# jsourati/nn-active-learning

Measured on AMD Instinct MI355X. Metric: patches/sec Fisher-scored (32^3, 2-class), higher is better.
Workload: dtype f32 (fp32 operands split into 16-bit pieces on the 16-bit MFMA, fp32 accumulate: fp16 pairs - 22-23 bits kept per operand, three products - in the conv under the head (forward + backward), in dec1's forward launch and in the other backward launches; bf16 triples - all 24 bits, exact, six products -

## Files before the change

### include/alq.h

```cpp
#ifndef ALQ_H
#define ALQ_H

#include <stddef.h>
#include <stdint.h>

#ifdef __cplusplus
extern "C" {
#endif

typedef struct alq_ctx alq_ctx;
typedef struct alq_model alq_model;

enum { ALQ_OK = 0, ALQ_EINVAL = -1, ALQ_EHIP = -2, ALQ_ENOMEM = -3, ALQ_EUNSUPPORTED = -4 };

enum { ALQ_CONV = 0, ALQ_CONVT = 1, ALQ_POOL = 2, ALQ_FC = 3 };

typedef struct {
    int32_t type;
    int32_t cout;
    int32_t k[3];
    int32_t s[3];
    int32_t relu;
    int32_t skip_src;
} alq_layer_t;
// ... 111 lines not shown
    const float *d_targets;
    const float *d_old_logits;
} alq_loss_t;

int alq_loss_stats(alq_ctx *ctx, const float *d_post, int c, int N, const int32_t *d_labels, const alq_loss_t *loss,
                   double *d_stats3);

int alq_param_grads_loss(alq_model *m, const float *d_x, int N, const int32_t *d_labels, const alq_loss_t *loss,
                         float loss_scale, float lwf_scale, float keep_prob, uint64_t seed, int64_t first_sample,
                         const int32_t *h_drop_layers, int n_drop_layers, float *d_grads, float *d_post, double *d_stats3);

int alq_rmsprop_step(alq_ctx *ctx, float *d_theta, const float *d_grad, float *d_ms, float *d_mom, int64_t n, float lr,
                     float decay, float momentum, float eps);

enum { ALQ_MT_L2 = 0, ALQ_MT_CE = 1 };
int64_t alq_mt_trip_voxels(void);
int alq_mt_cotangent(alq_ctx *ctx, const float *d_post, const float *d_teacher_post, int c, int64_t R, const int32_t *d_labels,
                     const alq_loss_t *loss, float loss_scale, float cons_scale, int measure, float *d_rows, double *d_stats3);
int alq_mt_stats(alq_ctx *ctx, const float *d_post, const float *d_teacher_post, int c, int64_t R, const int32_t *d_labels,
                 const alq_loss_t *loss, int measure, double *d_stats3);
int alq_param_grads_loss_mt(alq_model *m, const float *d_x, int N, const int32_t *d_labels, const alq_loss_t *loss,
                            float loss_scale, const float *d_teacher_post, int measure, float cons_scale, float keep_prob,
                            uint64_t seed, int64_t first_sample, const int32_t *h_drop_layers, int n_drop_layers, float *d_grads,
                            float *d_post, double *d_stats3);
int alq_model_set_aleatoric(alq_model *m, int on);
int alq_forward_au(alq_model *m, const float *d_x, int N, float keep_prob, uint64_t seed, int64_t first_sample,
                   const int32_t *h_drop_layers, int n_drop_layers, float *d_post, int64_t *d_pred, float *d_au, float *d_logits);
int64_t alq_mt_au_trip_voxels(void);
int alq_mt_cotangent_au(alq_ctx *ctx, const float *d_post, const float *d_teacher_post, const float *d_au, int c, int64_t R,
                        const int32_t *d_labels, const alq_loss_t *loss, float loss_scale, float cons_scale, float au_scale,
                        float au_log_rel_coeff, int measure, float *d_rows, double *d_stats3);
int alq_mt_stats_au(alq_ctx *ctx, const float *d_post, const float *d_teacher_post, const float *d_au, int c, int64_t R,
                    const int32_t *d_labels, const alq_loss_t *loss, float au_log_rel_coeff, int measure, double *d_stats3);
int alq_param_grads_loss_mt_au(alq_model *m, const float *d_x, int N, const int32_t *d_labels, const alq_loss_t *loss,
                               float loss_scale, const float *d_teacher_post, int measure, float cons_scale, float au_scale,
                               float au_log_rel_coeff, float keep_prob, uint64_t seed, int64_t first_sample,
                               const int32_t *h_drop_layers, int n_drop_layers, float *d_grads, float *d_post, double *d_stats3);
int alq_ema_step(alq_ctx *ctx, float *d_shadow, const float *d_theta, int64_t n, float decay);
int alq_perturb_input(alq_ctx *ctx, const float *d_x, float *d_out, int N, int H, int W, int C, float noise_std, uint64_t seed,
                      int64_t first_sample, int rotate, float angle);

int alq_sq_accum(alq_ctx *ctx, const float *d_grads, int64_t per_sample_len, int N, double *d_acc);

int alq_shrink_sum(alq_ctx *ctx, const float *d_grads, int N, int64_t P, const int64_t *h_layer_elems, int L, double *d_out);
int alq_class_layer_sums(alq_model *m, const float *d_x, int N, int J, const int32_t *d_cls, float *d_post, double *d_g);

int alq_diag_fisher(alq_model *m, const float *d_x, int N, const int32_t *d_cls, double *d_acc);

size_t alq_topk_mask_work_bytes(int64_t n);
int alq_topk_mask(alq_ctx *ctx, const double *d_v, int64_t n, int64_t k, float *d_mask, void *d_work);
int alq_threshold_mask(alq_ctx *ctx, const double *d_v, int64_t n, double thr, float *d_mask);
int alq_fisher_classes(alq_ctx *ctx, const double *d_g, const double *d_w, const double *d_diag, int N, int c, int L,
                       double *d_A);

int alq_row_norms(alq_ctx *ctx, const float *d_A, int64_t n, int f, double *d_norms);
int alq_cosine_sims(alq_ctx *ctx, const float *d_A, int64_t n, const float *d_B, int b, int f, const double *d_na,
                    const double *d_nb, double *d_C);
size_t alq_colsum_work_bytes(int64_t n, int b);
int alq_colsum_max(alq_ctx *ctx, const double *d_S, int64_t n, int b, const double *d_cmax,
                   const unsigned char *d_skip, double *d_out, void *d_work);
int alq_take_colmax(alq_ctx *ctx, const double *d_S, int64_t n, int b, int j, int first, double *d_v);
int alq_fold_rowmax(alq_ctx *ctx, const double *d_S, int t, int64_t n, double *d_v);

int alq_local_var2d(alq_ctx *ctx, const void *d_vol, int vol_is_f64, const int64_t pad_dims[3], const int32_t rads[3], int d,
                    const int64_t *d_inds, int64_t n, double *d_out);
int alq_segment_min(alq_ctx *ctx, const int32_t *d_labels, const int64_t dims[3], int32_t n_labels, const int64_t *d_inds,
                    const double *d_scores, int64_t n, double *d_table);

size_t alq_cc_work_bytes(const int64_t dims[3]);
int alq_cc_label(alq_ctx *ctx, const uint8_t *d_seg, const int64_t dims[3], int connectivity, int select_zero, int32_t *d_labels);
int alq_cc_keep_largest(alq_ctx *ctx, const uint8_t *d_seg, const int64_t dims[3], int connectivity, int skip_origin, uint8_t *d_out,
                        int64_t *d_info, void *d_work);
int alq_fill_holes(alq_ctx *ctx, const uint8_t *d_seg, const int64_t dims[3], uint8_t *d_out, int64_t *d_info, void *d_work);
int alq_cc_sizes(alq_ctx *ctx, const int32_t *d_labels, int64_t n, int32_t *d_sizes);
int alq_cc_relabel(alq_ctx *ctx, const int32_t *d_labels, int64_t n, const int32_t *d_table, const int32_t *d_sizes, int32_t min_size,
                   int32_t *d_out_i32, uint8_t *d_out_u8);

typedef struct alq_dcrf_params {
    float sdims_smooth[2];
    float sdims_app[2];
    float schan;
    float compat_smooth, compat_app;
    int32_t niter;
} alq_dcrf_params;
size_t alq_dcrf_work_bytes(const int64_t dims[3]);
int alq_dcrf2d(alq_ctx *ctx, const float *d_post, const float *d_img, const int64_t dims[3], const alq_dcrf_params *par,
               float *d_q1, uint8_t *d_map, void *d_work);

int alq_llfc_grads(alq_ctx *ctx, const float *d_feat, const float *d_post, const int32_t *d_labels, int n, int d, int c,
                   float *d_out);
size_t alq_llfc_hess_max_bytes(void);
int alq_llfc_hess(alq_ctx *ctx, const float *d_feat_one, const float *d_post_one, int d, int c, double *d_H);
int alq_llfc_if_path(int d, int c);
size_t alq_llfc_if_work_bytes(int n_pool, int c);
int alq_llfc_stoch_if(alq_ctx *ctx, const float *d_pool_feat, const float *d_pool_post, const int32_t *d_pool_labels, int n_pool,
                      const float *d_tr_feat, const float *d_tr_post, int n_tr, const int32_t *d_draws, int T, double scale, int d,
                      int c, int path, float *d_V, void *d_work);

int alq_aopt_tile(void);
int alq_aopt_max_workgroups(void);
size_t alq_aopt_work_bytes(int64_t n, int L);
int alq_aopt_svec(alq_ctx *ctx, const double *d_A, int64_t n, int L, double *d_V);
int alq_aopt_stats(alq_ctx *ctx, const double *d_V, const double *d_q, int64_t n, int m, const double *h_kvec,
                   const double *h_R, double mu, double obj, double *d_out, void *d_work);
int alq_aopt_direction(alq_ctx *ctx, const double *d_V, const double *d_q, int64_t n, int m, const double *h_kvec,
                       const double *h_R, const double *h_c_r, const double *h_c_1, double ratio, double mu, double obj,
                       double *d_dq, double *d_out, void *d_work);
int alq_aopt_linesearch(alq_ctx *ctx, const double *d_q, const double *d_dq, int64_t n, const double *h_alpha, int J,
                        double *d_out, void *d_work);
int alq_aopt_update(alq_ctx *ctx, double *d_q, const double *d_dq, const double *d_V, int64_t n, int m, double alpha,
                    double *d_out, void *d_work);

typedef struct {
    int32_t layer;
    int32_t pad;
    int64_t idx;
    double delta;
} alq_flip_t;
int alq_ref64_scores(alq_ctx *ctx, const alq_layer_t *layers, int n_layers, const int32_t in_dims[4],
                     const double *const *h_dW, const double *const *h_db, const float *d_x, const int64_t *d_rows, int N,
                     const alq_flip_t *d_flips, int flips_per_sample, double eps, int cand_cap,
                     double *d_logits, double *d_S, double *d_rms, alq_flip_t *d_cand, double *d_cand_key, int32_t *d_cand_count);

int alq_prof_enable(alq_ctx *ctx, int on);
int alq_prof_reset(alq_ctx *ctx);
int alq_prof_num_classes(void);
const char *alq_prof_class_name(int cls);
int alq_prof_read(alq_ctx *ctx, int cls, double *ms, int64_t *launches, double *flops);

int alq_model_debug_copy(alq_model *m, int layer_idx, int what, int N, float *d_out,
                         int64_t *elems_out);

int alq_debug_set_stamp_buffer(void *d_buf);
int alq_debug_set(int key, int value);
enum {
    ALQ_INFO_SUBNORMALS_OK = 0,
    ALQ_INFO_C3D_FWD = 1,
    ALQ_INFO_C3D_BWD = 2,
    ALQ_INFO_C3D_ONE_ACC = 3,
    ALQ_INFO_FLIP_OVERFLOW = 5,
    ALQ_INFO_F16_DERIVED = 6,
    ALQ_INFO_T3D_FWD = 7,
    ALQ_INFO_T3D_BWD = 8,
    ALQ_INFO_E3D_BWD = 9,
    ALQ_INFO_D3D_FWD = 10,
    ALQ_INFO_D3D_BWD = 11,
    ALQ_INFO_F3D_FWD = 12,
    ALQ_INFO_C3D_BWD_FORM = 13,
    ALQ_INFO_HOST_PACK_ELEMS = 14,
    ALQ_INFO_LSUM = 15,
    ALQ_INFO_DCP_FORM = 16,
    ALQ_INFO_E3D_BWD_FORM = 17,
    ALQ_INFO_C3D_BWD_WAVES = 19,
    ALQ_INFO_C3D_BWD_GRID = 20
};
int alq_model_engine_info(alq_model *m, int what);

int alq_synth_patches(alq_ctx *ctx, uint64_t seed, int64_t first_id, int64_t n,
                      int64_t elems_per_patch, float *d_out);

enum { ALQ_SRC_F32 = 0, ALQ_SRC_F64 = 1, ALQ_SRC_I16 = 2, ALQ_SRC_U8 = 3 };
int alq_vol_pack(alq_ctx *ctx, const void *const *d_src, int m, int src_type, const int32_t *dims, float *d_out);
int alq_mask_pack(alq_ctx *ctx, const uint8_t *d_src, const int32_t *dims, uint8_t *d_out);
int alq_slice_batch_check(const int32_t *h_dims, int nvol, const int32_t *h_desc, int b, const int32_t *crop, int C);
int alq_slice_batch(alq_ctx *ctx, const float *const *h_vols, const uint8_t *const *h_masks, const int32_t *h_dims, int nvol, int m,
                    const int32_t *h_desc, int b, const int32_t *crop, int C, float *d_X, int32_t *d_lab, int64_t *d_counts);
int64_t alq_slice_batch_trip_rows(void);
int alq_slice_batch_launch_samples(void);

#ifdef __cplusplus
}
#endif
#endif
```

### nn-active-learning_amd/csrc/alq_internal.h

```cpp
#pragma once
#include <hip/hip_runtime.h>

#include <cstdint>
#include <cstdio>
#include <memory>
#include <string>
#include <vector>

#include "alq.h"
#include "engine_switches.h"
#include "model_plan.h"

namespace alq {

#define ALQ_HIP(expr)                                                                     \
    do {                                                                                  \
        hipError_t e_ = (expr);                                                           \
        if (e_ != hipSuccess) {                                                           \
            ::alq::set_error("%s:%d: %s -> %s", __FILE__, __LINE__, #expr,               \
                             hipGetErrorString(e_));                                      \
            return ALQ_EHIP;                                                              \
        }                                                                                 \
    } while (0)

// ... 172 lines not shown
    int mask_cs = 0, mask_c0 = 0, mask_from = 0;
    int mask_to = 1 << 30;
    float *osumA = nullptr, *osumB = nullptr;
    int split = 0;
    int store_from = 0;
    int mask_split = 0;
    long long mask_delta = 0;
    const unsigned char *mask_bits = nullptr;
    unsigned char *sign_out = nullptr;
    const unsigned *in_bits = nullptr;
    const float *in_vec = nullptr;
    float in_vec_amax = 0.f;
    const unsigned *in_vec16 = nullptr;
    unsigned *out_amax = nullptr;
    int amax_from = 0;
    const unsigned *in_amax = nullptr, *in_amax2 = nullptr;
    float in_bound = 0.f;
    const float *fc_W = nullptr;
    long long fc_F = 0;
    float *fc_part = nullptr;
    unsigned *fc_bits = nullptr;
    unsigned *flip_cnt = nullptr, *flip_list = nullptr;
    int flip_cap = 0;
    float flip_l1 = 0.f;
    bool flip_bias_nonzero = false;
};

extern unsigned long long *g_igemm2_dbg;
extern int g_dbg_knobs[ALQ_NKNOBS];
inline bool two_slot_allowed() { return !g_dbg_knobs[KNOB_NO_V3] && !g_dbg_knobs[KNOB_NO_V4]; }
extern int g_dcp_last_form;
extern int g_no_f16x2;
extern int g_no_fixed;
extern int g_no_xcd_order;
int igemm2_build_plan(const IgemmPlan &p1, Igemm2Plan *p2);
void igemm2_pack_weights(Igemm2Plan *p2, const std::vector<float> &Bmat);
int igemm2_launch(alq_ctx *ctx, const Igemm2Plan &plan, const View &in, const View &out, const float *bias,
                  int relu, int accumulate, int N, int prof_cls, const Igemm2Fuse *fuse);

struct Igemm3Plan {
    bool ok = false;
    bool wres = false;
    int NTW = 1;
    int wgs_per_cu = 1;
    size_t lds_bytes = 0;
    std::vector<unsigned short> h_W;
    void *d_W = nullptr;
    std::vector<unsigned short> h_W16;
    void *d_W16 = nullptr;
    int w16_exp = 0;
};
int igemm3_build_plan(const Igemm2Plan &p2, Igemm3Plan *p3);
void igemm3_pack_weights(const Igemm2Plan &p2, Igemm3Plan *p3, const std::vector<float> &Bmat);
void igemm3_pack_weights_f16(const Igemm2Plan &p2, Igemm3Plan *p3, const std::vector<float> &Bmat);
int igemm3_launch(alq_ctx *ctx, const Igemm2Plan &p2, const Igemm3Plan &plan, const View &in, const View &out,
                  const float *bias, int relu, int accumulate, int N, int prof_cls, const Igemm2Fuse *fuse);

struct Igemm4Args {
    const float *in;
    float *out;
    const void *W;
    const float *bias;
    const float *mask;
    float *osumA, *osumB;
    const int *tdesc;
    const int *sdesc;
    const int *pdesc;
    const int *ttab;
    const int *vdesc;
    int in_cs, in_c0, out_cs, out_c0, Co;
    int mask_cs, mask_c0, mask_from, mask_to, split;
    int N, PT, tpg, rows;
    int PX, PYX, PZ;
    int smz, smy, smx;
    int soz, soy, sox, OD, OH, OW;
    int MD, MH, MW;
    int nph, ngr, NP;
    int nslots, plane_bytes;
    int in_pstride, out_pstride, in_bytes;
    int relu, accumulate, pair, store_from;
    int cls_ok;
    int in_split_ch, in_delta, out_split, out_delta, mask_split, mask_delta;
    int tt_ints, pd_off, td_off, wbytes, abytes;
    int dbg_repeat;
    unsigned long long *dbg;
    const unsigned *src_bits;
    int bits_pstride, bits_bytes;
    const float *fc_W;
    float *fc_part;
    unsigned char *fc_bits;
    int fc_F;
    int f16_ein;
    int f16_ew;
    const unsigned *in_amax, *in_amax2;
    unsigned *out_amax;
    int amax_from;
    int wp;
    int src_presplit;
    int xcd_order;
    int zreuse;
    float flip_tau;
    int flip_cap;
    unsigned *flip_cnt;
    unsigned *flip_list;
    const unsigned char *mask_bits;
    unsigned char *sign_out;
};

struct Igemm4Plan {
    bool ok = false;
    Igemm4Args a;
    int NTW = 1;
    int wp = 3;
    int xw = 0;
    std::shared_ptr<Igemm4Plan> alt16;
    bool multi = false;
    bool fic = false;
    int tune_fic = -1;
    int tune_epi = -1;
    size_t lds_bytes = 0;
    double flops_per_patch = 0;
    int Ci = 0, Co = 0;
    struct Unit { int chunk = 0, S = 0, w_off = 0; std::vector<int> tap; };
    std::vector<Unit> units;
    std::vector<int> h_tdesc, h_sdesc, h_pdesc, h_ttab, h_vdesc;
    int *d_tdesc = nullptr, *d_sdesc = nullptr, *d_pdesc = nullptr, *d_ttab = nullptr, *d_vdesc = nullptr;
    std::vector<unsigned short> h_W;
    void *d_W = nullptr;
    std::vector<unsigned short> h_W16;
    void *d_W16 = nullptr;
    int w16_exp = 0;
};
int igemm4_build_plan(const G4Geom &g, int max_batch, Igemm4Plan *plan, int wp = 3);
void igemm4_pack_weights(Igemm4Plan *plan, const std::vector<float> &Bmat );
int igemm4_launch(alq_ctx *ctx, const Igemm4Plan &plan, const View &in, const View &out, const float *bias,
                  int relu, int accumulate, int N, int prof_cls, const Igemm2Fuse *fuse);

struct C3dPlan {
    bool ok = false;
    int D = 0;
    int w_exp = 0;
    int oneacc = 1;
    double flops_per_patch = 0;
    std::vector<unsigned short> h_W;
    void *d_W = nullptr;
    std::vector<unsigned short> h_W7;
    void *d_W7 = nullptr;
};
void c3d_bwd7_pack(C3dPlan *plan, const std::vector<float> &Bmat);
int c3d_subnormals_ok(alq_ctx *ctx);
int c3d_fwd_build(const View &in, const View &out, const int k[3], const int lo[3], const int s[3], C3dPlan *plan);
void c3d_fwd_pack(C3dPlan *plan, const std::vector<float> &Bmat );
int c3d_fwd_launch(alq_ctx *ctx, const C3dPlan &plan, const View &in, const float *bias, int N, const unsigned *amaxA, const unsigned *amaxB,
                   const float *fc_W, float *fc_part, float *asum_part, unsigned char *fc_bits, float flip_tau);
int c3d_bwd_build(const View &fwd_in, const View &fwd_out, const int k[3], const int lo[3], const int s[3], C3dPlan *plan);
void c3d_bwd_pack(C3dPlan *plan, const std::vector<float> &Bmat_fwd );
void c3d_presplit_vec(const float *v, long long F, int e, std::vector<unsigned short> *out);
int c3d_bwd_launch(alq_ctx *ctx, const C3dPlan &plan, int N, const unsigned char *bits, const void *vec16, int e_in, const unsigned char *maskA,
                   float *dB, float *sumA, float *sumB, int rows_per_wave = 8, int waves_per_simd = 1 ,
                   int *grid_out = nullptr );

struct T3dPlan {
    bool ok = false;
    int kind = 0;
    int w_exp = 0;
    double flops_per_patch = 0;
    std::vector<unsigned short> h_W;
    void *d_W = nullptr;
};
int t3d_build(const View &in, const View &out, const int k[3], const int lo[3], const int s[3], T3dPlan *fwd, T3dPlan *bwd);
void t3d_fwd_pack(T3dPlan *plan, const float *W );
void t3d_bwd_pack(T3dPlan *plan, const float *W);
void t3d8_fwd_pack(T3dPlan *plan, const float *W );
void t3d8_bwd_pack(T3dPlan *plan, const float *W );
int t3d8_bwd_launch(alq_ctx *ctx, const T3dPlan &plan, const View &dout, const View &din, int N, float in_bound, const unsigned char *mask_bits, float *dsum);
int t3d_fwd_launch(alq_ctx *ctx, const T3dPlan &plan, const View &in, const View &out, const float *bias, int N, float *osum, unsigned *out_amax);
int t3d_bwd_launch(alq_ctx *ctx, const T3dPlan &plan, const View &dout, const View &din, int N, float in_bound, const unsigned char *mask_bits,
                   float *dsum);

struct E3dPlan {
    bool ok = false;
    int w_exp = 0;
    double flops_per_patch = 0;
    std::vector<unsigned short> h_Whi, h_Wlo;
    void *d_Whi = nullptr, *d_Wlo = nullptr;
};
int e3d_build(const View &in, const View &out, const int k[3], const int lo[3], const int s[3], E3dPlan *plan);
void e3d_pack(E3dPlan *plan, const float *W );
int e3d_bwd_launch(alq_ctx *ctx, const E3dPlan &plan, int N, const float *skip, const float *dpool, const unsigned char *am2, const unsigned char *sg2,
                   const unsigned char *am1, const unsigned char *sg1, float *dsum2, float *dsum1, float in_bound,
                   bool rows );

struct D3dPlan {
    bool ok = false;
    int w_exp = 0;
    double flops_per_patch = 0;
    std::vector<unsigned short> h_Whi, h_Wlo;
    void *d_Whi = nullptr, *d_Wlo = nullptr;
    std::vector<unsigned short> h_Bhi, h_Blo;
    void *d_Bhi = nullptr, *d_Blo = nullptr;
};
void d3d_bwd_pack(D3dPlan *plan, const float *W);
int d3d_bwd_launch(alq_ctx *ctx, const D3dPlan &plan, int N, const float *dout, float in_bound, float *dinA, float *dinB, float *sumB);
int d3d_build(const View &in, const View &out, const int k[3], const int lo[3], const int s[3], D3dPlan *plan);
void d3d_pack(D3dPlan *plan, const float *W );
int d3d_fwd_launch(alq_ctx *ctx, const D3dPlan &plan, int N, const float *inA, const float *inB, const unsigned *amaxA, const unsigned *amaxB,
                   const float *bias, int relu, float *out, unsigned char *sg, float *osum);

struct F3dPlan {
    bool ok = false;
    int w_exp = 0;
    double flops_per_patch = 0;
    std::vector<unsigned short> h_Whi, h_Wlo;
    void *d_Whi = nullptr, *d_Wlo = nullptr;
};
int f3d_build(const View &in, const View &out, const int k[3], const int lo[3], const int s[3], F3dPlan *plan);
void f3d_pack(F3dPlan *plan, const float *W );
int f3d_fwd_launch(alq_ctx *ctx, const F3dPlan &plan, int N, const float *in, const unsigned *amax, const float *bias, float *out, unsigned char *sg,
                   float *osum, float *pout, unsigned char *parg, float *posum);

struct DirectArgs {
    const float *in;
    float *out;
    const float *W;
    const float *bias;
    float *osum;
    int in_cs, in_c0, Ci, ID, IH, IW;
    int out_cs, out_c0, Co, OD, OH, OW;
    int MD, MH, MW;
    int PT, TZ, TY, TX, HZ, HY, HX, rows;
    int minz, miny, minx;
    int ntaps, tnx, tny, tnz;
    int tilesZ, tilesY, tilesX;
    int N, relu;
};

struct DirectPlan {
    DirectArgs a;
    bool ok = false;
    size_t lds_bytes = 0;
    double flops_per_patch = 0;
    float *d_W = nullptr;
};

int direct_build_plan(const IgemmPlan &p1, DirectPlan *dp);
int direct_launch(alq_ctx *ctx, const DirectPlan &dp, const View &in, const View &out, const float *bias, int relu,
                  int N, float *osum, int prof_cls);
int direct_conv_pool_launch(alq_ctx *ctx, const float *d_W, const View &in, const View &out, const View &pout,
                            const float *bias, int relu, uint8_t *argmax, float *osum, float *posum, int N,
                            double flops_per_patch, unsigned *amax = nullptr, unsigned char *sg = nullptr, unsigned char *psg = nullptr);

struct FcGemmPlan {
    bool ok = false;
    int K = 0, N = 0;
    std::vector<unsigned short> h_W;
    void *d_W = nullptr;
    std::vector<unsigned short> h_W16;
    void *d_W16 = nullptr;
    int w_exp = 0;
    int form = 0;
};
int fcgemm_build_plan(int K, int N, FcGemmPlan *plan);
void fcgemm_pack_weights(FcGemmPlan *plan, const std::vector<float> &Bmat );
void fcgemm_pack_weights_f16(FcGemmPlan *plan, const std::vector<float> &Bmat );
int fcgemm_launch(alq_ctx *ctx, const FcGemmPlan &plan, const View &in, const View &out, const float *bias, int relu,
                  int M, int prof_cls, float in_bound = 0.f, unsigned *row_amax = nullptr);

int wpack_stats(alq_ctx *ctx, const float *d_W, int Co, long long F, void *d_scal);
int wpack_permute(alq_ctx *ctx, const float *d_W, float *d_Wp, int Co, int D, int H, int Wd, int C);
int wpack_fc(alq_ctx *ctx, const float *d_Wp, long long ld, int K, int N, int kmajor, void *d_W3, void *d_W16, const void *d_scal);

struct Gemm {
    IgemmPlan p1;
    Igemm2Plan p2;
    Igemm3Plan p3;
    Igemm4Plan p4;
    FcGemmPlan pfc;
    bool pfc_f16 = false;
    bool p3_f16 = false;
    unsigned *fc_row_amax = nullptr;
    DirectPlan pd;
};

int k_pool_fwd(alq_ctx *, const View &in, const View &out, uint8_t *argmax, const int w[3],
               const int lo[3], int N, float *osum = nullptr, bool *fused = nullptr);
int k_pool_bwd_first(alq_ctx *, const View &dout, const View &pool_out, const uint8_t *argmax, const int w[3],
                     int ID, int IH, int IW, int N, float *dsum, int accumulate, int use_signs = 0);
int k_pool_bwd(alq_ctx *, const View &dout, const View &din, const uint8_t *argmax,
               const int w[3], const int lo[3], int N, int accumulate, const View *mask_act = nullptr,
               float *dsum = nullptr, bool *fused = nullptr, int store_din = 1, int use_signs = 0);
int k_chansum(alq_ctx *, const View &in, float *field, int N);
int k_mask_chansum(alq_ctx *, const View &dact, const View *act_or_null, float *field, int N);
int boxdot_slabs(long long vox);
int boxdot_conv_slabs(int D, int H, int W, const int k[3]);
int boxdot_convT_slabs(int ID, int IH, int IW, const int k[3], const int s[3]);
int k_boxdot_conv(alq_ctx *, const float *dsum, const float *asum, const float *asum2, int D, int H, int W,
                  const int k[3], const int lo[3], int N, double *Spart, int nslab_max);
int k_boxdot_convT(alq_ctx *, const float *dsum, const float *asum, const float *asum2, int ID, int IH, int IW,
                   const int k[3], const int s[3], const int lo[3], int N, double *Spart, int nslab_max);
int k_fc_small_fwd(alq_ctx *, const float *act, int64_t F, const float *Wp, int nout, int N,
                   float *partials, int nslices, unsigned *maskbits = nullptr);
int k_fc_small_dsum_bits(alq_ctx *, const unsigned *maskbits, const float *wv, int64_t F, int N, float *dsum);
int k_fc_small_finish(alq_ctx *, const float *partials, int nslices, const float *bias, int nout,
                      int relu, int N, float *out);
int k_fc_small_finish_diff(alq_ctx *, const float *partials, int nslices, const float *bias, int N, float *out);
int k_fc_small_bwd(alq_ctx *, const float *delta, int nout, const float *Wp, int64_t F, int N,
                   float *dact, const float *mask_act = nullptr, float *dsum = nullptr, int C = 0,
// ... 151 lines not shown
```

### nn-active-learning_amd/csrc/c3d.hip

```cpp
#include "f16_pair.h"
#include "sweep_common.h"

#include <algorithm>
#include <cmath>
#include <cstdlib>
#include <cstring>
#include <vector>

namespace alq {

namespace {
#ifndef C3_SCHED_MASK
#define C3_SCHED_MASK 0
#endif
#ifndef C3_PF
#define C3_PF 8
#endif
#ifndef C3_WD
#define C3_WD 4
#endif
static_assert(C3_PF == 8 || C3_PF == 16, "the ring of staging registers must divide the 16 units of a plane");
static_assert(C3_WD >= 1 && C3_WD <= 8, "weight-difference slices are fetched 1..8 rows ahead");
#ifndef C3_ABL
#define C3_ABL 0
#endif
#ifndef C3_PIPE
#define C3_PIPE 2
#endif
#ifndef C3_FILL_MASK
#define C3_FILL_MASK SW_FILL_MASK
#endif
#ifndef C3_PIN_SUMS
#define C3_PIN_SUMS 1
#endif
#ifndef C3_PEEL
#define C3_PEEL 1
#endif
#ifndef C3_EPI2
#define C3_EPI2 1
#endif
#ifndef C3_BPIPE
#define C3_BPIPE 2
#endif
#ifndef C3_B7PIPE
#define C3_B7PIPE 4
#endif
#ifndef C3_B7PIPE2
#define C3_B7PIPE2 2
#endif
#ifndef C3_B7PINW
#define C3_B7PINW 0
#endif
#ifndef C3_B7ABL
#define C3_B7ABL 0
#endif

constexpr int C3_TEN = 34 * 16;
constexpr int C3_PIECE = 2 * C3_TEN;
constexpr int C3_ROW = 2 * C3_PIECE;
constexpr int C3_PLANE = 34 * C3_ROW;
constexpr int C3_LDS = 2 * C3_PLANE;
static_assert(C3_LDS <= 160 * 1024, "two plane images must fit the CU's LDS");
}

struct C3FwdArgs {
    const float *inA, *inB;
    const void *W;
    const float *bias;
    const unsigned *amaxA, *amaxB;
    const float *fc_W;
    float *fc_part;
    float *asum_part;
    unsigned char *fc_bits;
    int N, D;
    int e_w;
    float flip_tau;
    unsigned long long *clk;
};

template <bool SUMS, bool ONEACC>
__global__ __launch_bounds__(256) __attribute__((amdgpu_waves_per_eu(1, 1))) void c3d_fwd_kernel(const C3FwdArgs a) {
    extern __shared__ __attribute__((aligned(16))) char lds[];
    const int tid = threadIdx.x;
    const int lane = tid & 63;
    const int wave = __builtin_amdgcn_readfirstlane(tid >> 6);
    const int lr = lane & 15, lq = lane >> 4;
    const int D = a.D;
    const unsigned plane_f = 32u * 32u * 8u;
    const unsigned patch_f = (unsigned)D * plane_f;

    for (int i = tid * 16; i < C3_LDS; i += 256 * 16) *reinterpret_cast<i32x4 *>(lds + i) = i32x4{0, 0, 0, 0};

    f16x8 Wh[18], Wl[18];
    {
        const i32x4 *Wg = reinterpret_cast<const i32x4 *>(a.W);
#pragma unroll
        for (int k = 0; k < 18; ++k) {
            Wh[k] = __builtin_bit_cast(f16x8, Wg[(k * 2 + 0) * 64 + lane]);
            Wl[k] = __builtin_bit_cast(f16x8, Wg[(k * 2 + 1) * 64 + lane]);
        }
#ifndef C3_NO_PIN
#pragma unroll
        for (int k = 0; k < 18; ++k) {
            i32x4 h = __builtin_bit_cast(i32x4, Wh[k]), l = __builtin_bit_cast(i32x4, Wl[k]);
            asm volatile("" : "+a"(h), "+a"(l));
            Wh[k] = __builtin_bit_cast(f16x8, h); Wl[k] = __builtin_bit_cast(f16x8, l);
        }
#endif
    }
    const f32x4 bias4 = *reinterpret_cast<const f32x4 *>(a.bias + (lq & 1) * 4);

    const int frag_lane = (lq >> 1) * C3_TEN + (2 * lr + (lq & 1)) * 16 + wave * 8 * C3_ROW;
    const int st_lane = (wave * 8 + 1) * C3_ROW + 16 + lane * 8;
    const unsigned epi_lane_f = 16u * lr + 4u * lq;

    const int G = gridDim.x, b0 = blockIdx.x;
    const int np = b0 < a.N ? (a.N - b0 + G - 1) / G : 0;
#ifdef C3_CLK
    const unsigned long long clk0 = __builtin_amdgcn_s_memtime(), rt0 = __builtin_amdgcn_s_memrealtime();
#endif

    f32x4 acc[3][8], accx[3][ONEACC ? 1 : 8];
#pragma unroll
    for (int s = 0; s < 3; ++s)
#pragma unroll
        for (int i = 0; i < 8; ++i) { acc[s][i] = f32x4{0.f, 0.f, 0.f, 0.f}; if constexpr (!ONEACC) accx[s][i] = f32x4{0.f, 0.f, 0.f, 0.f}; }

    typedef const unsigned __attribute__((address_space(4))) *cu32p;
    const cu32p amaxA_c = (cu32p)(unsigned long long)a.amaxA, amaxB_c = (cu32p)(unsigned long long)a.amaxB;
    auto patch_exp = [&](int p) __attribute__((always_inline)) {
        const unsigned fa = amaxA_c[p], fb = amaxB_c[p];
        return sw_patch_exp(fa > fb ? fa : fb);
    };
    const __amdgpu_buffer_rsrc_t inA_rsrc = sw_rsrc(a.inA, (unsigned long long)a.N * patch_f * 4u);
    const __amdgpu_buffer_rsrc_t inB_rsrc = sw_rsrc(a.inB, (unsigned long long)a.N * patch_f * 4u);
    const __amdgpu_buffer_rsrc_t wd_rsrc = sw_rsrc(a.fc_W, (unsigned long long)patch_f * 4u);
    const __amdgpu_buffer_rsrc_t bits_rsrc = sw_rsrc(a.fc_bits, (SUMS && a.fc_bits) ? (unsigned long long)a.N * (patch_f >> 2) : 0ull);
    auto patch_of = [&](int pi) __attribute__((always_inline)) { return (unsigned)(b0 + pi * G); };

    f32x4 R4[C3_PF];
    float sc = 1.f, sc11 = 2048.f;
    auto stage_unit = [&](int wbase, auto U) __attribute__((always_inline)) {
        constexpr int u = decltype(U)::value;
        const f32x4 v = R4[u % C3_PF];
        const float x0 = v.x * sc, x1 = v.y * sc, x2 = v.z * sc, x3 = v.w * sc;
        const f16x2 h01 = __builtin_convertvector(f32x2{x0, x1}, f16x2);
        const f16x2 h23 = __builtin_convertvector(f32x2{x2, x3}, f16x2);
        const f32x2 g01 = __builtin_convertvector(h01, f32x2), g23 = __builtin_convertvector(h23, f32x2);
        f16x2 l01, l23;
        if constexpr (ONEACC) {
            l01 = __builtin_convertvector(f32x2{x0 - g01.x, x1 - g01.y}, f16x2);
            l23 = __builtin_convertvector(f32x2{x2 - g23.x, x3 - g23.y}, f16x2);
        } else {
            l01 = __builtin_convertvector(f32x2{__builtin_fmaf(g01.x, -2048.f, v.x * sc11), __builtin_fmaf(g01.y, -2048.f, v.y * sc11)}, f16x2);
            l23 = __builtin_convertvector(f32x2{__builtin_fmaf(g23.x, -2048.f, v.z * sc11), __builtin_fmaf(g23.y, -2048.f, v.w * sc11)}, f16x2);
        }
        char *dst = lds + wbase + (u >> 1) * C3_ROW + (u & 1) * C3_TEN;
        if constexpr (C3_ABL & 64) { asm volatile("" :: "v"(h01), "v"(h23), "v"(l01), "v"(l23), "v"(dst)); return; }
        *reinterpret_cast<uint2 *>(dst) = uint2{__builtin_bit_cast(unsigned, h01), __builtin_bit_cast(unsigned, h23)};
        *reinterpret_cast<uint2 *>(dst + C3_PIECE) = uint2{__builtin_bit_cast(unsigned, l01), __builtin_bit_cast(unsigned, l23)};
    };
    auto load_unit = [&](unsigned voff, unsigned soff, auto U) __attribute__((always_inline)) {
        constexpr int u = decltype(U)::value;
        R4[u % C3_PF] = __builtin_bit_cast(f32x4, __builtin_amdgcn_raw_buffer_load_b128((u & 1) ? inB_rsrc : inA_rsrc, (int)voff, (int)(soff + (unsigned)((u % 16) >> 1) * 1024u), 0));
    };
    struct Cur { unsigned voff, soff; };
    auto cursor = [&](int pi, int z) __attribute__((always_inline)) {
        Cur c;
        const bool ok = pi < np;
        c.voff = ok ? (unsigned)lane * 16u : SW_OOB;
        c.soff = ok ? (patch_of(pi) * patch_f + (unsigned)z * plane_f) * 4u + (unsigned)(wave * 8) * 1024u : 0u;
        if constexpr (C3_ABL & 8) c.soff = (unsigned)(wave * 8) * 1024u;
        return c;
    };
    int c1_pi = 0, c1_z = 0, c2_pi = 0, c2_z = 0;
    auto advance = [&](int &pi, int &z) __attribute__((always_inline)) { if (++z == D) { z = 0; ++pi; } };

    float fs = 0.f, sa = 0.f;
    f32x4 wdq[C3_WD];
#pragma unroll
    for (int i = 0; i < C3_WD; ++i) wdq[i] = f32x4{0.f, 0.f, 0.f, 0.f};

    struct Epi { float inv; f32x4 b4; float tau; unsigned tau_u; unsigned zadj; unsigned off_w, off_b, row_f, bits_s; };
    auto epi_setup = [&](bool valid, int pe, int zo) __attribute__((always_inline)) {
        Epi e;
        const int p = valid ? (int)patch_of(pe) : 0;
        const int ce = valid ? patch_exp(p) : 0;
        e.inv = valid ? __builtin_ldexpf(1.f, -(ce + a.e_w)) : 0.f;
        e.b4 = valid ? bias4 : f32x4{0.f, 0.f, 0.f, 0.f};
        e.tau = (valid && (amaxA_c[p] | amaxB_c[p]) != 0u) ? __builtin_ldexpf(a.flip_tau, 14 - ce) : 0.f;
        e.tau_u = e.tau > 0.f ? (__builtin_bit_cast(unsigned, e.tau) - 1u) >> 1 : 0u;
        e.zadj = (bias4.x == 0.f && bias4.y == 0.f && bias4.z == 0.f && bias4.w == 0.f) ? 1u : 0u;
        e.off_w = valid ? epi_lane_f * 4u : SW_OOB;
        e.off_b = valid ? (epi_lane_f >> 2) : SW_OOB;
        e.row_f = (unsigned)(zo * 32 + wave * 8) * 256u;
        e.bits_s = (unsigned)p * (patch_f >> 2);
        return e;
    };
    auto wd_load = [&](const Epi &E, auto I) __attribute__((always_inline)) {
        constexpr int i = decltype(I)::value;
        if constexpr (C3_ABL & 32) return;
        wdq[i % C3_WD] = __builtin_bit_cast(f32x4, __builtin_amdgcn_raw_buffer_load_b128(wd_rsrc, (int)E.off_w, (int)((E.row_f + (unsigned)i * 256u) * 4u), 0));
    };

    auto wd_first = [&](const Epi &E) __attribute__((always_inline)) {
        wd_load(E, IC<0>{});
        if constexpr (C3_WD > 1) wd_load(E, IC<1>{});
        if constexpr (C3_WD > 2) wd_load(E, IC<2>{});
        if constexpr (C3_WD > 3) wd_load(E, IC<3>{});
        if constexpr (C3_WD > 4) wd_load(E, IC<4>{});
        if constexpr (C3_WD > 5) wd_load(E, IC<5>{});
        if constexpr (C3_WD > 6) wd_load(E, IC<6>{});
        if constexpr (C3_WD > 7) wd_load(E, IC<7>{});
    };
    auto epi_row = [&](auto S, auto I, const Epi &E) __attribute__((always_inline)) {
        constexpr int s = decltype(S)::value, i = decltype(I)::value;
        const f32x4 w4 = wdq[i % C3_WD];
        if constexpr (i + C3_WD < 8) wd_load(E, IC<i + C3_WD>{});
        const f32x4 c = acc[s][i];
        f32x4 val;
        if constexpr (ONEACC) {
            val.x = __builtin_fmaf(c.x, E.inv, E.b4.x); val.y = __builtin_fmaf(c.y, E.inv, E.b4.y);
            val.z = __builtin_fmaf(c.z, E.inv, E.b4.z); val.w = __builtin_fmaf(c.w, E.inv, E.b4.w);
        } else {
            const f32x4 d = accx[s][i];
            val.x = __builtin_fmaf(__builtin_fmaf(d.x, 0x1p-11f, c.x), E.inv, E.b4.x);
            val.y = __builtin_fmaf(__builtin_fmaf(d.y, 0x1p-11f, c.y), E.inv, E.b4.y);
            val.z = __builtin_fmaf(__builtin_fmaf(d.z, 0x1p-11f, c.z), E.inv, E.b4.z);
            val.w = __builtin_fmaf(__builtin_fmaf(d.w, 0x1p-11f, c.w), E.inv, E.b4.w);
        }
        unsigned unsure = 0u;
        if constexpr (SUMS) {
            const float mn = fminf(fminf(__builtin_fabsf(val.x), __builtin_fabsf(val.y)), fminf(__builtin_fabsf(val.z), __builtin_fabsf(val.w)));
#if C3_EPI2
            unsure = (((__builtin_bit_cast(unsigned, mn) - E.zadj) >> 1) - E.tau_u) >> 31;
#else
            unsure = (mn < E.tau && mn > 0.f) ? 16u : 0u;
#endif
        }
        val.x = fmaxf(val.x, 0.f); val.y = fmaxf(val.y, 0.f); val.z = fmaxf(val.z, 0.f); val.w = fmaxf(val.w, 0.f);
        fs += __builtin_fmaf(val.y, w4.y, val.x * w4.x) + __builtin_fmaf(val.w, w4.w, val.z * w4.z);
        if constexpr (SUMS) {
            sa += (val.x + val.y) + (val.z + val.w);
#if C3_EPI2
            const float r0 = val.x, r1 = val.y, r2 = val.z, r3 = val.w;
            unsigned nib = unsure;
            nib = __builtin_amdgcn_alignbit(nib, 0u - __builtin_bit_cast(unsigned, r3), 31);
            nib = __builtin_amdgcn_alignbit(nib, 0u - __builtin_bit_cast(unsigned, r2), 31);
            nib = __builtin_amdgcn_alignbit(nib, 0u - __builtin_bit_cast(unsigned, r1), 31);
            nib = __builtin_amdgcn_alignbit(nib, 0u - __builtin_bit_cast(unsigned, r0), 31);
#else
            const unsigned nib = (val.x > 0.f ? 1u : 0u) | (val.y > 0.f ? 2u : 0u) | (val.z > 0.f ? 4u : 0u) | (val.w > 0.f ? 8u : 0u) | unsure;
#endif
            if constexpr (!(C3_ABL & 16))
                __builtin_amdgcn_raw_buffer_store_b8((unsigned char)nib, bits_rsrc, (int)E.off_b, (int)(E.bits_s + ((E.row_f + (unsigned)i * 256u) >> 2)), 0);
            else asm volatile("" :: "v"(nib));
        }
#if C3_PIN_SUMS
        if constexpr (SUMS) asm volatile("" : "+v"(fs), "+v"(sa));
        else asm volatile("" : "+v"(fs));
#endif
    };
    auto wave_sum = [&](float x) __attribute__((always_inline)) {
        int v = __builtin_bit_cast(int, x);
#define C3_ROW_SHR_ADD(n) v = __builtin_bit_cast(int, __builtin_bit_cast(float, v) + __builtin_bit_cast(float, __builtin_amdgcn_update_dpp(0, v, 0x110 + (n), 0xf, 0xf, true)))
        C3_ROW_SHR_ADD(1); C3_ROW_SHR_ADD(2); C3_ROW_SHR_ADD(4); C3_ROW_SHR_ADD(8);
#undef C3_ROW_SHR_ADD
        const float r0 = __builtin_bit_cast(float, __builtin_amdgcn_readlane(v, 15));
        const float r1 = __builtin_bit_cast(float, __builtin_amdgcn_readlane(v, 31));
        const float r2 = __builtin_bit_cast(float, __builtin_amdgcn_readlane(v, 47));
        const float r3 = __builtin_bit_cast(float, __builtin_amdgcn_readlane(v, 63));
        return (r0 + r1) + (r2 + r3);
    };
    auto finish_patch = [&](int p) __attribute__((always_inline)) {
        const float t = wave_sum(fs);
        if (lane == 0) a.fc_part[(size_t)p * 4 + wave] = t;
        if constexpr (SUMS) {
            const float u = wave_sum(sa);
            if (lane == 0 && a.asum_part) a.asum_part[(size_t)p * 4 + wave] = u;
        }
        fs = 0.f; sa = 0.f;
    };

    auto step = [&](auto RR, int pi, int z, long long n) __attribute__((always_inline)) {
        constexpr int R = decltype(RR)::value;
        constexpr int S_lo = (R + 2) % 3, S_mid = R, S_hi = (R + 1) % 3;
        if constexpr (!(C3_ABL & 4)) asm volatile("s_waitcnt lgkmcnt(0)\n\ts_barrier" ::: "memory");
        const int abase = frag_lane + (int)(n & 1) * C3_PLANE;
        const int wbase = st_lane + (int)((n + 1) & 1) * C3_PLANE;
        const Cur C1 = cursor(c1_pi, c1_z), C2 = cursor(c2_pi, c2_z);
        {
            const int ce = c1_pi < np ? patch_exp((int)patch_of(c1_pi)) : 0;
            sc = __builtin_ldexpf(1.f, ce); sc11 = __builtin_ldexpf(1.f, ce + 11);
        }
        const bool ev = z >= 2 || (z == 0 && pi > 0);
        const Epi E = epi_setup(ev, z >= 2 ? pi : pi - 1, z >= 2 ? z - 2 : D - 1);

        auto frag = [&](int j, int s, f16x8 &bh, f16x8 &bl) __attribute__((always_inline)) {
            const char *p = lds + abase + j * C3_ROW + s * 32;
            bh = __builtin_bit_cast(f16x8, *reinterpret_cast<const i32x4 *>(p));
            bl = __builtin_bit_cast(f16x8, *reinterpret_cast<const i32x4 *>(p + C3_PIECE));
        };
        f16x8 Fh[3], Fl[3];
        frag(0, 0, Fh[0], Fl[0]);
        frag(0, 1, Fh[1], Fl[1]);
        auto block = [&](auto J, auto SS) __attribute__((always_inline)) {
            constexpr int j = decltype(J)::value, s = decltype(SS)::value, b = 2 * j + s;
            __builtin_amdgcn_sched_barrier(0);
            if constexpr (s == 0 && j < 8) {
                if constexpr (!(C3_ABL & 2)) epi_row(IC<S_hi>{}, J, E);
            }
            if constexpr (!(C3_ABL & 1) && j >= 2) {
                constexpr int u = 2 * (j - 2) + s;
                stage_unit(wbase, IC<u>{});
                if constexpr (u + C3_PF < 16) load_unit(C1.voff, C1.soff, IC<u + C3_PF>{}); else load_unit(C2.voff, C2.soff, IC<u + C3_PF - 16>{});
            }
            if constexpr (b + 2 < 20) frag((b + 2) / 2, (b + 2) & 1, Fh[(b + 2) % 3], Fl[(b + 2) % 3]);
            const f16x8 bh = Fh[b % 3], bl = Fl[b % 3];
            constexpr int rows_here = (j < 2 ? j + 1 : 3) < (10 - j) ? (j < 2 ? j + 1 : 3) : (10 - j);
#pragma unroll
            for (int di = 0; di < 3; ++di) {
                const int i = j - di;
                if (i < 0 || i > 7) continue;
#pragma unroll
                for (int dzi = 0; dzi < 3; ++dzi) {
                    const int k = (dzi * 3 + di) * 2 + s;
                    const int set = dzi == 0 ? S_hi : (dzi == 1 ? S_mid : S_lo);
                    const bool start = dzi == 0 && di == 0 && s == 0;
                    f32x4 c = acc[set][i];
                    if (start) c = f32x4{0.f, 0.f, 0.f, 0.f};
                    if constexpr (ONEACC) {
                        c = __builtin_amdgcn_mfma_f32_16x16x32_f16(Wl[k], bh, c, 0, 0, 0);
                        c = __builtin_amdgcn_mfma_f32_16x16x32_f16(Wh[k], bl, c, 0, 0, 0);
                        c = __builtin_amdgcn_mfma_f32_16x16x32_f16(Wh[k], bh, c, 0, 0, 0);
                    } else {
                        f32x4 d = accx[set][i];
                        if (start) d = f32x4{0.f, 0.f, 0.f, 0.f};
                        d = __builtin_amdgcn_mfma_f32_16x16x32_f16(Wl[k], bh, d, 0, 0, 0);
                        c = __builtin_amdgcn_mfma_f32_16x16x32_f16(Wh[k], bh, c, 0, 0, 0);
                        d = __builtin_amdgcn_mfma_f32_16x16x32_f16(Wh[k], bl, d, 0, 0, 0);
                        accx[set][i] = d;
                    }
                    acc[set][i] = c;
                }
            }
#if C3_PIPE
#pragma unroll
            for (int m = 0; m < 9 * rows_here; ++m) {
                __builtin_amdgcn_sched_group_barrier(0x008, 1, 0);
                __builtin_amdgcn_sched_group_barrier(C3_FILL_MASK, C3_PIPE, 0);
            }
#endif
        };
        auto row = [&](auto J) __attribute__((always_inline)) { block(J, IC<0>{}); block(J, IC<1>{}); };
        row(IC<0>{}); row(IC<1>{}); row(IC<2>{}); row(IC<3>{}); row(IC<4>{});
        row(IC<5>{}); row(IC<6>{}); row(IC<7>{}); row(IC<8>{}); row(IC<9>{});
        {
            const Epi En = epi_setup(z + 1 < D ? z >= 1 : true, pi, z + 1 < D ? z - 1 : D - 2);
            wd_first(En);
        }
        if constexpr (R == 0) { if (z == 0 && pi > 0) finish_patch((int)patch_of(pi - 1)); }
        c1_pi = c2_pi; c1_z = c2_z;
        advance(c2_pi, c2_z);
    };
    auto light = [&](auto S, int pe, int zo) __attribute__((always_inline)) {
        constexpr int s = decltype(S)::value;
        const Epi E = epi_setup(true, pe, zo);
        auto rows = [&](auto I) __attribute__((always_inline)) { epi_row(S, I, E); };
        rows(IC<0>{}); rows(IC<1>{}); rows(IC<2>{}); rows(IC<3>{}); rows(IC<4>{}); rows(IC<5>{}); rows(IC<6>{}); rows(IC<7>{});
#pragma unroll
        for (int i = 0; i < 8; ++i) { acc[s][i] = f32x4{0.f, 0.f, 0.f, 0.f}; if constexpr (!ONEACC) accx[s][i] = f32x4{0.f, 0.f, 0.f, 0.f}; }
        {
            const Epi En = epi_setup(zo == D - 2, pe, D - 1);
            wd_first(En);
        }
    };

    __syncthreads();
    if (np > 0) {
        const Cur C0 = cursor(0, 0);
        const int ce = patch_exp((int)patch_of(0));
        sc = __builtin_ldexpf(1.f, ce); sc11 = __builtin_ldexpf(1.f, ce + 11);
        const int wb = st_lane;
        auto eight = [&](auto U0) __attribute__((always_inline)) {
            constexpr int u0 = decltype(U0)::value;
            load_unit(C0.voff, C0.soff, IC<u0>{}); load_unit(C0.voff, C0.soff, IC<u0 + 1>{}); load_unit(C0.voff, C0.soff, IC<u0 + 2>{}); load_unit(C0.voff, C0.soff, IC<u0 + 3>{});
            load_unit(C0.voff, C0.soff, IC<u0 + 4>{}); load_unit(C0.voff, C0.soff, IC<u0 + 5>{}); load_unit(C0.voff, C0.soff, IC<u0 + 6>{}); load_unit(C0.voff, C0.soff, IC<u0 + 7>{});
            stage_unit(wb, IC<u0>{}); stage_unit(wb, IC<u0 + 1>{}); stage_unit(wb, IC<u0 + 2>{}); stage_unit(wb, IC<u0 + 3>{});
            stage_unit(wb, IC<u0 + 4>{}); stage_unit(wb, IC<u0 + 5>{}); stage_unit(wb, IC<u0 + 6>{}); stage_unit(wb, IC<u0 + 7>{});
        };
        eight(IC<0>{}); eight(IC<8>{});
        c1_pi = 0; c1_z = 0;
        advance(c1_pi, c1_z);
        c2_pi = c1_pi; c2_z = c1_z;
        advance(c2_pi, c2_z);
        const Cur C1 = cursor(c1_pi, c1_z);
        load_unit(C1.voff, C1.soff, IC<0>{}); load_unit(C1.voff, C1.soff, IC<1>{}); load_unit(C1.voff, C1.soff, IC<2>{}); load_unit(C1.voff, C1.soff, IC<3>{});
        load_unit(C1.voff, C1.soff, IC<4>{}); load_unit(C1.voff, C1.soff, IC<5>{}); load_unit(C1.voff, C1.soff, IC<6>{}); load_unit(C1.voff, C1.soff, IC<7>{});
        if constexpr (C3_PF == 16) {
            load_unit(C1.voff, C1.soff, IC<8>{}); load_unit(C1.voff, C1.soff, IC<9>{}); load_unit(C1.voff, C1.soff, IC<10>{}); load_unit(C1.voff, C1.soff, IC<11>{});
            load_unit(C1.voff, C1.soff, IC<12>{}); load_unit(C1.voff, C1.soff, IC<13>{}); load_unit(C1.voff, C1.soff, IC<14>{}); load_unit(C1.voff, C1.soff, IC<15>{});
        }
    }

    long long n = 0;
    for (int pi = 0; pi < np; ++pi) {
#if C3_PEEL
        for (int zz = 0; zz < 10; ++zz) {
            step(IC<0>{}, pi, 3 * zz, n); ++n;
            step(IC<1>{}, pi, 3 * zz + 1, n); ++n;
            step(IC<2>{}, pi, 3 * zz + 2, n); ++n;
        }
        step(IC<0>{}, pi, 30, n); ++n;
        step(IC<1>{}, pi, 31, n); ++n;
        light(IC<0>{}, pi, D - 2);
#else
        for (int zz = 0; zz < 11; ++zz) {
            step(IC<0>{}, pi, 3 * zz, n); ++n;
            step(IC<1>{}, pi, 3 * zz + 1, n); ++n;
            if (zz < 10) { step(IC<2>{}, pi, 3 * zz + 2, n); ++n; }
            else light(IC<0>{}, pi, D - 2);
        }
#endif
    }
    if (np > 0) {
        light(IC<1>{}, np - 1, D - 1);
        finish_patch((int)patch_of(np - 1));
    }
#ifdef C3_CLK
    if (a.clk && tid == 0) { a.clk[2 * b0] = __builtin_amdgcn_s_memtime() - clk0; a.clk[2 * b0 + 1] = __builtin_amdgcn_s_memrealtime() - rt0; }
#endif
}

namespace {
constexpr int B3_TEN = 34 * 16;
constexpr int B3_ROW = 2 * B3_TEN;
}

struct C3BwdArgs {
    const unsigned char *bits;
    const void *vec;
    const void *W;
    const unsigned char *maskA;
    float *dB;
    float *sumA, *sumB;
    int N, D;
    int e_in, e_w;
};

template <bool ONEACC, int RW>
__global__ __launch_bounds__(256) __attribute__((amdgpu_waves_per_eu(1, 1))) void c3d_bwd_kernel(const C3BwdArgs a) {
    extern __shared__ __attribute__((aligned(16))) char lds[];
    static_assert(ONEACC, "the backward kernel is built for the one-accumulator form");
    static_assert(RW == 4 || RW == 8, "4 waves x RW rows: a half or a whole patch per workgroup");
    constexpr int NR = 4 * RW;
    constexpr int NPARTS = 32 / NR;
    constexpr int PLANE = (NR + 2) * B3_ROW;
    constexpr int DUMMY = 2 * PLANE;
    constexpr int NU = RW / 2;
    const int tid = threadIdx.x;
    const int lane = tid & 63;
    const int wave = __builtin_amdgcn_readfirstlane(tid >> 6);
    const int lj = lane & 15, lq = lane >> 4;
    const int D = a.D;
    const unsigned plane_v = 32u * 32u;
    const unsigned patch_v = (unsigned)D * plane_v;

    for (int i = tid * 16; i < DUMMY + 2 * B3_ROW; i += 256 * 16) *reinterpret_cast<i32x4 *>(lds + i) = i32x4{0, 0, 0, 0};

    f16x8 Wh[9], Wl[9];
    {
        const i32x4 *Wg = reinterpret_cast<const i32x4 *>(a.W);
#pragma unroll
        for (int k = 0; k < 9; ++k) {
            Wh[k] = __builtin_bit_cast(f16x8, Wg[(k * 2 + 0) * 64 + lane]);
            Wl[k] = __builtin_bit_cast(f16x8, Wg[(k * 2 + 1) * 64 + lane]);
        }
        if constexpr (RW == 4) {
#pragma unroll
            for (int k = 0; k < 9; ++k) {
                i32x4 h = __builtin_bit_cast(i32x4, Wh[k]), l = __builtin_bit_cast(i32x4, Wl[k]);
                asm volatile("" : "+a"(h), "+a"(l));
                Wh[k] = __builtin_bit_cast(f16x8, h); Wl[k] = __builtin_bit_cast(f16x8, l);
            }
        }
    }
    const int frag_lane = (lj + (lq < 2 ? lq : 2)) * 16 + wave * RW * B3_ROW;
    const int st_lane = (wave * RW + 1 + (lane >> 5)) * B3_ROW + ((lane & 31) + 1) * 16;
    const float inv = __builtin_ldexpf(1.f, -(a.e_in + a.e_w));

    const int G = gridDim.x, b0 = blockIdx.x;
    const int nitems = a.N * NPARTS;
    const int np = b0 < nitems ? (nitems - b0 + G - 1) / G : 0;

    f32x4 acc[3][RW][2];
#pragma unroll
    for (int s = 0; s < 3; ++s)
#pragma unroll
        for (int i = 0; i < RW; ++i) { acc[s][i][0] = f32x4{0.f, 0.f, 0.f, 0.f}; acc[s][i][1] = f32x4{0.f, 0.f, 0.f, 0.f}; }

    const __amdgpu_buffer_rsrc_t vec_rsrc = sw_rsrc(a.vec, (unsigned long long)patch_v * 32u);
    const __amdgpu_buffer_rsrc_t bits_rsrc = sw_rsrc(a.bits, (unsigned long long)a.N * patch_v * 2u);
    const __amdgpu_buffer_rsrc_t mask_rsrc = sw_rsrc(a.maskA, a.maskA ? (unsigned long long)a.N * patch_v * 2u : 0ull);
    const __amdgpu_buffer_rsrc_t dB_rsrc = sw_rsrc(a.dB, (unsigned long long)a.N * patch_v * 32u);
    const __amdgpu_buffer_rsrc_t sA_rsrc = sw_rsrc(a.sumA, (unsigned long long)a.N * patch_v * 4u);
    const __amdgpu_buffer_rsrc_t sB_rsrc = sw_rsrc(a.sumB, (unsigned long long)a.N * patch_v * 4u);
    auto item_patch = [&](int pi) __attribute__((always_inline)) { return (unsigned)((b0 + pi * G) / NPARTS); };
    auto item_y0 = [&](int pi) __attribute__((always_inline)) { return ((b0 + pi * G) % NPARTS) * NR; };

    i32x4 Vh[2], Vl[2], Hh, Hl;
    unsigned Sb[2], Hb = 0u;
    struct Src { unsigned voff, vvox, soff; };
    auto src_of = [&](int pi, bool halo) __attribute__((always_inline)) {
        Src c;
        const bool ok = pi < np;
        const int y0 = ok ? item_y0(pi) : 0;
        int y = y0 + wave * RW + (lane >> 5);
        bool live = ok;
        if (halo) {
            y = wave == 0 ? y0 - 1 : y0 + NR;
            live = ok && lane < 32 && y >= 0 && y < 32;
        }
        c.vvox = (unsigned)((live ? y : 0) * 32 + (lane & 31));
        c.voff = live ? c.vvox * 2u : SW_OOB;
        c.soff = ok ? item_patch(pi) * patch_v * 2u : 0u;
        return c;
    };
    auto mask8 = [&](int b, i32x4 h, i32x4 l, i32x4 *oh, i32x4 *ol) __attribute__((always_inline)) {
// ... 211 lines not shown
        }
        c1_pi = 0; c1_z = 0;
        advance(c1_pi, c1_z);
        c2_pi = c1_pi; c2_z = c1_z;
        advance(c2_pi, c2_z);
        const Src C1 = src_of(c1_pi, false);
        load_unit(C1, (unsigned)c1_z, IC<0>{}); load_unit(C1, (unsigned)c1_z, IC<1>{});
        if constexpr (RW == 4) { if (halo_wave) load_halo(src_of(c1_pi, true), (unsigned)c1_z); }
    }
    long long n = 0;
    for (int pi = 0; pi < np; ++pi) {
#if C3_PEEL
        for (int zz = 0; zz < 10; ++zz) {
            step(IC<0>{}, pi, 3 * zz, n); ++n;
            step(IC<1>{}, pi, 3 * zz + 1, n); ++n;
            step(IC<2>{}, pi, 3 * zz + 2, n); ++n;
        }
        step(IC<0>{}, pi, 30, n); ++n;
        step(IC<1>{}, pi, 31, n); ++n;
        light(IC<0>{}, pi, D - 2);
#else
        for (int zz = 0; zz < 11; ++zz) {
            step(IC<0>{}, pi, 3 * zz, n); ++n;
            step(IC<1>{}, pi, 3 * zz + 1, n); ++n;
            if (zz < 10) { step(IC<2>{}, pi, 3 * zz + 2, n); ++n; }
            else light(IC<0>{}, pi, D - 2);
        }
#endif
    }
    if (np > 0) light(IC<1>{}, np - 1, D - 1);
}

namespace {
constexpr int P7_ROW = 34 * 16;
constexpr int P7_PIECE = 34 * P7_ROW;
constexpr int P7_PLANE = 2 * P7_PIECE + 128;
constexpr int P7_LDS = 4 * P7_PLANE;
constexpr int P7_WS = 2 * 64 * 16;
static_assert((P7_ROW / 16) % 16 == 2 && (P7_PLANE / 16) % 16 == 0 && P7_LDS + P7_WS <= 160 * 1024, "bank-conflict-free pitches (see above)");
}

template <int RW, int NW>
__global__ __launch_bounds__(NW * 64) __attribute__((amdgpu_waves_per_eu(NW / 4, NW / 4))) void c3d_bwd7_kernel(const C3BwdArgs a) {
    extern __shared__ __attribute__((aligned(16))) char lds[];
    static_assert(RW * NW == 32 && (NW == 4 || NW == 8), "the waves' strips of RW rows tile the 32 rows of a plane");
    constexpr int NU = RW / 2;
    constexpr int FSETS = NW == 4 ? 2 : 1;
    constexpr int PIPE = NW == 4 ? C3_B7PIPE : C3_B7PIPE2;
    constexpr bool WS_LDS = NW == 8;
    const int tid = threadIdx.x;
    const int lane = tid & 63;
    const int wave = __builtin_amdgcn_readfirstlane(tid >> 6);
    const int lj = lane & 15, lq = lane >> 4;
    const int D = a.D;
    const unsigned plane_v = 32u * 32u;
    const unsigned patch_v = (unsigned)D * plane_v;

    for (int i = tid * 16; i < P7_LDS; i += NW * 64 * 16) *reinterpret_cast<i32x4 *>(lds + i) = i32x4{0, 0, 0, 0};

    f16x8 Wa[3][2], Wb[3][2], Ws[2];
    {
        const i32x4 *Wg = reinterpret_cast<const i32x4 *>(a.W);
#pragma unroll
        for (int dz = 0; dz < 3; ++dz)
#pragma unroll
            for (int pc = 0; pc < 2; ++pc) {
                Wa[dz][pc] = __builtin_bit_cast(f16x8, Wg[((0 + dz) * 2 + pc) * 64 + lane]);
                Wb[dz][pc] = __builtin_bit_cast(f16x8, Wg[((3 + dz) * 2 + pc) * 64 + lane]);
            }
        Ws[0] = __builtin_bit_cast(f16x8, Wg[(6 * 2 + 0) * 64 + lane]);
        Ws[1] = __builtin_bit_cast(f16x8, Wg[(6 * 2 + 1) * 64 + lane]);
        if constexpr (WS_LDS) {
            if (wave == 0) {
                *reinterpret_cast<i32x4 *>(lds + P7_LDS + lane * 16) = __builtin_bit_cast(i32x4, Ws[0]);
                *reinterpret_cast<i32x4 *>(lds + P7_LDS + 1024 + lane * 16) = __builtin_bit_cast(i32x4, Ws[1]);
            }
        }
#if C3_B7PINW
#pragma unroll
        for (int dz = 0; dz < 3; ++dz)
#pragma unroll
            for (int pc = 0; pc < 2; ++pc) {
                i32x4 x = __builtin_bit_cast(i32x4, Wa[dz][pc]), y = __builtin_bit_cast(i32x4, Wb[dz][pc]);
                asm volatile("" : "+a"(x), "+a"(y));
                Wa[dz][pc] = __builtin_bit_cast(f16x8, x); Wb[dz][pc] = __builtin_bit_cast(f16x8, y);
            }
#endif
    }
    const int offA = wave * RW * P7_ROW + (lq < 3 ? (lj + lq) * 16 : P7_ROW + lj * 16);
    const int offB = (wave * RW + 1) * P7_ROW + (lq < 2 ? (lj + 1 + lq) * 16 : P7_ROW + (lj + lq - 2) * 16);
    const int offS = (wave * RW + 2) * P7_ROW + (lj + 2) * 16;
    const int ringS = lq < 2 ? lq + 2 : 0;
    const int st_lane = (wave * RW + 1 + (lane >> 5)) * P7_ROW + ((lane & 31) + 1) * 16;
    const float inv = __builtin_ldexpf(1.f, -(a.e_in + a.e_w));

    const int G = gridDim.x, b0 = blockIdx.x;
    const int np = b0 < a.N ? (a.N - b0 + G - 1) / G : 0;

    f32x4 acc[3][RW][2];
#pragma unroll
    for (int s = 0; s < 3; ++s)
#pragma unroll
        for (int i = 0; i < RW; ++i) { acc[s][i][0] = f32x4{0.f, 0.f, 0.f, 0.f}; acc[s][i][1] = f32x4{0.f, 0.f, 0.f, 0.f}; }

    const __amdgpu_buffer_rsrc_t vec_rsrc = sw_rsrc(a.vec, (unsigned long long)patch_v * 32u);
    const __amdgpu_buffer_rsrc_t bits_rsrc = sw_rsrc(a.bits, (unsigned long long)a.N * patch_v * 2u);
    const __amdgpu_buffer_rsrc_t mask_rsrc = sw_rsrc(a.maskA, a.maskA ? (unsigned long long)a.N * patch_v * 2u : 0ull);
    const __amdgpu_buffer_rsrc_t dB_rsrc = sw_rsrc(a.dB, (unsigned long long)a.N * patch_v * 32u);
    const __amdgpu_buffer_rsrc_t sA_rsrc = sw_rsrc(a.sumA, (unsigned long long)a.N * patch_v * 4u);
    const __amdgpu_buffer_rsrc_t sB_rsrc = sw_rsrc(a.sumB, (unsigned long long)a.N * patch_v * 4u);
    auto item_patch = [&](int pi) __attribute__((always_inline)) { return (unsigned)(b0 + pi * G); };

    i32x4 Vh[2], Vl[2];
    unsigned Sb[2];
    struct Src { unsigned voff, vvox, soff; };
    auto src_of = [&](int pi) __attribute__((always_inline)) {
        Src c;
        const bool ok = pi < np;
        const int y = wave * RW + (lane >> 5);
        c.vvox = (unsigned)(y * 32 + (lane & 31));
        c.voff = ok ? c.vvox * 2u : SW_OOB;
        c.soff = ok ? item_patch(pi) * patch_v * 2u : 0u;
        return c;
    };
    auto mask8 = [&](int b, i32x4 h, i32x4 l, i32x4 *oh, i32x4 *ol) __attribute__((always_inline)) {
        const unsigned m0 = (unsigned)__builtin_amdgcn_sbfe(b, 0, 1), m1 = (unsigned)__builtin_amdgcn_sbfe(b, 1, 1);
        const unsigned m2 = (unsigned)__builtin_amdgcn_sbfe(b, 2, 1), m3 = (unsigned)__builtin_amdgcn_sbfe(b, 3, 1);
        const unsigned m4 = (unsigned)__builtin_amdgcn_sbfe(b, 8, 1), m5 = (unsigned)__builtin_amdgcn_sbfe(b, 9, 1);
        const unsigned m6 = (unsigned)__builtin_amdgcn_sbfe(b, 10, 1), m7 = (unsigned)__builtin_amdgcn_sbfe(b, 11, 1);
        const unsigned k0 = (m0 & 0xffffu) | (m1 & 0xffff0000u), k1 = (m2 & 0xffffu) | (m3 & 0xffff0000u);
        const unsigned k2 = (m4 & 0xffffu) | (m5 & 0xffff0000u), k3 = (m6 & 0xffffu) | (m7 & 0xffff0000u);
        *oh = i32x4{(int)((unsigned)h.x & k0), (int)((unsigned)h.y & k1), (int)((unsigned)h.z & k2), (int)((unsigned)h.w & k3)};
        *ol = i32x4{(int)((unsigned)l.x & k0), (int)((unsigned)l.y & k1), (int)((unsigned)l.z & k2), (int)((unsigned)l.w & k3)};
    };
    auto load_unit = [&](const Src &c, unsigned z, auto U) __attribute__((always_inline)) {
        constexpr int u = decltype(U)::value;
        const unsigned so = (z * plane_v + (unsigned)u * 64u);
        Vh[u & 1] = __builtin_amdgcn_raw_buffer_load_b128(vec_rsrc, (int)(c.vvox * 32u), (int)(so * 32u), 0);
        Vl[u & 1] = __builtin_amdgcn_raw_buffer_load_b128(vec_rsrc, (int)(c.vvox * 32u + 16u), (int)(so * 32u), 0);
        Sb[u & 1] = (unsigned short)__builtin_amdgcn_raw_buffer_load_b16(bits_rsrc, (int)c.voff, (int)(c.soff + so * 2u), 0);
    };
    auto stage_unit = [&](int wbase, auto U) __attribute__((always_inline)) {
        constexpr int u = decltype(U)::value;
        i32x4 oh, ol;
        mask8((int)Sb[u & 1], Vh[u & 1], Vl[u & 1], &oh, &ol);
        char *dst = lds + wbase + (2 * u) * P7_ROW;
        *reinterpret_cast<i32x4 *>(dst) = oh;
        *reinterpret_cast<i32x4 *>(dst + P7_PIECE) = ol;
    };

    int c1_pi = 0, c1_z = 0, c2_pi = 0, c2_z = 0;
    auto advance = [&](int &pi, int &z) __attribute__((always_inline)) { if (++z == D) { z = 0; ++pi; } };

    unsigned mkq[2][2] = {{0u, 0u}, {0u, 0u}};
    struct Epi { unsigned pv; unsigned row_v; float inv; unsigned off_mask, off_dB, off_sum; };
    auto epi_setup = [&](bool valid, int pe, int zo) __attribute__((always_inline)) {
        Epi e;
        e.pv = valid ? item_patch(pe) * patch_v : 0u;
        e.row_v = (unsigned)(zo * 32 + wave * RW) * 32u;
        e.inv = valid ? inv : 0.f;
        e.off_mask = (valid && lq < 2) ? (unsigned)(lj * 2 + lq) : SW_OOB;
        e.off_dB = (valid && lq >= 2) ? (unsigned)lj * 32u + (unsigned)(lq - 2) * 16u : SW_OOB;
        e.off_sum = valid ? (unsigned)((lq & 1) * 16 + lj) * 4u : SW_OOB;
        return e;
    };
    auto mask_load = [&](const Epi &E, auto I) __attribute__((always_inline)) {
        constexpr int i = decltype(I)::value;
#pragma unroll
        for (int hx = 0; hx < 2; ++hx)
            mkq[i & 1][hx] = (unsigned char)__builtin_amdgcn_raw_buffer_load_b8(mask_rsrc, (int)E.off_mask,
                                                                               (int)((E.pv + E.row_v + (unsigned)i * 32u + (unsigned)hx * 16u) * 2u), 0);
    };
    const bool has_mask = a.maskA != nullptr;
    float t_keep = 0.f;
    auto epi_half = [&](auto S, auto I, auto HX, const Epi &E) __attribute__((always_inline)) {
        constexpr int s = decltype(S)::value, i = decltype(I)::value, hx = decltype(HX)::value;
        const unsigned mk = mkq[i & 1][hx];
        if constexpr (hx == 1 && i + 2 < RW) mask_load(E, IC<i + 2>{});
        const f32x4 c = acc[s][i][hx];
        const int nib = (lq < 2 && has_mask) ? (int)mk : 15;
        const float v0 = c.x * E.inv, v1 = c.y * E.inv, v2 = c.z * E.inv, v3 = c.w * E.inv;
        f32x4 val;
        unsigned k0 = (unsigned)__builtin_amdgcn_sbfe(nib, 0, 1), k1 = (unsigned)__builtin_amdgcn_sbfe(nib, 1, 1);
        unsigned k2 = (unsigned)__builtin_amdgcn_sbfe(nib, 2, 1), k3 = (unsigned)__builtin_amdgcn_sbfe(nib, 3, 1);
        asm("" : "+v"(k0), "+v"(k1), "+v"(k2), "+v"(k3));
        val.x = __builtin_bit_cast(float, __builtin_bit_cast(unsigned, v0) & k0);
        val.y = __builtin_bit_cast(float, __builtin_bit_cast(unsigned, v1) & k1);
        val.z = __builtin_bit_cast(float, __builtin_bit_cast(unsigned, v2) & k2);
        val.w = __builtin_bit_cast(float, __builtin_bit_cast(unsigned, v3) & k3);
        const unsigned vox = E.pv + E.row_v + (unsigned)i * 32u + (unsigned)hx * 16u;
        __builtin_amdgcn_raw_buffer_store_b128(__builtin_bit_cast(i32x4, val), dB_rsrc, (int)E.off_dB, (int)(vox * 32u), 2 );
        if constexpr (!(C3_B7ABL & 8)) ALQ_STORE_HOLD("v"(val));
        const float t = (val.x + val.y) + (val.z + val.w);
        const unsigned tu = __builtin_bit_cast(unsigned, t);
        const auto sw = hx == 0 ? __builtin_amdgcn_permlane16_swap(tu, 0u, false, false) : __builtin_amdgcn_permlane16_swap(0u, tu, false, false);
        const unsigned s0 = sw[0], s1 = sw[1];
        const float t2 = __builtin_bit_cast(float, s0) + __builtin_bit_cast(float, s1);
        if constexpr (hx == 0) {
            t_keep = t2;
        } else {
            const float ts = t_keep + t2;
            const unsigned rowv = E.pv + E.row_v + (unsigned)i * 32u;
            __builtin_amdgcn_raw_buffer_store_b32(__builtin_bit_cast(int, ts), sA_rsrc, (int)(lq < 2 ? E.off_sum : SW_OOB), (int)(rowv * 4u), 0);
            __builtin_amdgcn_raw_buffer_store_b32(__builtin_bit_cast(int, ts), sB_rsrc, (int)(lq >= 2 ? E.off_sum : SW_OOB), (int)(rowv * 4u), 0);
        }
    };
    auto epi_row = [&](auto S, auto I, const Epi &E) __attribute__((always_inline)) {
        epi_half(S, I, IC<0>{}, E);
        epi_half(S, I, IC<1>{}, E);
    };
    auto s_weights = [&](int kill, f16x8 &sh, f16x8 &sl) __attribute__((always_inline)) {
        const int km = lq == kill ? 0 : -1;
        i32x4 h, l;
        if constexpr (WS_LDS) {
            h = *reinterpret_cast<const i32x4 *>(lds + P7_LDS + lane * 16);
            l = *reinterpret_cast<const i32x4 *>(lds + P7_LDS + 1024 + lane * 16);
        } else {
            h = __builtin_bit_cast(i32x4, Ws[0]); l = __builtin_bit_cast(i32x4, Ws[1]);
        }
        h.x &= km; h.y &= km; h.z &= km; h.w &= km;
        l.x &= km; l.y &= km; l.z &= km; l.w &= km;
        sh = __builtin_bit_cast(f16x8, h); sl = __builtin_bit_cast(f16x8, l);
    };
    auto mac3 = [&](f32x4 c, const f16x8 &wh, const f16x8 &wl, const f16x8 &bh, const f16x8 &bl) __attribute__((always_inline)) {
        c = __builtin_amdgcn_mfma_f32_16x16x32_f16(wl, bh, c, 0, 0, 0);
        c = __builtin_amdgcn_mfma_f32_16x16x32_f16(wh, bl, c, 0, 0, 0);
        c = __builtin_amdgcn_mfma_f32_16x16x32_f16(wh, bh, c, 0, 0, 0);
        return c;
    };

    auto step = [&](auto RR, int pi, int z, long long n) __attribute__((always_inline)) {
        constexpr int R = decltype(RR)::value;
        constexpr int S_lo = (R + 2) % 3, S_mid = R, S_hi = (R + 1) % 3;
        asm volatile("s_waitcnt lgkmcnt(0)\n\ts_barrier" ::: "memory");
        const int cur = (int)(n & 3) * P7_PLANE;
        const int baseA = offA + cur, baseB = offB + cur;
        const int baseS = offS + (int)((unsigned)((int)(n & 3) + ringS) & 3u) * P7_PLANE;
        const int wbase = st_lane + (int)((n + 1) & 3) * P7_PLANE;
        const Src C1 = src_of(c1_pi), C2 = src_of(c2_pi);
        const unsigned z1 = (unsigned)c1_z, z2 = (unsigned)c2_z;
        const bool ev = z >= 2 || (z == 0 && pi > 0);
        const Epi E = epi_setup(ev, z >= 2 ? pi : pi - 1, z >= 2 ? z - 2 : D - 1);
        f16x8 sh, sl;
        s_weights(z == 1 ? 0 : -1, sh, sl);

        struct Frag { f16x8 ah, al, bh, bl, sh, sl; };
        auto frag_s = [&](int i, int hx, Frag &f) __attribute__((always_inline)) {
            const int o = i * P7_ROW + hx * 256;
            f.sh = __builtin_bit_cast(f16x8, *reinterpret_cast<const i32x4 *>(lds + baseS + o));
            f.sl = __builtin_bit_cast(f16x8, *reinterpret_cast<const i32x4 *>(lds + baseS + o + P7_PIECE));
        };
        auto frag_a = [&](int i, int hx, Frag &f) __attribute__((always_inline)) {
            const int o = i * P7_ROW + hx * 256;
            f.ah = __builtin_bit_cast(f16x8, *reinterpret_cast<const i32x4 *>(lds + baseA + o));
            f.al = __builtin_bit_cast(f16x8, *reinterpret_cast<const i32x4 *>(lds + baseA + o + P7_PIECE));
        };
        auto frag_b = [&](int i, int hx, Frag &f) __attribute__((always_inline)) {
            const int o = i * P7_ROW + hx * 256;
            f.bh = __builtin_bit_cast(f16x8, *reinterpret_cast<const i32x4 *>(lds + baseB + o));
            f.bl = __builtin_bit_cast(f16x8, *reinterpret_cast<const i32x4 *>(lds + baseB + o + P7_PIECE));
        };
        auto frag_ab = [&](int i, int hx, Frag &f) __attribute__((always_inline)) { frag_a(i, hx, f); frag_b(i, hx, f); };
        auto frag = [&](int i, int hx, Frag &f) __attribute__((always_inline)) { frag_ab(i, hx, f); frag_s(i, hx, f); };
        Frag fc, fn;
        if constexpr (FSETS == 2) frag(0, 0, fc);
        if constexpr (FSETS == 1) frag_a(0, 0, fc);
        auto mfma_half = [&](auto I, int hx) __attribute__((always_inline)) {
            constexpr int i = decltype(I)::value;
            f32x4 c0 = f32x4{0.f, 0.f, 0.f, 0.f}, c1 = acc[S_mid][i][hx], c2 = acc[S_lo][i][hx];
            c0 = mac3(c0, Wa[0][0], Wa[0][1], fc.ah, fc.al);
            c1 = mac3(c1, Wa[1][0], Wa[1][1], fc.ah, fc.al);
            c2 = mac3(c2, Wa[2][0], Wa[2][1], fc.ah, fc.al);
            c0 = mac3(c0, Wb[0][0], Wb[0][1], fc.bh, fc.bl);
            c1 = mac3(c1, Wb[1][0], Wb[1][1], fc.bh, fc.bl);
            c2 = mac3(c2, Wb[2][0], Wb[2][1], fc.bh, fc.bl);
            if constexpr (!(C3_B7ABL & 4)) c2 = mac3(c2, sh, sl, fc.sh, fc.sl);
            acc[S_hi][i][hx] = c0; acc[S_mid][i][hx] = c1; acc[S_lo][i][hx] = c2;
        };
        auto row = [&](auto I) __attribute__((always_inline)) {
            constexpr int i = decltype(I)::value;
            __builtin_amdgcn_sched_barrier(0);
            if constexpr (FSETS == 1) {
                static_assert(NU == 2, "two units per plane and wave");
#pragma unroll
                for (int hx = 0; hx < 2; ++hx) {
                    frag_b(i, hx, fc);
                    if constexpr (!(C3_B7ABL & 4)) frag_s(i, hx, fc);
                    if constexpr (!(C3_B7ABL & 1)) {
                        if (hx == 0) epi_half(IC<S_hi>{}, I, IC<0>{}, E);
                        else epi_half(IC<S_hi>{}, I, IC<1>{}, E);
                    } else { const f32x4 k0 = acc[S_hi][i][hx]; asm volatile("" :: "v"(k0)); }
                    if (hx == 0) frag_a(i, 1, fn);
                    else if (i < RW - 1) frag_a(i + 1, 0, fn);
                    if constexpr ((i & 1) == 0 && !(C3_B7ABL & 2)) {
                        if (hx == 1) {
                            stage_unit(wbase, IC<i / 2>{});
                            load_unit(C2, z2, IC<i / 2>{});
                        }
                    }
                    mfma_half(I, hx);
                    fc.ah = fn.ah; fc.al = fn.al;
                    if constexpr (PIPE != 0) {
#pragma unroll
                        for (int m = 0; m < 21; ++m) {
                            __builtin_amdgcn_sched_group_barrier(0x008, 1, 0);
                            __builtin_amdgcn_sched_group_barrier(C3_FILL_MASK, PIPE, 0);
                        }
                        __builtin_amdgcn_sched_barrier(0);
                    }
                }
                return;
            }
            if constexpr (!(C3_B7ABL & 1)) epi_row(IC<S_hi>{}, I, E);
            else { const f32x4 k0 = acc[S_hi][i][0], k1 = acc[S_hi][i][1]; asm volatile("" :: "v"(k0), "v"(k1)); }
            if constexpr ((i & 1) == 0 && !(C3_B7ABL & 2)) {
                stage_unit(wbase, IC<i / 2>{});
                if constexpr (i / 2 + 2 < NU) load_unit(C1, z1, IC<i / 2 + 2>{}); else load_unit(C2, z2, IC<i / 2 + 2 - NU>{});
            }
#pragma unroll
            for (int hx = 0; hx < 2; ++hx) {
                if (hx == 0) frag(i, 1, fn);
                else if (i < RW - 1) frag(i + 1, 0, fn);
                mfma_half(I, hx);
                fc = fn;
            }
            if constexpr (PIPE != 0) {
#pragma unroll
                for (int m = 0; m < 42; ++m) {
                    __builtin_amdgcn_sched_group_barrier(0x008, 1, 0);
                    __builtin_amdgcn_sched_group_barrier(C3_FILL_MASK, PIPE, 0);
                }
            }
        };
        row(IC<0>{}); row(IC<1>{}); row(IC<2>{}); row(IC<3>{});
        if constexpr (RW == 8) { row(IC<4>{}); row(IC<5>{}); row(IC<6>{}); row(IC<7>{}); }
        {
            const Epi En = epi_setup(z + 1 < D ? z >= 1 : true, pi, z + 1 < D ? z - 1 : D - 2);
            mask_load(En, IC<0>{});
            mask_load(En, IC<1>{});
        }
        c1_pi = c2_pi; c1_z = c2_z;
        advance(c2_pi, c2_z);
    };
    auto light = [&](auto S, auto LAST, int pe, int zo, long long n) __attribute__((always_inline)) {
        constexpr int s = decltype(S)::value;
        constexpr bool last = decltype(LAST)::value != 0;
        const Epi E = epi_setup(true, pe, zo);
        auto rows = [&](auto I) __attribute__((always_inline)) { epi_row(S, I, E); };
        rows(IC<0>{}); rows(IC<1>{}); rows(IC<2>{}); rows(IC<3>{});
        if constexpr (RW == 8) { rows(IC<4>{}); rows(IC<5>{}); rows(IC<6>{}); rows(IC<7>{}); }
#pragma unroll
        for (int i = 0; i < RW; ++i) { acc[s][i][0] = f32x4{0.f, 0.f, 0.f, 0.f}; acc[s][i][1] = f32x4{0.f, 0.f, 0.f, 0.f}; }
        if constexpr (last) {
            constexpr int sp = (s + 1) % 3;
            f16x8 sh, sl;
            s_weights(2, sh, sl);
            const int baseS = offS + (int)((unsigned)((int)(n & 3) + ringS) & 3u) * P7_PLANE;
#pragma unroll
            for (int i = 0; i < RW; ++i)
#pragma unroll
                for (int hx = 0; hx < 2; ++hx) {
                    const int o = i * P7_ROW + hx * 256;
                    const f16x8 bh = __builtin_bit_cast(f16x8, *reinterpret_cast<const i32x4 *>(lds + baseS + o));
                    const f16x8 bl = __builtin_bit_cast(f16x8, *reinterpret_cast<const i32x4 *>(lds + baseS + o + P7_PIECE));
                    acc[sp][i][hx] = mac3(acc[sp][i][hx], sh, sl, bh, bl);
                }
        }
        {
            const Epi En = epi_setup(zo == D - 2, pe, D - 1);
            mask_load(En, IC<0>{});
            mask_load(En, IC<1>{});
        }
    };

    __syncthreads();
    if (np > 0) {
        const Src C0 = src_of(0);
        const int wb = st_lane;
        load_unit(C0, 0u, IC<0>{}); load_unit(C0, 0u, IC<1>{});
        stage_unit(wb, IC<0>{}); stage_unit(wb, IC<1>{});
        if constexpr (NU == 4) {
            load_unit(C0, 0u, IC<2>{}); load_unit(C0, 0u, IC<3>{});
            stage_unit(wb, IC<2>{}); stage_unit(wb, IC<3>{});
        }
        c1_pi = 0; c1_z = 0;
        advance(c1_pi, c1_z);
        c2_pi = c1_pi; c2_z = c1_z;
        advance(c2_pi, c2_z);
        const Src C1 = src_of(c1_pi);
        load_unit(C1, (unsigned)c1_z, IC<0>{}); load_unit(C1, (unsigned)c1_z, IC<1>{});
    }
    long long n = 0;
    for (int pi = 0; pi < np; ++pi) {
        for (int zz = 0; zz < 10; ++zz) {
            step(IC<0>{}, pi, 3 * zz, n); ++n;
            step(IC<1>{}, pi, 3 * zz + 1, n); ++n;
            step(IC<2>{}, pi, 3 * zz + 2, n); ++n;
        }
        step(IC<0>{}, pi, 30, n); ++n;
        step(IC<1>{}, pi, 31, n); ++n;
        light(IC<0>{}, IC<1>{}, pi, D - 2, n);
    }
    if (np > 0) light(IC<1>{}, IC<0>{}, np - 1, D - 1, n);
}

__global__ void c3d_subnormal_probe(float *out) {
    f16x8 a, b;
#pragma unroll
    for (int i = 0; i < 8; ++i) { a[i] = (_Float16)0x1p-20f; b[i] = (_Float16)0x1p10f; }
    const f32x4 d = __builtin_amdgcn_mfma_f32_16x16x32_f16(a, b, f32x4{0.f, 0.f, 0.f, 0.f}, 0, 0, 0);
    if (threadIdx.x == 0) out[0] = d.x;
}

int c3d_subnormals_ok(alq_ctx *ctx) {
    if (ctx->f16_subnormal_mfma >= 0) return ctx->f16_subnormal_mfma;
    float *d = nullptr, h = -1.f;
    if (hipMalloc(&d, sizeof(float)) != hipSuccess) { (void)hipGetLastError(); return 0; }
    hipLaunchKernelGGL(c3d_subnormal_probe, dim3(1), dim3(64), 0, ctx->stream, d);
    const bool ok = hipGetLastError() == hipSuccess &&
                    hipMemcpyAsync(&h, d, sizeof(float), hipMemcpyDeviceToHost, ctx->stream) == hipSuccess &&
                    hipStreamSynchronize(ctx->stream) == hipSuccess;
    (void)hipFree(d);
    if (!ok) { (void)hipGetLastError(); return 0; }
    ctx->f16_subnormal_mfma = (h == 0x1p-5f) ? 1 : 0;
    return ctx->f16_subnormal_mfma;
}

int c3d_fwd_build(const View &in, const View &out, const int k[3], const int lo[3], const int s[3], C3dPlan *plan) {
    plan->ok = false;
    if (getenv("ALQ_NO_C3D")) return ALQ_OK;
    if (!is_conv3_same(k, lo, s)) return ALQ_OK;
    if (!(in.D == 32 && in.H == 32 && in.W == 32 && out.D == 32 && out.H == 32 && out.W == 32)) return ALQ_OK;
    if (!(in.C == 16 && in.split == 8 && in.cs == 8 && in.c0 == 0 && out.C == 8)) return ALQ_OK;
    plan->D = in.D;
    plan->oneacc = getenv("ALQ_C3D_TWOACC") ? 0 : 1;
    plan->flops_per_patch = 2.0 * 27 * 16 * 8 * (double)in.vox();
    plan->ok = true;
    return ALQ_OK;
}

void c3d_fwd_pack(C3dPlan *plan, const std::vector<float> &Bmat) {
    plan->w_exp = f16_pair_exp(Bmat.data(), Bmat.size());
    plan->h_W.assign((size_t)18 * 2 * 64 * 8, 0);
    for (int dzi = 0; dzi < 3; ++dzi)
        for (int dyi = 0; dyi < 3; ++dyi)
            for (int s = 0; s < 2; ++s)
                for (int lane = 0; lane < 64; ++lane) {
                    const int i = lane & 15, kg = lane >> 4, v = i >> 3, co = i & 7, t = kg >> 1, p = kg & 1;
                    const int dxi = 2 * s + p - v;
                    const int ks = (dzi * 3 + dyi) * 2 + s;
                    for (int c = 0; c < 8; ++c) {
                        float w = 0.f;
                        if (dxi >= 0 && dxi <= 2) w = Bmat[((size_t)((dzi * 3 + dyi) * 3 + dxi) * 16 + 8 * t + c) * 8 + co];
                        f16_pair_split(w, plan->w_exp, plan->oneacc ? 0 : 11, &plan->h_W[((size_t)(ks * 2 + 0) * 64 + lane) * 8 + c],
                                       &plan->h_W[((size_t)(ks * 2 + 1) * 64 + lane) * 8 + c]);
                    }
                }
}

int c3d_fwd_launch(alq_ctx *ctx, const C3dPlan &plan, const View &in, const float *bias, int N, const unsigned *amaxA, const unsigned *amaxB,
                   const float *fc_W, float *fc_part, float *asum_part, unsigned char *fc_bits, float flip_tau) {
    ALQ_REQUIRE(plan.ok && plan.d_W, ALQ_EINVAL, "c3d: weights not set");
    ALQ_REQUIRE(in.split == 8 && in.cs == 8 && in.C == 16 && in.D == plan.D && in.H == 32 && in.W == 32 && plan.D == 32, ALQ_EINVAL, "c3d: input view mismatch");
    ALQ_REQUIRE(amaxA && amaxB && fc_W && fc_part && bias, ALQ_EINVAL, "c3d: missing argument");
    SWEEP_REQUIRE_PATCHES(N, "c3d");
    if (N <= 0) return ALQ_OK;
    C3FwdArgs a;
    a.inA = in.p; a.inB = in.p + in.delta; a.W = plan.d_W; a.bias = bias; a.amaxA = amaxA; a.amaxB = amaxB;
    a.fc_W = fc_W; a.fc_part = fc_part; a.asum_part = asum_part; a.fc_bits = fc_bits; a.N = N; a.D = plan.D; a.e_w = plan.w_exp;
    a.flip_tau = flip_tau; a.clk = nullptr;
    const unsigned grid = (unsigned)std::min(N, 256);
    ProfScope ps(ctx, PROF_IGEMM_F16, plan.flops_per_patch * N);
    auto go = [&](auto kfn) { return sweep_launch(ctx, kfn, grid, 256, C3_LDS, a); };
    if (fc_bits) return plan.oneacc ? go(c3d_fwd_kernel<true, true>) : go(c3d_fwd_kernel<true, false>);
    return plan.oneacc ? go(c3d_fwd_kernel<false, true>) : go(c3d_fwd_kernel<false, false>);
}

int c3d_bwd_build(const View &fwd_in, const View &fwd_out, const int k[3], const int lo[3], const int s[3], C3dPlan *plan) {
    C3dPlan f;
    ALQ_TRY(c3d_fwd_build(fwd_in, fwd_out, k, lo, s, &f));
    plan->ok = f.ok;
    plan->D = f.D;
    plan->oneacc = 1;
    plan->flops_per_patch = f.flops_per_patch;
    return ALQ_OK;
}

void c3d_bwd_pack(C3dPlan *plan, const std::vector<float> &Bmat) {
    plan->w_exp = f16_pair_exp(Bmat.data(), Bmat.size());
    plan->h_W.assign((size_t)9 * 2 * 64 * 8, 0);
    for (int dzi = 0; dzi < 3; ++dzi)
        for (int di = 0; di < 3; ++di)
            for (int lane = 0; lane < 64; ++lane) {
                const int ci = lane & 15, kg = lane >> 4;
                const int ks = dzi * 3 + di;
                for (int c = 0; c < 8; ++c) {
                    float w = 0.f;
                    if (kg < 3) w = Bmat[((size_t)(((2 - dzi) * 3 + (2 - di)) * 3 + (2 - kg)) * 16 + ci) * 8 + c];
                    f16_pair_split(w, plan->w_exp, 0, &plan->h_W[((size_t)(ks * 2 + 0) * 64 + lane) * 8 + c], &plan->h_W[((size_t)(ks * 2 + 1) * 64 + lane) * 8 + c]);
                }
            }
}

void c3d_bwd7_pack(C3dPlan *plan, const std::vector<float> &Bmat) {
    plan->h_W7.assign((size_t)7 * 2 * 64 * 8, 0);
    for (int f = 0; f < 7; ++f)
        for (int lane = 0; lane < 64; ++lane) {
            const int ci = lane & 15, q = lane >> 4;
            int dz = -1, dy = 0, dx = 0;
            if (f < 3) { dz = f; if (q < 3) { dy = 0; dx = q; } else { dy = 1; dx = 0; } }
            else if (f < 6) { dz = f - 3; const int p = 4 + q; dy = p / 3; dx = p % 3; }
            else if (q < 3) { dz = q; dy = 2; dx = 2; }
            for (int c = 0; c < 8; ++c) {
                float w = 0.f;
                if (dz >= 0) w = Bmat[((size_t)(((2 - dz) * 3 + (2 - dy)) * 3 + (2 - dx)) * 16 + ci) * 8 + c];
                f16_pair_split(w, plan->w_exp, 0, &plan->h_W7[((size_t)(f * 2 + 0) * 64 + lane) * 8 + c], &plan->h_W7[((size_t)(f * 2 + 1) * 64 + lane) * 8 + c]);
            }
        }
}

void c3d_presplit_vec(const float *v, long long F, int e, std::vector<unsigned short> *out) {
    out->assign((size_t)F * 2, 0);
    for (long long vox = 0; vox < F / 8; ++vox)
        for (int c = 0; c < 8; ++c) f16_pair_split(v[vox * 8 + c], e, 0, &(*out)[(size_t)vox * 16 + c], &(*out)[(size_t)vox * 16 + 8 + c]);
}

int c3d_bwd_launch(alq_ctx *ctx, const C3dPlan &plan, int N, const unsigned char *bits, const void *vec16, int e_in, const unsigned char *maskA,
                   float *dB, float *sumA, float *sumB, int rows_per_wave, int waves_per_simd, int *grid_out) {
    ALQ_REQUIRE(plan.ok && plan.d_W && plan.D == 32, ALQ_EINVAL, "c3d: backward weights not set");
    ALQ_REQUIRE(bits && vec16 && dB && sumA && sumB, ALQ_EINVAL, "c3d: missing argument");
    SWEEP_REQUIRE_PATCHES(N, "c3d");
    if (grid_out) *grid_out = 0;
    if (N <= 0) return ALQ_OK;
    C3BwdArgs a;
    a.bits = bits; a.vec = vec16; a.W = plan.d_W; a.maskA = maskA; a.dB = dB; a.sumA = sumA; a.sumB = sumB;
    a.N = N; a.D = plan.D; a.e_in = e_in; a.e_w = plan.w_exp;
    ProfScope ps(ctx, PROF_IGEMM_F16, plan.flops_per_patch * N);
    const int rows8 = rows_per_wave == 4 ? 0 : 1;
    if (rows_per_wave == 7 && plan.d_W7) {
        a.W = plan.d_W7;
        unsigned g = (unsigned)std::min(N, 256);
        if (g_dbg_knobs[KNOB_C3B7_GRID_CAP] > 0) g = std::min<unsigned>(g, (unsigned)g_dbg_knobs[KNOB_C3B7_GRID_CAP]);
        if (grid_out) *grid_out = (int)g;
        if (waves_per_simd == 2) return sweep_launch(ctx, c3d_bwd7_kernel<4, 8>, g, 512, P7_LDS + P7_WS, a);
        return sweep_launch(ctx, c3d_bwd7_kernel<8, 4>, g, 256, P7_LDS, a);
    }
    if (grid_out) *grid_out = rows8 ? std::min(N, 256) : std::min(2 * N, 256);
    if (rows8) return sweep_launch(ctx, c3d_bwd_kernel<true, 8>, (unsigned)std::min(N, 256), 256, 2 * (32 + 2) * B3_ROW + 2 * B3_ROW, a);
    return sweep_launch(ctx, c3d_bwd_kernel<true, 4>, (unsigned)std::min(2 * N, 256), 256, 2 * (16 + 2) * B3_ROW + 2 * B3_ROW, a);
}

}
```

### nn-active-learning_amd/csrc/engine_switches.h

```cpp
#ifndef ALQ_ENGINE_SWITCHES_H
#define ALQ_ENGINE_SWITCHES_H
#include <cstddef>
#include <cstdlib>

namespace alq {

enum Knob {
    KNOB_REPEAT = 0,
    KNOB_FLAGS = 1,
    KNOB_NO_BWD_FUSE = 2,
    KNOB_NO_FWD_FUSE = 3,
    KNOB_NO_V3 = 4,
    KNOB_NO_V4 = 5,
    KNOB_NO_POOL_FIRST = 6,
    KNOB_NO_CONV_POOL = 7,
    KNOB_DCP_NARROW = 8,
    KNOB_E3D_GRID_CAP = 9,
    KNOB_C3B7_GRID_CAP = 10,
    ALQ_NKNOBS = 11
};

struct EngineSwitches {
    int knobs[ALQ_NKNOBS] = {0, 0, 0, 0, 0, 0, 0, 0, 0, 0, 0};
    int disable_v2 = 0;
    int disable_v3 = 0;
    int disable_v4 = 0;
    int no_fcgemm = 0;
    int no_split = 0;
    int no_wide2d_rule = 0;
    int no_v3_f16 = 0;
    int no_v3_f16_fwd = 0;
    int no_co_split = 0;
    int no_co_split_f16 = 0;
    int no_class_tiles = 0;
    int no_fc_bits = 0;
    int no_fc_fuse = 0;
    int no_fc_f16 = 0;
    int no_fc_f16_fwd = 0;
    int f16_derived_mask = 0;
    int has_f16_derived_mask = 0;
    int no_f16x2 = 0;
    int no_xcd_order = 0;
    int no_fixed = 0;
    int no_bound16 = 0;
    int no_flipfix = 0;
    int no_presplit = 0;
    int no_signs = 0;
    int no_signs0 = 0;
    int f16_fwd_mask = -1;
    int no_f16_derived = 0;
    int no_light_kernels = 0;
    int no_c3d = 0;
    int c3_bwd_rows = 7;
    int c3_bwd_waves = 2;
    int no_e3d = 0;
    int e3d_rows = 0;
    int no_d3d = 0;
    int no_d3b = 0;
    int no_f3d = 0;
    int no_t3d = 0;
};

enum SwitchRule {
    SW_PRESENT,
    SW_FIRST_IS_1,
    SW_ATOI_EQ,
    SW_INT,
    SW_ROWS
};

struct SwitchRow {
    const char *env;
    size_t member;
    SwitchRule rule;
    int arg;
};

#define ALQ_SW(env, member, rule, arg) {env, offsetof(EngineSwitches, member), rule, arg}
inline const SwitchRow kSwitchTable[] = {
    ALQ_SW("ALQ_DEBUG_REPEAT", knobs[KNOB_REPEAT], SW_INT, 0),
    ALQ_SW("ALQ_DEBUG_FLAGS", knobs[KNOB_FLAGS], SW_INT, 0),
    ALQ_SW("ALQ_NO_BWD_FUSE", knobs[KNOB_NO_BWD_FUSE], SW_INT, 0),
    ALQ_SW("ALQ_NO_FWD_FUSE", knobs[KNOB_NO_FWD_FUSE], SW_INT, 0),
    ALQ_SW("ALQ_NO_V3", knobs[KNOB_NO_V3], SW_INT, 0),
    ALQ_SW("ALQ_NO_V4", knobs[KNOB_NO_V4], SW_INT, 0),
    ALQ_SW("ALQ_NO_POOL_FIRST", knobs[KNOB_NO_POOL_FIRST], SW_INT, 0),
    ALQ_SW("ALQ_NO_CONV_POOL", knobs[KNOB_NO_CONV_POOL], SW_INT, 0),
    ALQ_SW("ALQ_DCP_NARROW", knobs[KNOB_DCP_NARROW], SW_INT, 0),
    ALQ_SW("ALQ_E3D_GRID_CAP", knobs[KNOB_E3D_GRID_CAP], SW_INT, 0),
    ALQ_SW("ALQ_DISABLE_V2", disable_v2, SW_FIRST_IS_1, 0),
    ALQ_SW("ALQ_DISABLE_V3", disable_v3, SW_FIRST_IS_1, 0),
    ALQ_SW("ALQ_DISABLE_V4", disable_v4, SW_PRESENT, 0),
    ALQ_SW("ALQ_NO_FCGEMM", no_fcgemm, SW_PRESENT, 0),
    ALQ_SW("ALQ_NO_SPLIT", no_split, SW_PRESENT, 0),
    ALQ_SW("ALQ_NO_WIDE2D_RULE", no_wide2d_rule, SW_PRESENT, 0),
    ALQ_SW("ALQ_NO_V3_F16", no_v3_f16, SW_PRESENT, 0),
    ALQ_SW("ALQ_NO_V3_F16_FWD", no_v3_f16_fwd, SW_PRESENT, 0),
    ALQ_SW("ALQ_NO_CO_SPLIT", no_co_split, SW_PRESENT, 0),
    ALQ_SW("ALQ_NO_CO_SPLIT_F16", no_co_split_f16, SW_PRESENT, 0),
    ALQ_SW("ALQ_NO_CLASS_TILES", no_class_tiles, SW_PRESENT, 0),
    ALQ_SW("ALQ_NO_FC_BITS", no_fc_bits, SW_PRESENT, 0),
    ALQ_SW("ALQ_NO_FC_FUSE", no_fc_fuse, SW_PRESENT, 0),
    ALQ_SW("ALQ_NO_FC_F16", no_fc_f16, SW_PRESENT, 0),
    ALQ_SW("ALQ_NO_FC_F16_FWD", no_fc_f16_fwd, SW_PRESENT, 0),
    ALQ_SW("ALQ_F16_DERIVED_MASK", f16_derived_mask, SW_INT, 0),
    ALQ_SW("ALQ_F16_DERIVED_MASK", has_f16_derived_mask, SW_PRESENT, 0),
    ALQ_SW("ALQ_NO_F16X2", no_f16x2, SW_PRESENT, 0),
    ALQ_SW("ALQ_NO_XCD_ORDER", no_xcd_order, SW_PRESENT, 0),
    ALQ_SW("ALQ_NO_FIXED", no_fixed, SW_PRESENT, 0),
    ALQ_SW("ALQ_NO_BOUND16", no_bound16, SW_PRESENT, 0),
    ALQ_SW("ALQ_NO_FLIPFIX", no_flipfix, SW_PRESENT, 0),
    ALQ_SW("ALQ_NO_PRESPLIT", no_presplit, SW_PRESENT, 0),
    ALQ_SW("ALQ_NO_SIGNS", no_signs, SW_PRESENT, 0),
    ALQ_SW("ALQ_NO_SIGNS0", no_signs0, SW_PRESENT, 0),
    ALQ_SW("ALQ_F16_FWD_MASK", f16_fwd_mask, SW_INT, 0),
    ALQ_SW("ALQ_F16_DERIVED", no_f16_derived, SW_ATOI_EQ, 0),
    ALQ_SW("ALQ_NO_F16_DERIVED", no_f16_derived, SW_ATOI_EQ, 1),
    ALQ_SW("ALQ_NO_LIGHT_KERNELS", no_light_kernels, SW_PRESENT, 0),
    ALQ_SW("ALQ_NO_C3D", no_c3d, SW_PRESENT, 0),
    ALQ_SW("ALQ_C3D_BWD_ROWS", c3_bwd_rows, SW_ROWS, 0),
    ALQ_SW("ALQ_NO_E3D", no_e3d, SW_PRESENT, 0),
    ALQ_SW("ALQ_E3D_ROWS", e3d_rows, SW_ATOI_EQ, 1),
    ALQ_SW("ALQ_NO_D3D", no_d3d, SW_PRESENT, 0),
    ALQ_SW("ALQ_NO_D3D_BWD", no_d3b, SW_PRESENT, 0),
    ALQ_SW("ALQ_NO_F3D", no_f3d, SW_PRESENT, 0),
    ALQ_SW("ALQ_NO_T3D", no_t3d, SW_PRESENT, 0),
};
#undef ALQ_SW
inline const int kNumSwitchRows = (int)(sizeof(kSwitchTable) / sizeof(kSwitchTable[0]));

inline int &switch_member(EngineSwitches &sw, const SwitchRow &row) {
    return *reinterpret_cast<int *>(reinterpret_cast<char *>(&sw) + row.member);
}

inline EngineSwitches read_engine_switches() {
    EngineSwitches sw;
    for (const SwitchRow &row : kSwitchTable) {
        const char *v = std::getenv(row.env);
        int &dst = switch_member(sw, row);
        switch (row.rule) {
            case SW_PRESENT:    if (v) dst = 1; break;
            case SW_FIRST_IS_1: if (v && v[0] == '1') dst = 1; break;
            case SW_ATOI_EQ:    if (v && std::atoi(v) == row.arg) dst = 1; break;
            case SW_INT:        if (v) dst = std::atoi(v); break;
            case SW_ROWS:       dst = (v && std::atoi(v) == 4) ? 4 : ((v && std::atoi(v) == 8) ? 8 : 7); break;
        }
    }
    if (const char *v = std::getenv("ALQ_C3D_BWD_WAVES")) sw.c3_bwd_waves = std::atoi(v) == 1 ? 1 : 2;
    return sw;
}

}
#endif
```

### nn-active-learning_amd/csrc/igemm2.hip

```cpp
#include "alq_internal.h"

#include <algorithm>
#include <cmath>
#include <cstring>

namespace alq {

typedef float f32x4 __attribute__((ext_vector_type(4)));
typedef float f32x2 __attribute__((ext_vector_type(2)));

#ifdef ALQ_STAMPS
#define STAMP(var) asm volatile("s_memtime %0\n\ts_waitcnt lgkmcnt(0)" : "=s"(var)::"memory")
#define PHASE_END(idx)                         \
    do {                                       \
        unsigned long long t_now_;             \
        STAMP(t_now_);                         \
        ph[idx] += t_now_ - t_last;            \
        t_last = t_now_;                       \
    } while (0)
#else
#define PHASE_END(idx) do {} while (0)
#endif

constexpr int I2_CBP = 12;
// ... 331 lines not shown
                        mm(a1, b1);
                        __builtin_amdgcn_sched_barrier(0);
                    }
                }
            }
            PHASE_END(6);
        }
        have_pend = true;
        p_out = c_out; p_cls = c_cls; p_l = c_l; p_g = c_g;
        more = next_more;
    }
    if (have_pend) flush();
#ifdef ALQ_STAMPS
    PHASE_END(7);
    if (a.dbg && tid == 0)
        for (int i = 0; i < 8; ++i) a.dbg[blockIdx.x * 8 + i] = ph[i];
#endif
}

int igemm2_build_plan(const IgemmPlan &p1, Igemm2Plan *p2) {
    p2->ok = false;
    const IgemmArgs &a1 = p1.a;
    if (p1.smallc || p1.CB != 8 || a1.NB != 1 || p1.NTW > 3 || a1.ntaps > 27 || a1.Co % 4) return ALQ_OK;
    const int halo = a1.HZ * a1.HY * a1.HX;
    const int nhv = a1.PT * halo;
    if (nhv * 2 > 256 * I2_MAXSLOT) return ALQ_OK;
    if (a1.HZ > 255 || a1.HY > 255 || a1.HX > 255 || a1.PT > 127) return ALQ_OK;
    const size_t wchunk = (size_t)a1.ntaps * p1.NTW * 128 * 4;
    size_t wres_max = I2_WRES_MAX;
    if (const char *e = getenv("ALQ_WRES_KB")) wres_max = (size_t)atoi(e) * 1024;
    const bool wres = wchunk * a1.nchunks <= wres_max * p1.NTW;
    const size_t wbytes = wres ? wchunk * a1.nchunks : wchunk;
    const size_t lds = wbytes + (size_t)nhv * I2_CBP * 4;
    if (lds > 156 * 1024) return ALQ_OK;
    Igemm2Args &a = p2->a;
    std::memset(&a, 0, sizeof(a));
    a.Ci = a1.Ci; a.ID = a1.ID; a.IH = a1.IH; a.IW = a1.IW;
    a.Co = a1.Co; a.OD = a1.OD; a.OH = a1.OH; a.OW = a1.OW;
    a.MD = a1.MD; a.MH = a1.MH; a.MW = a1.MW;
    a.sm = a1.sm; a.so = a1.so; a.ooffz = a1.ooffz; a.ooffy = a1.ooffy; a.ooffx = a1.ooffx;
    a.PT = a1.PT; a.TZ = a1.TZ; a.TY = a1.TY; a.TX = a1.TX; a.HZ = a1.HZ; a.HY = a1.HY; a.HX = a1.HX;
    a.rows = a1.rows; a.minz = a1.minz; a.miny = a1.miny; a.minx = a1.minx;
    a.ntaps = a1.ntaps; a.nchunks = a1.nchunks;
    a.tilesZ = a1.tilesZ; a.tilesY = a1.tilesY; a.tilesX = a1.tilesX;
    {
        std::vector<int> off(a1.ntaps);
        for (int t = 0; t < a1.ntaps; ++t) off[t] = a1.tapoff[t] / 10 * I2_CBP;
        bool found = false;
        for (int nx = 1; nx <= a1.ntaps && !found; ++nx) {
            if (a1.ntaps % nx) continue;
            for (int ny = 1; nx * ny <= a1.ntaps && !found; ++ny) {
                if ((a1.ntaps / nx) % ny) continue;
                const int nz = a1.ntaps / (nx * ny);
                const int sx = nx > 1 ? off[1] - off[0] : 0;
                const int sy = ny > 1 ? off[nx] - off[0] : 0;
                const int sz = nz > 1 ? off[nx * ny] - off[0] : 0;
                bool okb = true;
                for (int t = 0; t < a1.ntaps && okb; ++t) {
                    const int ix = t % nx, iy = (t / nx) % ny, iz = t / (nx * ny);
                    okb = off[t] == off[0] + iz * sz + iy * sy + ix * sx;
                }
                if (okb) {
                    a.t0 = off[0]; a.tsx = sx; a.tsy = sy; a.tsz = sz; a.tnx = nx; a.tny = ny;
                    found = true;
                }
            }
        }
        if (!found) return ALQ_OK;
    }
    a.split = 1 << 30;
    {
        const int dimsI[3] = {a.ID, a.IH, a.IW}, dimsM[3] = {a.MD, a.MH, a.MW};
        const int T[3] = {a.TZ, a.TY, a.TX}, tiles[3] = {a.tilesZ, a.tilesY, a.tilesX};
        const int mins[3] = {a.minz, a.miny, a.minx}, H[3] = {a.HZ, a.HY, a.HX};
        auto cls_of = [&](int d, int t) { return (t == 0 ? 1 : 0) | (t == tiles[d] - 1 ? 2 : 0); };
        auto valid1 = [&](int d, int t, int h) {
            const int c = t * T[d] * a.sm + mins[d] + h;
            return c >= 0 && c < dimsI[d];
        };
        for (int d = 0; d < 3; ++d)
            for (int t = 1; t + 1 < tiles[d]; ++t)
                for (int h = 0; h < H[d]; ++h)
                    if (!valid1(d, t, h)) return ALQ_OK;
        a.tpg = a.tilesZ * a.tilesY * a.tilesX;
        a.in_pstride = a.PT * a.ID * a.IH * a.IW;
        a.out_pstride = a.PT * a.OD * a.OH * a.OW;
        p2->h_tdesc.assign((size_t)a.tpg * 8, 0);
        for (int tz = 0; tz < a.tilesZ; ++tz)
            for (int ty = 0; ty < a.tilesY; ++ty)
                for (int tx = 0; tx < a.tilesX; ++tx) {
                    int *td = &p2->h_tdesc[(((size_t)tz * a.tilesY + ty) * a.tilesX + tx) * 8];
                    const int mz0 = tz * a.TZ, my0 = ty * a.TY, mx0 = tx * a.TX;
                    const int z0 = mz0 * a.sm + a.minz, y0 = my0 * a.sm + a.miny, x0 = mx0 * a.sm + a.minx;
                    td[0] = (z0 * a.IH + y0) * a.IW + x0;
                    td[1] = ((mz0 * a.so + a.ooffz) * a.OH + my0 * a.so + a.ooffy) * a.OW + mx0 * a.so + a.ooffx;
                    const int cls = cls_of(0, tz) | (cls_of(1, ty) << 2) | (cls_of(2, tx) << 4);
                    const bool full = a.rows == 256 && mz0 + a.TZ <= a.MD && my0 + a.TY <= a.MH && mx0 + a.TX <= a.MW;
                    td[2] = cls | (full ? 256 : 0);
                    td[3] = mz0; td[4] = my0; td[5] = mx0;
                }
        (void)dimsM;
        auto rep = [&](int d, int c) { return (c & 1) ? 0 : ((c & 2) ? tiles[d] - 1 : (tiles[d] > 2 ? 1 : 0)); };
        p2->h_sdesc.assign((size_t)nhv * 4, 0);
        for (int pt = 0; pt < a.PT; ++pt)
            for (int hz = 0; hz < a.HZ; ++hz)
                for (int hy = 0; hy < a.HY; ++hy)
                    for (int hx = 0; hx < a.HX; ++hx) {
                        const int hv = ((pt * a.HZ + hz) * a.HY + hy) * a.HX + hx;
                        int *sd = &p2->h_sdesc[(size_t)hv * 4];
                        sd[0] = ((pt * a.ID + hz) * a.IH + hy) * a.IW + hx;
                        unsigned long long m = 0;
                        for (int c = 0; c < 64; ++c) {
                            const int cz = c & 3, cy = (c >> 2) & 3, cx = (c >> 4) & 3;
                            if (valid1(0, rep(0, cz), hz) && valid1(1, rep(1, cy), hy) && valid1(2, rep(2, cx), hx))
                                m |= 1ull << c;
                        }
                        sd[1] = (int)(unsigned)(m & 0xffffffffull);
                        sd[2] = (int)(unsigned)(m >> 32);
                        sd[3] = (pt << 24) | (hz << 16) | (hy << 8) | hx;
                    }
    }
    p2->NTW = p1.NTW;
    p2->wres = wres;
    p2->lds_bytes = lds;
    int max_wgs = 2;
    if (const char *e = getenv("ALQ_MAX_WGS")) max_wgs = atoi(e);
    p2->wgs_per_cu = std::max<int>(1, std::min<int>(max_wgs, (int)((160 * 1024) / (lds + 512))));
    p2->flops_per_patch = p1.flops_per_patch;
    p2->ok = true;
    return ALQ_OK;
}

void igemm2_pack_weights(Igemm2Plan *p2, const std::vector<float> &Bmat) {
    const Igemm2Args &a = p2->a;
    const int NTW = p2->NTW, Ci = a.Ci, Co = a.Co;
    p2->h_W.assign((size_t)a.nchunks * a.ntaps * NTW * 128, 0.f);
    for (int ch = 0; ch < a.nchunks; ++ch)
        for (int tp = 0; tp < a.ntaps; ++tp)
            for (int nt = 0; nt < NTW; ++nt)
                for (int lane = 0; lane < 64; ++lane)
                    for (int s = 0; s < 2; ++s) {
                        const int c = ch * 8 + 2 * (lane >> 4) + s;
                        const int co = nt * 16 + (lane & 15);
                        if (co < Co)
                            p2->h_W[((((size_t)ch * a.ntaps + tp) * NTW + nt) * 64 + lane) * 2 + s] =
                                Bmat[((size_t)tp * Ci + c) * Co + co];
                    }
}

unsigned long long *g_igemm2_dbg = nullptr;
int g_no_f16x2 = 0;
int g_no_xcd_order = 0;
int g_no_fixed = 0;
int g_dbg_knobs[ALQ_NKNOBS] = {0, 0, 0, 0, 0, 0, 0, 0, 0, 0, 0};

template <int NTW, bool WRES, int GEO, bool SUMS>
static int launch2_s(alq_ctx *ctx, const Igemm2Plan &plan, const Igemm2Args &a, unsigned grid) {
    auto kfn = igemm2_kernel<NTW, WRES, GEO, SUMS>;
    if (plan.lds_bytes > 64 * 1024)
        ALQ_HIP(hipFuncSetAttribute(reinterpret_cast<const void *>(kfn), hipFuncAttributeMaxDynamicSharedMemorySize,
                                    (int)plan.lds_bytes));
    hipLaunchKernelGGL(kfn, dim3(grid), dim3(256), plan.lds_bytes, ctx->stream, a);
    ALQ_HIP(hipGetLastError());
    return ALQ_OK;
}

template <int NTW, bool WRES, int GEO>
static int launch2_t(alq_ctx *ctx, const Igemm2Plan &plan, const Igemm2Args &a, unsigned grid) {
    return (a.osumA || a.osumB) ? launch2_s<NTW, WRES, GEO, true>(ctx, plan, a, grid)
                                : launch2_s<NTW, WRES, GEO, false>(ctx, plan, a, grid);
}

int igemm2_launch(alq_ctx *ctx, const Igemm2Plan &plan, const View &in, const View &out, const float *bias, int relu,
                  int accumulate, int N, int prof_cls, const Igemm2Fuse *fuse) {
    Igemm2Args a = plan.a;
    ALQ_REQUIRE(in.C == a.Ci && in.D == a.ID && in.H == a.IH && in.W == a.IW, ALQ_EINVAL,
                "igemm2: input view does not match plan");
    ALQ_REQUIRE(out.C == a.Co && out.D == a.OD && out.H == a.OH && out.W == a.OW, ALQ_EINVAL,
                "igemm2: output view does not match plan");
    ALQ_REQUIRE(plan.d_W != nullptr, ALQ_EINVAL, "igemm2: weights not set");
    ALQ_REQUIRE((long long)N * in.vox() * in.cs < (1LL << 29) && (long long)N * out.vox() * out.cs < (1LL << 29),
                ALQ_EUNSUPPORTED, "igemm2: tensor exceeds the 32-bit byte-offset range (lower the batch)");
    ALQ_REQUIRE(in.cs % 4 == 0 && in.c0 % 4 == 0 && out.cs % 4 == 0 && out.c0 % 4 == 0, ALQ_EUNSUPPORTED,
                "igemm2: channel slice not 16-byte aligned");
    if (fuse) ALQ_REQUIRE(fuse->split % 4 == 0 && fuse->mask_cs % 4 == 0 && fuse->mask_c0 % 4 == 0 && fuse->mask_from % 4 == 0, ALQ_EUNSUPPORTED,
                          "igemm2: fused epilogue needs 4-channel aligned slices");
    a.in = in.p; a.in_cs = in.cs; a.in_c0 = in.c0;
    a.out = out.p; a.out_cs = out.cs; a.out_c0 = out.c0;
    a.W = plan.d_W; a.bias = bias; a.relu = relu; a.accumulate = accumulate; a.N = N;
    a.in_bytes = (int)((long long)N * in.vox() * in.cs * 4);
    a.dbg = nullptr;
    if (g_igemm2_dbg) {
        static int want = -2;
        if (want == -2) { const char *e = getenv("ALQ_STAMP_ONLY"); want = e ? atoi(e) : -1; }
        static int ordinal = 0;
        static unsigned long long *last = nullptr;
        if (last != g_igemm2_dbg) { last = g_igemm2_dbg; ordinal = 0; }
        if (want < 0 || ordinal == want) a.dbg = g_igemm2_dbg;
        ++ordinal;
    }
    a.dbg_repeat = g_dbg_knobs[KNOB_REPEAT];
    a.dbg_flags = g_dbg_knobs[KNOB_FLAGS];
    if (fuse) {
        a.mask = fuse->mask; a.mask_cs = fuse->mask_cs; a.mask_c0 = fuse->mask_c0; a.mask_from = fuse->mask_from;
        a.osumA = fuse->osumA; a.osumB = fuse->osumB;
        a.split = fuse->split > 0 ? fuse->split : (1 << 30);
    }
    const int pgroups = (N + a.PT - 1) / a.PT;
    const long long total = (long long)pgroups * a.tilesZ * a.tilesY * a.tilesX;
    const unsigned grid = (unsigned)std::min<long long>(total, 256LL * plan.wgs_per_cu);
    ProfScope ps(ctx, prof_cls, plan.flops_per_patch * N);
    int geo = 0;
    if (a.ntaps == 27 && a.tnx == 3 && a.tny == 3 && a.HY == 6 && a.HX == 18) {
        const int SX = I2_CBP, SY = 18 * I2_CBP, SZ = 6 * 18 * I2_CBP;
        if (a.t0 == 0 && a.tsx == SX && a.tsy == SY && a.tsz == SZ) geo = 1;
        if (a.t0 == 2 * (SX + SY + SZ) && a.tsx == -SX && a.tsy == -SY && a.tsz == -SZ) geo = 2;
    }
#define ALQ_L2(NT)                                                                                       \
    case NT:                                                                                             \
        if (geo == 1) return plan.wres ? launch2_t<NT, true, 1>(ctx, plan, a, grid) : launch2_t<NT, false, 1>(ctx, plan, a, grid); \
        if (geo == 2) return plan.wres ? launch2_t<NT, true, 2>(ctx, plan, a, grid) : launch2_t<NT, false, 2>(ctx, plan, a, grid); \
        return plan.wres ? launch2_t<NT, true, 0>(ctx, plan, a, grid) : launch2_t<NT, false, 0>(ctx, plan, a, grid)
    switch (plan.NTW) { ALQ_L2(1); ALQ_L2(2); ALQ_L2(3); }
#undef ALQ_L2
    set_error("igemm2: NTW=%d unsupported", plan.NTW);
    return ALQ_EUNSUPPORTED;
}

}
```

### nn-active-learning_amd/csrc/model.hip

```cpp
#include <algorithm>
#include <cstring>
#include <string>

#include "model_types.h"

using namespace alq;

static int g_knob_override[ALQ_NKNOBS] = {-1, -1, -1, -1, -1, -1, -1, -1, -1, -1, -1};

static void apply_knobs(const alq_model *m) {
    for (int k = 0; k < ALQ_NKNOBS; ++k) g_dbg_knobs[k] = g_knob_override[k] >= 0 ? g_knob_override[k] : m->sw.knobs[k];
    g_no_f16x2 = m->sw.no_f16x2;
    g_no_xcd_order = m->sw.no_xcd_order;
    g_no_fixed = m->sw.no_fixed;
}

static int gemm_build(const EngineSwitches &sw, const ConvDesc &d, int max_batch, Gemm *g, const G4Geom *g4 = nullptr) {
    ALQ_TRY(igemm_build_plan(d, max_batch, &g->p1));
    if (g4 && !sw.disable_v4) {
        G4Geom gg = *g4;
        gg.flops_per_patch = g->p1.flops_per_patch;
        ALQ_TRY(igemm4_build_plan(gg, max_batch, &g->p4));
    }
    ALQ_TRY(igemm2_build_plan(g->p1, &g->p2));
    ALQ_TRY(direct_build_plan(g->p1, &g->pd));
    if (sw.disable_v2) { g->p2.ok = false; g->pd.ok = false; }
    ALQ_TRY(igemm3_build_plan(g->p2, &g->p3));
    if (d.ID == 1 && d.IH == 1 && d.IW == 1 && d.tz.size() == 1 && d.sm == 1 && d.so == 1 && !sw.no_fcgemm)
        ALQ_TRY(fcgemm_build_plan(d.Ci, d.Co, &g->pfc));
    if (sw.disable_v3) g->p3.ok = false;
    return ALQ_OK;
}

int prepare_call(alq_model *m, bool fisher) {
    m->last.call_fisher = fisher;
    apply_knobs(m);
    if (!two_slot_allowed()) ALQ_TRY(refresh_fallback_forms(m));
    return ALQ_OK;
}

GemmRoute gemm_route(const Gemm &g, const View &in, const View &out, int accumulate, const Igemm2Fuse *fuse) {
    if (g.pd.ok && !accumulate && !(fuse && (fuse->mask || fuse->osumB || fuse->split))) return ROUTE_DIRECT;
    if (g.pfc.ok && !accumulate && !fuse && two_slot_allowed()) return ROUTE_FCGEMM;
    const bool split_view = in.split != 0 || out.split != 0;
    if (g.p4.ok && (two_slot_allowed() || split_view)) return ROUTE_IGEMM4;
    if (g.p3.ok && !g_dbg_knobs[KNOB_NO_V3]) return ROUTE_IGEMM3;
    return g.p2.ok ? ROUTE_IGEMM2 : ROUTE_IGEMM;
}

int gemm_launch(alq_ctx *ctx, const Gemm &g, const View &in, const View &out, const float *bias, int relu,
                int accumulate, int N, int cls, const Igemm2Fuse *fuse, bool *fused, float fc_in_bound) {
    const GemmRoute route = gemm_route(g, in, out, accumulate, fuse);
    ALQ_REQUIRE(route <= ROUTE_FCGEMM || g.p4.ok || (in.split == 0 && out.split == 0), ALQ_EUNSUPPORTED, "split concat view without a two-slot plan");
    if (fused) *fused = fuse != nullptr && route != ROUTE_FCGEMM && route != ROUTE_IGEMM;
    const int cls3 = cls == PROF_IGEMM_BWD ? PROF_IGEMM3_BWD : PROF_IGEMM3_FWD;
    switch (route) {
        case ROUTE_DIRECT: return direct_launch(ctx, g.pd, in, out, bias, relu, N, fuse ? fuse->osumA : nullptr, PROF_DIRECT);
        case ROUTE_FCGEMM:
            return fcgemm_launch(ctx, g.pfc, in, out, bias, relu, N, cls3, (g_no_f16x2 || bias || relu) ? 0.f : fc_in_bound,
                                 (cls == PROF_IGEMM_FWD && !g_no_f16x2) ? g.fc_row_amax : nullptr);
        case ROUTE_IGEMM4: return igemm4_launch(ctx, g.p4, in, out, bias, relu, accumulate, N, cls3, fuse);
        case ROUTE_IGEMM3: return igemm3_launch(ctx, g.p2, g.p3, in, out, bias, relu, accumulate, N, cls3, fuse);
        case ROUTE_IGEMM2: return igemm2_launch(ctx, g.p2, in, out, bias, relu, accumulate, N, cls, fuse);
        case ROUTE_IGEMM: break;
    }
    return igemm_launch(ctx, g.p1, in, out, bias, relu, accumulate, N, cls);
}

static View mkview(float *p, const Shp &s, int cs, int c0, int C) {
    View v; v.p = p; v.D = s.D; v.H = s.H; v.W = s.W; v.cs = cs; v.c0 = c0; v.C = C; return v;
}

struct ActViews { std::vector<View> act, dact, catv, dcatv; };

static int alloc_activations(alq_model *m, const ModelShape &ms, ActViews *av) {
    const EngineSwitches &sw = m->sw;
    const int n_layers = (int)ms.layers.size(), NB = m->max_batch;
    std::vector<View> &act = av->act, &dact = av->dact, &catv = av->catv, &dcatv = av->dcatv;
    act.resize(n_layers); dact.resize(n_layers); catv.resize(n_layers); dcatv.resize(n_layers);
    for (int d = 0; d < n_layers; ++d) {
        if (ms.src_of[d] < 0) continue;
        const int s = ms.src_of[d];
        const LayerShape &dl = ms.layers[d];
        const alq_layer_t &dsp = m->layers[d].spec;
        const Shp &sh = ms.layers[s].out;
        const int Cs = sh.C, Cp = ms.layers[d - 1].out.C;
        float *buf, *dbuf;
        const size_t el = (size_t)NB * sh.D * sh.H * sh.W * (Cs + Cp);
        ALQ_TRY(m->dalloc(&buf, el));
        ALQ_TRY(m->dalloc(&dbuf, el));
        unsigned char *sbuf = nullptr;
        if (Cs % 4 == 0 && Cp % 4 == 0) ALQ_TRY(m->dalloc(&sbuf, el / 4));
        bool split_ok = false;
        if (Cs == Cp && Cs % 8 == 0 && dsp.type == ALQ_CONV && !sw.disable_v4 && !sw.no_split) {
            Igemm4Plan tf, tb;
            ALQ_TRY(igemm4_build_plan(conv_fwd_geom(dl.in, dl.out, dsp, dl.lo), NB, &tf));
            ALQ_TRY(igemm4_build_plan(conv_bwd_geom(dl.in, dl.out, dsp, dl.lo), NB, &tb));
            split_ok = tf.ok && tb.ok && !tb.a.pair;
        }
        m->layers[s].out_is_skip_src = true;
        if (split_ok) {
            const long long half = (long long)NB * sh.D * sh.H * sh.W * Cs;
            act[s] = mkview(buf, sh, Cs, 0, Cs);
            act[d - 1] = mkview(buf + half, sh, Cp, 0, Cp);
            dact[s] = mkview(dbuf, sh, Cs, 0, Cs);
            dact[d - 1] = mkview(dbuf + half, sh, Cp, 0, Cp);
            catv[d] = mkview(buf, sh, Cs, 0, Cs + Cp);
            catv[d].split = Cs; catv[d].delta = half;
            if (sbuf) { act[s].sg = sbuf; act[d - 1].sg = sbuf + half / 4; catv[d].sg = sbuf; }
            dcatv[d] = mkview(dbuf, sh, Cs, 0, Cs + Cp);
            dcatv[d].split = Cs; dcatv[d].delta = half;
            continue;
        }
        act[s] = mkview(buf, sh, Cs + Cp, 0, Cs);
        act[d - 1] = mkview(buf, sh, Cs + Cp, Cs, Cp);
        dact[s] = mkview(dbuf, sh, Cs + Cp, 0, Cs);
        dact[d - 1] = mkview(dbuf, sh, Cs + Cp, Cs, Cp);
        catv[d] = mkview(buf, sh, Cs + Cp, 0, Cs + Cp);
        dcatv[d] = mkview(dbuf, sh, Cs + Cp, 0, Cs + Cp);
        if (sbuf) { act[s].sg = sbuf; act[d - 1].sg = sbuf; catv[d].sg = sbuf; }
    }
    for (int i = 0; i < n_layers; ++i) {
        if (act[i].p) continue;
        const Shp &sh = ms.layers[i].out;
        const alq_layer_t &sp = m->layers[i].spec;
        float *buf, *dbuf;
        const size_t el = (size_t)NB * sh.D * sh.H * sh.W * sh.C;
        ALQ_TRY(m->dalloc(&buf, el));
        ALQ_TRY(m->dalloc(&dbuf, el));
        act[i] = mkview(buf, sh, sh.C, 0, sh.C);
        dact[i] = mkview(dbuf, sh, sh.C, 0, sh.C);
        if (sh.C % 4 == 0 && sp.type != ALQ_FC && (sp.type == ALQ_POOL || sp.relu)) ALQ_TRY(m->dalloc(&act[i].sg, el / 4));
    }
    m->logits = act[n_layers - 1].p;
    m->dlogits = dact[n_layers - 1].p;
    ALQ_TRY(m->dalloc(&m->post, (size_t)NB * m->nclass * m->V));
    ALQ_TRY(m->dalloc(&m->S, (size_t)NB * m->L));
    ALQ_TRY(m->dalloc(&m->sizes, (size_t)m->L));
    ALQ_TRY(m->dalloc(&m->Apart, (size_t)((NB + 63) / 64) * m->L * m->L));
    return ALQ_OK;
}

static int plan_conv(alq_model *m, const LayerShape &ls, Layer &ly) {
    const EngineSwitches &sw = m->sw;
    const int NB = m->max_batch;
    const alq_layer_t &sp = ly.spec;
    const bool first_param = (ly.pidx == 0);
    const ConvDesc d = conv_fwd_desc(ls.in, ls.out, sp, ly.lo);
    const G4Geom g4 = conv_fwd_geom(ls.in, ls.out, sp, ly.lo);
    ly.fwd.resize(1);
    ALQ_TRY(gemm_build(sw, d, NB, &ly.fwd[0], &g4));
    if (ly.fwd[0].p4.ok && ly.fwd[0].p3.ok && d.ID == 1 && d.tz.size() >= 25 && !sw.no_wide2d_rule) ly.fwd[0].p4.ok = false;
    if (!ly.fwd[0].p4.ok && !ly.fwd[0].pd.ok && !ly.fwd[0].pfc.ok && ly.fwd[0].p3.ok && ly.fwd[0].p2.a.PT == 1 && sp.skip_src < 0 &&
        !sw.no_v3_f16_fwd && !sw.no_v3_f16) {
        ly.fwd[0].p3_f16 = true;
        m->v3_fwd_f16 = true;
    }
    if (!ly.fwd[0].p4.ok && !ly.fwd[0].p3.ok && !ly.fwd[0].pd.ok && sp.cout > 32 && !sw.no_co_split) {
        for (int w : {32, 48, 16}) {
            if (sp.cout % w || sp.cout <= w) continue;
            std::vector<Gemm> parts(sp.cout / w);
// ... 368 lines not shown
    ALQ_TRY(k_softmax(m->ctx, m->logits, m->nclass, N, m->post, nullptr));
    ALQ_TRY(run_backward(m, d_x, N));
    int nblocks = 0;
    ALQ_TRY(k_fisher_finalize(m->ctx, m->Spart, m->nslab, m->nslab_max, m->max_batch, m->S, m->L, m->sizes, m->post,
                              d_p1_in, N, diag_load, d_p1_out, d_g0, d_g1, d_A, d_trace, m->Apart, &nblocks));
    if (d_Asum) ALQ_TRY(k_reduce_Asum(m->ctx, m->Apart, nblocks, m->L * m->L, d_Asum));
    return ALQ_OK;
}

static int stage_rows(alq_model *m, const float *d_pool, const int64_t *d_rows, int N) {
    ALQ_REQUIRE(d_pool && d_rows, ALQ_EINVAL, "null pool / row list");
    if (!m->x_stage) ALQ_TRY(m->dalloc(&m->x_stage, (size_t)m->max_batch * m->epp));
    return gather_rows_impl(m->ctx, d_pool, d_rows, N, m->epp, m->x_stage);
}

int alq_forward_rows(alq_model *m, const float *d_pool, const int64_t *d_rows, int N, float *d_post, int64_t *d_pred,
                     float *d_feat, int feature_layer_idx) {
    ALQ_REFUSE_DENSE(m, "alq_forward_rows");
    ALQ_REQUIRE(m != nullptr, ALQ_EINVAL, "alq_forward_rows: null model");
    ALQ_REQUIRE(N >= 0 && N <= m->max_batch, ALQ_EINVAL, "alq_forward_rows: N=%d exceeds max_batch=%d", N, m->max_batch);
    if (N == 0) return ALQ_OK;
    ALQ_HIP(hipSetDevice(m->ctx->device));
    ALQ_TRY(stage_rows(m, d_pool, d_rows, N));
    return alq_forward(m, m->x_stage, N, d_post, d_pred, d_feat, feature_layer_idx);
}

int alq_fisher_rows(alq_model *m, const float *d_pool, const int64_t *d_rows, int N, const float *d_p1_in, double diag_load,
                    float *d_p1_out, double *d_g0, double *d_g1, double *d_A, double *d_trace, double *d_Asum) {
    ALQ_REFUSE_DENSE(m, "alq_fisher_rows");
    ALQ_REQUIRE(m != nullptr, ALQ_EINVAL, "alq_fisher_rows: null model");
    ALQ_REQUIRE(N >= 0 && N <= m->max_batch, ALQ_EINVAL, "alq_fisher_rows: N=%d exceeds max_batch=%d", N, m->max_batch);
    ALQ_HIP(hipSetDevice(m->ctx->device));
    if (N > 0) ALQ_TRY(stage_rows(m, d_pool, d_rows, N));
    return alq_fisher(m, N > 0 ? m->x_stage : d_pool, N, d_p1_in, diag_load, d_p1_out, d_g0, d_g1, d_A, d_trace, d_Asum);
}

int alq_model_debug_copy(alq_model *m, int layer_idx, int what, int N, float *d_out, int64_t *elems_out) {
    ALQ_REQUIRE(m && d_out && N >= 1 && N <= m->max_batch, ALQ_EINVAL, "alq_model_debug_copy: bad argument");
    ALQ_HIP(hipSetDevice(m->ctx->device));
    if (what == 4) {
        if (elems_out) *elems_out = (int64_t)N * m->L;
        return debug_f64_copy(m->ctx, m->S, (long long)N * m->L, d_out);
    }
    if (what == 5) {
        const Layer &head = m->layers.back();
        ALQ_REQUIRE(head.fc_part2 && m->last.fwd.head_fused, ALQ_EUNSUPPORTED, "the last pass did not run the fused fc head");
        const int ns = m->last.fwd.c3 ? 4 : head.fc_slices2;
        if (elems_out) *elems_out = (int64_t)N * ns;
        ALQ_HIP(hipMemcpyAsync(d_out, m->last.fwd.c3 ? head.c3_part : head.fc_part2, (size_t)N * ns * sizeof(float), hipMemcpyDeviceToDevice,
                               m->ctx->stream));
        return ALQ_OK;
    }
    ALQ_REQUIRE(layer_idx >= 0 && layer_idx < (int)m->layers.size(), ALQ_EINVAL, "bad layer index");
    const Layer &ly = m->layers[layer_idx];
    if (what >= 6 && what <= 10) {
        ALQ_REQUIRE(ly.spec.type == ALQ_FC && ly.fwd.size() == 1 && ly.fwd[0].pfc.ok && ly.weights_set, ALQ_EUNSUPPORTED, "layer %d has no streaming-GEMM weights", layer_idx);
        if (what == 10) {
            int32_t wd[4] = {ly.fwd[0].pfc.w_exp, ly.bwd.pfc.w_exp, 0, 0};
            std::memcpy(&wd[2], &ly.bwd_l1, 8);
            if (elems_out) *elems_out = 4;
            ALQ_HIP(hipMemcpyAsync(d_out, wd, 16, hipMemcpyHostToDevice, m->ctx->stream));
            ALQ_HIP(hipStreamSynchronize(m->ctx->stream));
            return ALQ_OK;
        }
        const FcGemmPlan &pl = what <= 7 ? ly.fwd[0].pfc : ly.bwd.pfc;
        const void *src = (what & 1) ? pl.d_W16 : pl.d_W;
        ALQ_REQUIRE(pl.ok && src, ALQ_EUNSUPPORTED, "layer %d: this form is not packed", layer_idx);
        const int64_t e = (int64_t)pl.K * pl.N * ((what & 1) ? 2 : 3) / 2;
        if (elems_out) *elems_out = e;
        ALQ_HIP(hipMemcpyAsync(d_out, src, (size_t)e * 4, hipMemcpyDeviceToDevice, m->ctx->stream));
        return ALQ_OK;
    }
    if (what >= 11 && what <= 13) {
        if (what == 11) {
            ALQ_REQUIRE(ly.osum && m->last.call_fisher, ALQ_EUNSUPPORTED, "layer %d: no channel sums of its output in the last pass", layer_idx);
            if (elems_out) *elems_out = (int64_t)N * ly.out.vox();
            ALQ_HIP(hipMemcpyAsync(d_out, ly.osum, (size_t)N * ly.out.vox() * sizeof(float), hipMemcpyDeviceToDevice, m->ctx->stream));
            return ALQ_OK;
        }
        if (what == 12) {
            const View &v = ly.out;
            ALQ_REQUIRE(v.sg && m->last.fwd.signs_ready[layer_idx] && ((v.C | v.cs | v.c0) & 3) == 0 && ((int64_t)N * v.vox() * v.cs) % 16 == 0, ALQ_EUNSUPPORTED,
                        "layer %d: no sign field of its output in the last pass", layer_idx);
            if (elems_out) *elems_out = (int64_t)N * v.vox() * v.cs / 16;
            ALQ_HIP(hipMemcpyAsync(d_out, v.sg, (size_t)N * v.vox() * v.cs / 4, hipMemcpyDeviceToDevice, m->ctx->stream));
            return ALQ_OK;
        }
        ALQ_REQUIRE(ly.spec.type == ALQ_POOL && ly.argmax && ((int64_t)N * ly.out.vox() * ly.out.C) % 4 == 0, ALQ_EUNSUPPORTED, "layer %d has no arg-max field", layer_idx);
        if (elems_out) *elems_out = (int64_t)N * ly.out.vox() * ly.out.C / 4;
        ALQ_HIP(hipMemcpyAsync(d_out, ly.argmax, (size_t)N * ly.out.vox() * ly.out.C, hipMemcpyDeviceToDevice, m->ctx->stream));
        return ALQ_OK;
    }
    if (what == 14) {
        ALQ_REQUIRE(ly.spec.type == ALQ_FC && ly.fc_maskbits && m->last.call_fisher && ((int64_t)N * ly.F) % 16 == 0, ALQ_EUNSUPPORTED,
                    "layer %d: no sign bytes of its input in the last pass", layer_idx);
        if (elems_out) *elems_out = (int64_t)N * ly.F / 16;
        ALQ_HIP(hipMemcpyAsync(d_out, ly.fc_maskbits, (size_t)N * ly.F / 4, hipMemcpyDeviceToDevice, m->ctx->stream));
        return ALQ_OK;
    }
    if (what == 0 || what == 1) {
        const Layer &head = m->layers.back();
        ALQ_REQUIRE(!(layer_idx + 2 == (int)m->layers.size() && head.spec.type == ALQ_FC &&
                      (what == 0 ? m->last.fwd.head_fused
                                 : (m->last.call_fisher && head.fc_maskbits != nullptr && two_slot_allowed()))),
                    ALQ_EUNSUPPORTED, "layer %d: this tensor is not materialised in a Fisher pass (fc head fused into the layer: "
                    "create the model under ALQ_NO_FC_BITS=1 to keep it)", layer_idx);
        const View &v = what == 0 ? ly.out : ly.dout;
        if (elems_out) *elems_out = (int64_t)N * v.elems();
        return debug_view_copy(m->ctx, v, N, d_out);
    }
    ALQ_REQUIRE(ly.pidx >= 0 && !ly.dense_head && (what == 2 || what == 3), ALQ_EINVAL, "layer has no channel-sum fields");
    const bool isfc = ly.spec.type == ALQ_FC;
    const int64_t e = (int64_t)N * (isfc ? 1 : (what == 2 ? ly.in.vox() : ly.out.vox()));
    if (elems_out) *elems_out = e;
    ALQ_HIP(hipMemcpyAsync(d_out, what == 2 ? ly.asum : ly.dsum, e * sizeof(float), hipMemcpyDeviceToDevice,
                           m->ctx->stream));
    return ALQ_OK;
}

int alq_model_engine_info(alq_model *m, int what) {
    ALQ_REQUIRE(m, ALQ_EINVAL, "alq_model_engine_info: bad argument");
    switch (what) {
        case ALQ_INFO_SUBNORMALS_OK:
            ALQ_HIP(hipSetDevice(m->ctx->device));
            return c3d_subnormals_ok(m->ctx);
        case ALQ_INFO_C3D_FWD: return m->last.fwd.c3 ? 1 : 0;
        case ALQ_INFO_C3D_BWD: return m->last.bwd.c3_bwd ? 1 : 0;
        case ALQ_INFO_C3D_ONE_ACC:
            for (const Layer &ly : m->layers)
                if (ly.c3f.ok) return ly.c3f.oneacc;
            return 0;
        case ALQ_INFO_FLIP_OVERFLOW: {
            ALQ_HIP(hipSetDevice(m->ctx->device));
            if (!m->flip_overflow) return 0;
            unsigned h = 0;
            ALQ_HIP(hipMemcpyAsync(&h, m->flip_overflow, sizeof(unsigned), hipMemcpyDeviceToHost, m->ctx->stream));
            ALQ_HIP(hipStreamSynchronize(m->ctx->stream));
            return h > 0x7fffffffu ? 0x7fffffff : (int)h;
        }
        case ALQ_INFO_F16_DERIVED: return m->last.fwd.f16_derived ? 1 : 0;
        case ALQ_INFO_T3D_FWD: return m->last.fwd.t3f;
        case ALQ_INFO_T3D_BWD: return m->last.bwd.t3b;
        case ALQ_INFO_E3D_BWD: return m->last.bwd.e3b;
        case ALQ_INFO_D3D_FWD: return m->last.fwd.d3f;
        case ALQ_INFO_D3D_BWD: return m->last.bwd.d3b;
        case ALQ_INFO_F3D_FWD: return m->last.fwd.f3f;
        case ALQ_INFO_C3D_BWD_FORM: return m->last.bwd.c3_bwd ? m->sw.c3_bwd_rows : 0;
        case ALQ_INFO_HOST_PACK_ELEMS: return m->host_pack_elems > 0x7fffffffll ? 0x7fffffff : (int)m->host_pack_elems;
        case ALQ_INFO_LSUM: return m->last.lsum;
        case ALQ_INFO_DCP_FORM: return m->last.fwd.dcp;
        case ALQ_INFO_E3D_BWD_FORM: return m->last.bwd.e3b_form;
        case ALQ_INFO_C3D_BWD_WAVES: return m->last.bwd.c3_bwd ? (m->sw.c3_bwd_rows == 7 ? m->sw.c3_bwd_waves : 1) : 0;
        case ALQ_INFO_C3D_BWD_GRID: return m->last.bwd.c3_bwd ? m->last.bwd.c3b_grid : 0;
        default: break;
    }
    set_error("alq_model_engine_info: bad argument");
    return ALQ_EINVAL;
}

int alq_debug_set(int key, int value) {
    ALQ_REQUIRE(key >= 0 && key < ALQ_NKNOBS, ALQ_EINVAL, "alq_debug_set: bad key");
    g_knob_override[key] = value > 0 ? value : -1;
    g_dbg_knobs[key] = value;
    return ALQ_OK;
}

int alq_debug_set_stamp_buffer(void *d_buf) {
    g_igemm2_dbg = reinterpret_cast<unsigned long long *>(d_buf);
    return ALQ_OK;
}

}
```

### nn-active-learning_amd/csrc/model_types.h

```cpp
#pragma once
#include <algorithm>

#include "alq_internal.h"

namespace alq {

struct Layer {
    alq_layer_t spec;
    int pidx = -1;
    View in, out;
    View din, dout;
    int lo[3] = {0, 0, 0};
    bool dense_fc_small = false;
    bool dense_head = false;
    int64_t F = 0;
    int64_t w_elems = 0, b_elems = 0;
    float *d_bias = nullptr;
    float *d_Wp = nullptr;
    std::vector<Gemm> fwd;
    std::vector<Gemm> fwd_co;
    int fwd_co_w = 0;
    Igemm4Plan fwd_all;
    Gemm bwd;
    bool has_bwd = false;
    bool weights_set = false;
    float *d_Wres = nullptr;
    bool fallback_stale = false;
    uint8_t *argmax = nullptr;
    float *asum = nullptr, *dsum = nullptr;
    double *ls_field = nullptr;
    float *osum = nullptr;
    float *fc_partials = nullptr;
    unsigned *fc_maskbits = nullptr;
    float *fc_wv = nullptr;
    unsigned *fc_wv16 = nullptr;
    float fc_wv_amax = 0.f;
    unsigned *amax_fwd = nullptr;
    double bwd_l1 = 0;
    float *d_W32 = nullptr;
    float fwd_l1 = 0.f;
    float out_l1 = 0.f, out_bmax = 0.f;
    unsigned *bound_fwd = nullptr;
    float *fc_part2 = nullptr;
    int fc_slices2 = 0;
    C3dPlan c3f, c3b;
    D3dPlan d3f;
    F3dPlan f3f;
    E3dPlan e3b;
    T3dPlan t3f, t3b;
    float *c3_part = nullptr, *c3_asum = nullptr;
    unsigned short *fc_wv16c = nullptr;
    int fc_slices = 0;
    bool out_is_skip_src = false;
    std::vector<std::vector<int>> class_taps;
    std::vector<float> hv_hW;
    int hv_src = 0;
    bool hv_stale = false;
    float *hv_W = nullptr;
    double *hv_A = nullptr, *hv_D = nullptr, *hv_Ra = nullptr, *hv_Rd = nullptr;
};

}

struct PassInfo {
    struct Fwd {
        bool head_fused = false;
        bool c3 = false;
        int t3f = 0;
        int d3f = 0;
        int f3f = 0;
        int dcp = 0;
        bool f16_derived = false;
        bool signs_ready[64] = {};
    } fwd;
    struct Bwd {
        bool c3_bwd = false;
        int c3b_grid = 0;
        int t3b = 0;
        int e3b = 0;
        int e3b_form = 0;
        int d3b = 0;
    } bwd;
    int lsum = 0;
    bool call_fisher = false;
};

struct alq_model {
    alq_ctx *ctx = nullptr;
    int max_batch = 0;
    alq::EngineSwitches sw;
    PassInfo last;
    unsigned *amax_a = nullptr, *amax_b = nullptr, *amax_tiles = nullptr;
    unsigned *flip_cnt = nullptr, *flip_list = nullptr;
    int flip_cap = 0;
    unsigned *bound_all = nullptr;
    unsigned *in_amax = nullptr;
    bool v3_fwd_f16 = false;
    unsigned *flip_overflow = nullptr;
    size_t amax_tiles_len = 0;
    int in_dims[4] = {1, 1, 1, 1};
    int nclass = 0;
    bool dense = false;
    int64_t V = 1;
    bool aleatoric = false;
    float *au = nullptr;
    double *dh_part = nullptr;
    int L = 0;
    std::vector<alq::Layer> layers;
    std::vector<void *> allocs;
    float *logits = nullptr, *dlogits = nullptr, *post = nullptr;
    double *S = nullptr, *sizes = nullptr, *Apart = nullptr;
    double *Spart = nullptr;
    int *nslab = nullptr;
    int nslab_max = 1;
    float *wg_partial = nullptr;
    size_t wg_partial_len = 0;
    double *gn_partial = nullptr;
    size_t gn_partial_len = 0;
    double *df_scratch = nullptr;
    double *ls_part = nullptr;
    std::vector<int> ls_nslab;
    int ls_nslab_max = 0;
    float *x_stage = nullptr;
    int64_t epp = 0;
    int f16_fwd_derived = 0;
    int64_t host_pack_elems = 0;
    void *d_wscal = nullptr;
    bool hv_ready = false;
    double *hv_part = nullptr;
    double *hv_p64 = nullptr;

    template <typename T>
    int dalloc(T **p, size_t count) {
        void *q = nullptr;
        const size_t bytes = std::max<size_t>(count * sizeof(T), 256);
        if (hipMalloc(&q, bytes) != hipSuccess) {
            alq::set_error("hipMalloc of %zu bytes failed", bytes);
            return ALQ_ENOMEM;
        }
        allocs.push_back(q);
        *p = reinterpret_cast<T *>(q);
        return ALQ_OK;
    }
};

template <typename T, typename D>
int ensure(alq_model *m, D **d, size_t count) {
    T *p = static_cast<T *>(*d);
    if (!p) ALQ_TRY(m->dalloc(&p, count));
    *d = p;
    return ALQ_OK;
}

template <typename T, typename D>
int upload(alq_model *m, D **d, const std::vector<T> &h) {
    ALQ_TRY(ensure<T>(m, d, h.size()));
    ALQ_HIP(hipMemcpyAsync(*d, h.data(), h.size() * sizeof(T), hipMemcpyHostToDevice, m->ctx->stream));
    return ALQ_OK;
}

template <typename T, typename D>
int upload_release(alq_model *m, D **d, std::vector<T> *h) {
    ALQ_TRY(upload(m, d, *h));
    ALQ_HIP(hipStreamSynchronize(m->ctx->stream));
    std::vector<T>().swap(*h);
    return ALQ_OK;
}

namespace alq { int refresh_fallback_forms(alq_model *m); }

struct DropSpec {
    unsigned long long layers = 0;
    float keep_prob = 1.f;
    unsigned long long seed = 0;
    long long first_sample = 0;
    bool on(int i) const { return keep_prob < 1.f && i < 64 && ((layers >> i) & 1ull); }
};
int make_drop(const alq_model *m, float keep_prob, uint64_t seed, int64_t first_sample, const int32_t *h_layers, int n_layers, DropSpec *d);
int prepare_call(alq_model *m, bool fisher);
int run_forward(alq_model *m, const float *d_x, int N, bool with_sums, bool keep_all = false, const DropSpec *drop = nullptr);
int run_backward(alq_model *m, const float *d_x, int N);
enum GemmRoute { ROUTE_DIRECT, ROUTE_FCGEMM, ROUTE_IGEMM4, ROUTE_IGEMM3, ROUTE_IGEMM2, ROUTE_IGEMM };
GemmRoute gemm_route(const alq::Gemm &g, const alq::View &in, const alq::View &out, int accumulate, const alq::Igemm2Fuse *fuse);
int gemm_launch(alq_ctx *ctx, const alq::Gemm &g, const alq::View &in, const alq::View &out, const float *bias, int relu, int accumulate, int N,
                int cls, const alq::Igemm2Fuse *fuse = nullptr, bool *fused = nullptr, float fc_in_bound = 0.f);
alq::View flat_view(const alq::View &v);

int dense_forward_head(alq_model *m, const float *d_x, int N, float *d_post, int64_t *d_pred, bool want_logits, float *d_au = nullptr,
                       float *d_logits = nullptr);
#define ALQ_REFUSE_ALEATORIC(m, who)                                                                                           \
    ALQ_REQUIRE(!(m) || !(m)->aleatoric, ALQ_EUNSUPPORTED,                                                                      \
                "%s: the model's head has a log-variance channel (alq_model_set_aleatoric): alq_param_grads_loss_mt_au", who)
#define ALQ_REFUSE_DENSE(m, who)                                                                                                \
    ALQ_REQUIRE(!(m) || !(m)->dense, ALQ_EUNSUPPORTED, "%s: not defined for a fully-convolutional model (1x1 conv head)", who)
```

### nn-active-learning_amd/csrc/passes.hip

```cpp
#include <algorithm>
#include <cmath>

#include "model_types.h"

using namespace alq;

static int ensure_bounds(alq_model *m) {
    if (m->bound_all) return ALQ_OK;
    const int nl = (int)m->layers.size();
    ALQ_TRY(m->dalloc(&m->bound_all, (size_t)nl * m->max_batch));
    for (int k = 0; k < nl; ++k) m->layers[k].bound_fwd = m->bound_all + (size_t)k * m->max_batch;
    return ALQ_OK;
}

static int ensure_amax_tiles(alq_model *m, size_t len) {
    if (len <= m->amax_tiles_len) return ALQ_OK;
    ALQ_TRY(m->dalloc(&m->amax_tiles, (size_t)m->max_batch * len));
    m->amax_tiles_len = len;
    return ALQ_OK;
}

static FwdBoundsArgs fwd_bounds_args(const alq_model *m) {
    const int nl = (int)m->layers.size();
    FwdBoundsArgs ba;
// ... 60 lines not shown
static bool d3d_fwd_applies(const FwdPass &P, int i, const Igemm2Fuse *fuse) {
    const alq_model *m = P.m;
    const Layer &ly = m->layers[i];
    return fuse && ly.d3f.ok && ly.d3f.d_Whi && !m->sw.no_d3d && fuse->in_amax && fuse->in_amax2 && !P.prod[i] && !g_no_f16x2 && two_slot_allowed() &&
           ((P.with_sums && fuse->osumA) || (P.light && !m->sw.no_light_kernels)) && ly.in.split == 16 && !(P.drop && P.drop->on(i));
}

static bool f3d_fwd_applies(const FwdPass &P, int i, const Igemm2Fuse *fuse) {
    const alq_model *m = P.m;
    const DropSpec *drop = P.drop;
    const Layer &ly = m->layers[i];
    const Layer *nx = i + 1 < (int)m->layers.size() ? &m->layers[i + 1] : nullptr;
    return fuse && ly.f3f.ok && ly.f3f.d_Whi && !m->sw.no_f3d && P.cons[i] == 2 && fuse->in_amax && !fuse->in_amax2 && !P.prod[i] && !g_no_f16x2 && two_slot_allowed() &&
           ((P.with_sums && fuse->osumA) || (P.light && !m->sw.no_light_kernels)) && ly.spec.relu && ly.in.split == 0 && !(drop && (drop->on(i) || drop->on(i + 1))) && nx && nx->spec.type == ALQ_POOL &&
           nx->spec.k[0] == 2 && nx->spec.k[1] == 2 && nx->spec.k[2] == 2 && nx->lo[0] == 0 && nx->lo[1] == 0 && nx->lo[2] == 0 && nx->out.D == 8 && nx->out.H == 8 &&
           nx->out.W == 8 && nx->out.C == 16 && nx->out.cs == 16 && nx->out.c0 == 0 && !nx->out.split && nx->argmax && !P.prod[i + 1];
}

static bool t3d_fwd_applies(const FwdPass &P, int i) {
    const alq_model *m = P.m;
    const Layer &ly = m->layers[i];
    return ly.t3f.ok && ly.t3f.d_W && !m->sw.no_t3d && !g_dbg_knobs[KNOB_NO_FWD_FUSE] && two_slot_allowed() && !P.cons[i] && !ly.spec.relu &&
           !(P.drop && P.drop->on(i)) && (!P.with_sums || ly.osum) && !(ly.t3f.kind == 8 && P.prod[i]);
}

static int plan_input_scales(FwdPass &P) {
    alq_model *m = P.m;
    const DropSpec *drop = P.drop;
    const int nl = (int)m->layers.size();
    const bool no16 = g_no_f16x2 != 0;
    std::vector<char> &prod = P.prod, &cons = P.cons;
    prod.assign(nl, 0);
    cons.assign(nl, 0);
    if ((P.with_sums || P.light) && !no16 && !g_dbg_knobs[KNOB_NO_FWD_FUSE] && two_slot_allowed()) {
        auto prod_ok = [&](int p) {
            if (p < 0) return false;
            const Layer &l = m->layers[p];
            if (p == 0 && P.dcp) return true;
            if (!l.osum) return false;
            if (l.spec.type == ALQ_CONV) return l.fwd[0].p4.ok && !l.fwd[0].pd.ok && !l.fwd[0].pfc.ok && l.fwd[0].p4.a.PT == 1;
            if (l.spec.type == ALQ_CONVT) return l.fwd_all.ok && l.fwd_all.a.PT == 1;
            return false;
        };
        size_t need = 0;
        for (int j = 1; j < nl; ++j) {
            const Layer &l = m->layers[j];
            if (l.dense_head) continue;
            const Igemm4Plan *pl = l.spec.type == ALQ_CONV ? &l.fwd[0].p4 : (l.spec.type == ALQ_CONVT ? &l.fwd_all : nullptr);
            if (!pl || !pl->ok || !pl->d_W16 || pl->multi || pl->a.PT != 1 || !l.osum) continue;
            if (l.spec.type == ALQ_CONV && (l.fwd[0].pd.ok || l.fwd[0].pfc.ok)) continue;
            const int s_ = l.spec.skip_src;
            if (m->sw.f16_fwd_mask < 0 && !m->sw.no_f16_derived && nl <= 16 && ((m->f16_fwd_derived >> j) & 1) && l.spec.type == ALQ_CONV && P.dcp &&
                (s_ >= 0) == (l.in.split != 0) && !(drop && drop->layers)) {
                cons[j] = 2;
                prod[0] = 1;
                continue;
            }
            if (!(j == nl - 2 && m->layers[nl - 1].fc_part2 && l.spec.type == ALQ_CONV) && m->sw.f16_fwd_mask < 0) continue;
            if (l.spec.type == ALQ_CONVT && !pl->fic) continue;
            if (!prod_ok(j - 1) || (s_ >= 0 && !prod_ok(s_))) continue;
            if ((s_ >= 0) != (l.in.split != 0)) continue;
            if (m->sw.f16_fwd_mask >= 0 && !((m->sw.f16_fwd_mask >> j) & 1)) continue;
            cons[j] = 1; prod[j - 1] = 1;
            if (s_ >= 0) prod[s_] = 1;
        }
        for (int p = 0; p < nl; ++p) {
            if (!prod[p]) continue;
            Layer &l = m->layers[p];
            if (!l.amax_fwd) ALQ_TRY(m->dalloc(&l.amax_fwd, (size_t)m->max_batch));
            if (l.spec.type == ALQ_CONV && !(p == 0 && P.dcp)) need = std::max(need, (size_t)l.fwd[0].p4.a.tpg * 4);
            if (l.spec.type == ALQ_CONVT) need = std::max(need, (size_t)l.fwd_all.a.tpg * (l.fwd_all.multi ? l.fwd_all.a.ngr : 1) * 4);
            if (l.spec.type == ALQ_CONVT && l.t3f.ok) need = std::max(need, (size_t)16);
        }
        ALQ_TRY(ensure_amax_tiles(m, need));
    }
    for (int j = 0; j < nl; ++j) P.any_derived = P.any_derived || cons[j] == 2;
    m->last.fwd.f16_derived = P.any_derived;
    if (P.any_derived) ALQ_TRY(ensure_bounds(m));
    P.v3f16 = m->v3_fwd_f16 && (P.with_sums || P.light) && !no16 && !drop && !P.any_derived && !P.dcp && nl <= 16 &&
              !g_dbg_knobs[KNOB_NO_FWD_FUSE] && two_slot_allowed() && m->layers[0].in.split == 0 && m->layers[0].in.cs == m->layers[0].in.C;
    if (P.v3f16) {
        if (!m->in_amax) ALQ_TRY(m->dalloc(&m->in_amax, (size_t)m->max_batch));
        ALQ_TRY(ensure_bounds(m));
        ALQ_TRY(k_rowmax_abs(m->ctx, P.d_x, P.N, (long long)m->layers[0].in.vox() * m->layers[0].in.C, m->in_amax));
        FwdBoundsArgs ba = fwd_bounds_args(m);
        ba.from_input = 1;
        ALQ_TRY(k_fwd_bounds(m->ctx, m->in_amax, P.N, m->max_batch, ba, m->bound_all));
    }
    return ALQ_OK;
}

static void fwd_take_amax(const FwdPass &P, Igemm2Fuse &fz, int j) {
    const alq_model *m = P.m;
    if (!P.cons[j]) return;
    const bool dv = P.cons[j] == 2;
    fz.in_amax = dv ? m->layers[j - 1].bound_fwd : m->layers[j - 1].amax_fwd;
    if (m->layers[j].spec.skip_src >= 0) {
        const Layer &sl = m->layers[m->layers[j].spec.skip_src];
        fz.in_amax2 = dv ? sl.bound_fwd : sl.amax_fwd;
    }
}


static int fwd_conv_pool(FwdPass &P, FwdStep &s, bool *took) {
    if (!(s.i == 0 && P.dcp)) return ALQ_OK;
    alq_model *m = P.m;
    alq_ctx *ctx = m->ctx;
    Layer &ly = m->layers[0], &nx = m->layers[1];
    const alq_layer_t &sp = ly.spec;
    const bool with_sums = P.with_sums;
    if (P.prod[0]) ALQ_HIP(hipMemsetAsync(ly.amax_fwd, 0, (size_t)P.N * sizeof(unsigned), ctx->stream));
    const bool sg_here = with_sums && !m->sw.no_signs && !m->sw.no_signs0 && sp.relu && ly.out.sg != nullptr;
    ALQ_TRY(direct_conv_pool_launch(ctx, ly.fwd[0].pd.d_W, s.in, ly.out, nx.out, ly.d_bias, sp.relu, nx.argmax,
                                    with_sums ? ly.osum : nullptr, with_sums ? nx.osum : nullptr, P.N,
                                    ly.fwd[0].pd.flops_per_patch, P.prod[0] ? ly.amax_fwd : nullptr,
                                    sg_here ? ly.out.sg : nullptr, (sg_here && nx.out.sg) ? nx.out.sg : nullptr));
    m->last.fwd.dcp = g_dcp_last_form;
    m->last.fwd.signs_ready[0] = sg_here;
    m->last.fwd.signs_ready[1] = sg_here && nx.out.sg != nullptr;
    if (P.any_derived)
        ALQ_TRY(k_fwd_bounds(ctx, ly.amax_fwd, P.N, m->max_batch, fwd_bounds_args(m), m->bound_all));
    s.fused = true;
    P.skip_next = true;
    *took = true;
    return ALQ_OK;
}

static int fwd_head_conv(FwdPass &P, FwdStep &s, bool *took) {
    alq_model *m = P.m;
    alq_ctx *ctx = m->ctx;
    const int nl = (int)m->layers.size(), i = s.i, N = P.N;
    if (!(s.fuse && i + 2 == nl && m->layers[nl - 1].fc_part2 && two_slot_allowed())) return ALQ_OK;
    Layer &ly = m->layers[i], &nx = m->layers[i + 1];
    const alq_layer_t &sp = ly.spec;
    const View &in = s.in;
    Igemm2Fuse &fz = s.fz;
    fz.fc_W = nx.fc_wv; fz.fc_F = nx.F; fz.fc_part = nx.fc_part2; fz.fc_bits = P.with_sums ? nx.fc_maskbits : nullptr;
    fwd_take_amax(P, fz, i);
    const bool flipfix = flipfix_applies(P, i, &fz);
    if (flipfix) {
        if (!m->flip_list) {
            m->flip_cap = flip_list_len(m->max_batch);
            ALQ_TRY(m->dalloc(&m->flip_cnt, (size_t)flip_segments(m->max_batch)));
            ALQ_TRY(m->dalloc(&m->flip_list, (size_t)m->flip_cap));
            ALQ_TRY(m->dalloc(&m->flip_overflow, (size_t)1));
            ALQ_HIP(hipMemsetAsync(m->flip_overflow, 0, sizeof(unsigned), ctx->stream));
        }
        fz.flip_cnt = m->flip_cnt; fz.flip_list = m->flip_list; fz.flip_cap = m->flip_cap; fz.flip_l1 = ly.fwd_l1; fz.flip_bias_nonzero = ly.out_bmax > 0.f;
    }
    P.c3_head = c3d_fwd_applies(P, i, &fz);
    if (P.c3_head)
        ALQ_TRY(c3d_fwd_launch(ctx, ly.c3f, in, ly.d_bias, N, fz.in_amax, fz.in_amax2, nx.fc_wv, nx.c3_part,
                               P.with_sums ? nx.c3_asum : nullptr, reinterpret_cast<unsigned char *>(fz.fc_bits),
                               flipfix ? std::ldexp(ly.fwd_l1, -24) : 0.f));
    else
        ALQ_TRY(igemm4_launch(ctx, ly.fwd[0].p4, in, ly.out, ly.d_bias, ly.spec.relu, 0, N, PROF_IGEMM3_FWD, &fz));
    if (flipfix)
        ALQ_TRY(k_flip_fix(ctx, m->flip_list, m->flip_cnt, m->flip_cap, N, in.p, in.split ? in.p + in.delta : nullptr,
                           in.split ? in.split : in.C, in.split ? in.C - in.split : 0, in.D, in.H, in.W, sp.k[0], sp.k[1], sp.k[2],
                           ly.lo[0], ly.lo[1], ly.lo[2], ly.d_W32, ly.d_bias, sp.cout,
                           reinterpret_cast<unsigned char *>(nx.fc_maskbits), nx.F, m->flip_overflow));
    s.fused = true;
    P.fc_head_fused = true;
    m->last.fwd.head_fused = true;
    m->last.fwd.c3 = P.c3_head;
    *took = true;
    return ALQ_OK;
}

static int fwd_conv_d3d(FwdPass &P, FwdStep &s, bool *took) {
    if (!d3d_fwd_applies(P, s.i, s.fuse)) return ALQ_OK;
    alq_model *m = P.m;
    Layer &ly = m->layers[s.i];
    const bool sgd = P.with_sums && !m->sw.no_signs && ly.spec.relu && ly.out.sg;
    ALQ_TRY(d3d_fwd_launch(m->ctx, ly.d3f, P.N, s.in.p, s.in.p + s.in.delta, s.fz.in_amax, s.fz.in_amax2, ly.d_bias, ly.spec.relu ? 1 : 0, ly.out.p,
                           sgd ? ly.out.sg : nullptr, s.fz.osumA));
    m->last.fwd.signs_ready[s.i] = sgd;
    m->last.fwd.d3f = 1;
    s.fused = true;
    *took = true;
    return ALQ_OK;
}

static int fwd_conv_f3d(FwdPass &P, FwdStep &s, bool *took) {
    if (!f3d_fwd_applies(P, s.i, s.fuse)) return ALQ_OK;
    alq_model *m = P.m;
    Layer &ly = m->layers[s.i], &nx = m->layers[s.i + 1];
    const bool sgd = P.with_sums && !m->sw.no_signs && ly.out.sg;
    ALQ_TRY(f3d_fwd_launch(m->ctx, ly.f3f, P.N, s.in.p, s.fz.in_amax, ly.d_bias, ly.out.p, sgd ? ly.out.sg : nullptr, s.fz.osumA, nx.out.p, nx.argmax,
                           P.with_sums ? nx.osum : nullptr));
    m->last.fwd.signs_ready[s.i] = sgd;
    m->last.fwd.f3f = 1;
    s.fused = true;
    P.skip_next = true;
    *took = true;
    return ALQ_OK;
}

static int fwd_conv_sliced(FwdPass &P, FwdStep &s, bool *took) {
    alq_model *m = P.m;
    const int i = s.i;
    Layer &ly = m->layers[i];
    if (!(!ly.fwd_co.empty() && !P.prod[i] && !P.cons[i] && two_slot_allowed())) return ALQ_OK;
    Igemm2Fuse sz;
    const bool s16 = P.v3f16 && i >= 1 && s.in.split == 0 && ly.spec.skip_src < 0 && !m->sw.no_co_split_f16;
    if (s16) sz.in_amax = m->layers[i - 1].bound_fwd;
    for (size_t j = 0; j < ly.fwd_co.size(); ++j) {
        View oj = ly.out;
        oj.c0 = ly.out.c0 + (int)j * ly.fwd_co_w;
        oj.C = ly.fwd_co_w;
        bool f1 = false;
        ALQ_TRY(gemm_launch(m->ctx, ly.fwd_co[j], s.in, oj, ly.d_bias + j * ly.fwd_co_w, ly.spec.relu, 0, P.N, PROF_IGEMM_FWD, s16 ? &sz : nullptr, &f1));
    }
    s.fused = false;
    *took = true;
    return ALQ_OK;
}

static int fwd_conv_gemm(FwdPass &P, FwdStep &s) {
    alq_model *m = P.m;
    const int i = s.i;
    Layer &ly = m->layers[i];
    const Igemm2Fuse *fuse = s.fuse;
    const bool sg_here = P.with_sums && fuse && !m->sw.no_signs && ly.spec.relu && ly.out.sg && gemm_route(ly.fwd[0], s.in, ly.out, 0, fuse) == ROUTE_IGEMM4;
    if (sg_here) s.fz.sign_out = ly.out.sg;
    Igemm2Fuse hz;
    const Igemm2Fuse *fu = fuse;
    if (P.v3f16 && !ly.fwd[0].p4.ok && !ly.fwd[0].pd.ok && !ly.fwd[0].pfc.ok && ly.fwd[0].p3.ok && ly.fwd[0].p3.d_W16 && ly.fwd[0].p2.a.PT == 1 &&
        s.in.split == 0 && ly.spec.skip_src < 0) {
        if (fuse) hz = *fuse;
        hz.in_amax = i == 0 ? m->in_amax : m->layers[i - 1].bound_fwd;
        hz.in_amax2 = nullptr;
        fu = &hz;
    }
    bool f2 = false;
    ALQ_TRY(gemm_launch(m->ctx, ly.fwd[0], s.in, ly.out, ly.d_bias, ly.spec.relu, 0, P.N, PROF_IGEMM_FWD, fu, &f2));
    s.fused = fuse ? f2 : false;
    m->last.fwd.signs_ready[i] = sg_here;
    if (fuse && P.prod[i]) ALQ_TRY(k_rowmax_u32(m->ctx, m->amax_tiles, ly.fwd[0].p4.a.tpg * 4, P.N, ly.amax_fwd));
    return ALQ_OK;
}

static int fwd_convt(FwdPass &P, FwdStep &s) {
    alq_model *m = P.m;
    alq_ctx *ctx = m->ctx;
    const int i = s.i, N = P.N;
    Layer &ly = m->layers[i];
    const Igemm2Fuse *fuse = s.fuse;
    if (t3d_fwd_applies(P, i)) {
        const bool want_amax = P.prod[i] != 0;
        ALQ_TRY(t3d_fwd_launch(ctx, ly.t3f, s.in, ly.out, ly.d_bias, N, P.with_sums ? ly.osum : nullptr, want_amax ? m->amax_tiles : nullptr));
        if (want_amax) ALQ_TRY(k_rowmax_u32(ctx, m->amax_tiles, 16, N, ly.amax_fwd));
        s.fused = true;
        m->last.fwd.t3f += 1;
        return ALQ_OK;
    }
    if (ly.fwd_all.ok && two_slot_allowed()) {
        const bool want_amax = fuse && P.prod[i];
        if (fuse) fwd_take_amax(P, s.fz, i);
        if (want_amax) s.fz.out_amax = m->amax_tiles;
        const bool sg_here = P.with_sums && fuse && !m->sw.no_signs && ly.spec.relu && ly.out.sg;
        if (sg_here) s.fz.sign_out = ly.out.sg;
        ALQ_TRY(igemm4_launch(ctx, ly.fwd_all, s.in, ly.out, ly.d_bias, ly.spec.relu, 0, N, PROF_IGEMM3_FWD, fuse));
        m->last.fwd.signs_ready[i] = sg_here;
        if (want_amax)
            ALQ_TRY(k_rowmax_u32(ctx, m->amax_tiles, ly.fwd_all.a.tpg * (ly.fwd_all.multi ? ly.fwd_all.a.ngr : 1) * 4, N, ly.amax_fwd));
        s.fused = fuse != nullptr;
        return ALQ_OK;
    }
    bool all = true;
    for (auto &p : ly.fwd) {
        bool f1 = false;
        ALQ_TRY(gemm_launch(ctx, p, s.in, ly.out, ly.d_bias, ly.spec.relu, 0, N, PROF_IGEMM_FWD, fuse, &f1));
        all = all && f1;
    }
    s.fused = all;
    return ALQ_OK;
}

static int fwd_fc(FwdPass &P, FwdStep &s) {
    alq_model *m = P.m;
    alq_ctx *ctx = m->ctx;
    const int i = s.i, N = P.N;
    Layer &ly = m->layers[i];
    if (P.with_sums) {
        const bool prev_spatial = i > 0 && m->layers[i - 1].osum != nullptr;
        if (P.c3_head) ALQ_TRY(k_rowsum_field(ctx, ly.c3_asum, 4, N, ly.asum));
        else if (prev_spatial) ALQ_TRY(k_rowsum_field(ctx, m->layers[i - 1].osum, m->layers[i - 1].out.vox(), N, ly.asum));
        else ALQ_TRY(k_chansum(ctx, flat_view(s.in), ly.asum, N));
    }
    if (ly.dense_fc_small && P.fc_head_fused) {
        ALQ_TRY(k_fc_small_finish_diff(ctx, P.c3_head ? ly.c3_part : ly.fc_part2, P.c3_head ? 4 : ly.fc_slices2, ly.d_bias, N, ly.out.p));
    } else if (ly.dense_fc_small) {
        ALQ_TRY(k_fc_small_fwd(ctx, s.in.p, ly.F, ly.d_Wp, ly.spec.cout, N, ly.fc_partials, ly.fc_slices,
                               P.with_sums ? ly.fc_maskbits : nullptr));
        ALQ_TRY(k_fc_small_finish(ctx, ly.fc_partials, ly.fc_slices, ly.d_bias, ly.spec.cout,
                                  ly.spec.relu, N, ly.out.p));
    } else {
        ALQ_TRY(gemm_launch(ctx, ly.fwd[0], flat_view(s.in), ly.out, ly.d_bias, ly.spec.relu, 0, N,
                            PROF_IGEMM_FWD));
    }
    return ALQ_OK;
}

int run_forward(alq_model *m, const float *d_x, int N, bool with_sums, bool keep_all, const DropSpec *drop) {
    alq_ctx *ctx = m->ctx;
    const int nl = (int)m->layers.size();
// ... 409 lines not shown
```

### nn-active-learning_amd/csrc/t3d.hip

```cpp
#include "f16_pair.h"
#include "sweep_common.h"
#ifndef T3_CLOBBER
#define T3_CLOBBER : "memory"
#endif

#include <algorithm>
#include <cmath>
#include <cstdlib>
#include <cstring>
#include <vector>

namespace alq {

struct T3FwdArgs {
    const float *in;
    float *out;
    const unsigned short *W;
    const float *bias;
    float *osum;
    unsigned *out_amax;
    int N;
};
struct T3BwdArgs {
    const float *dout;
// ... 97 lines not shown
        for (int k = 0; k < T3F_PF; ++k) {
            const int T = T0 + k;
            __builtin_amdgcn_sched_barrier(0);
            const T3Cur cur = t3_tile(live ? T : 0, total, wave);
            const int p = cur.p, iz = cur.iz, iy = cur.s;
            {
                auto split_row = [&](int base, const f32x4 &R) __attribute__((always_inline)) {
                    float x = R.x, y = R.y, z = R.z, w = R.w;
                    const unsigned h0 = t3_split2(x, y), h1 = t3_split2(z, w);
                    const unsigned m0 = t3_split2(x, y), m1 = t3_split2(z, w);
                    *reinterpret_cast<i32x2 *>(strip + (base + 0) * T3F_ROWB + w_off) = i32x2{(int)h0, (int)h1};
                    *reinterpret_cast<i32x2 *>(strip + (base + 1) * T3F_ROWB + w_off) = i32x2{(int)m0, (int)m1};
                    *reinterpret_cast<i32x2 *>(strip + (base + 2) * T3F_ROWB + w_off) = i32x2{(int)t3_pack2(x, y), (int)t3_pack2(z, w)};
                };
                split_row(0, R0[k]);
                split_row(3, R1[k]);
            }
            fetch(T + T3F_PF, R0[k], R1[k]);
            bf16x8 fn[2][3];
#pragma unroll
            for (int d = 0; d < 2; ++d)
#pragma unroll
                for (int pc = 0; pc < 3; ++pc)
                    fn[d][pc] = *reinterpret_cast<const bf16x8 *>(strip + (d * 3 + pc) * T3F_ROWB + f_off);
            if (k == 0) {
                const int keep = iy == 0 ? 0 : -1;
#pragma unroll
                for (int d = 0; d < 2; ++d)
#pragma unroll
                    for (int pc = 0; pc < 3; ++pc) {
                        i32x4 t = __builtin_bit_cast(i32x4, fo[d][pc]);
                        t.x &= keep; t.y &= keep; t.z &= keep; t.w &= keep;
                        fo[d][pc] = __builtin_bit_cast(bf16x8, t);
                    }
            }
            f32x4 acc[2][2];
#pragma unroll
            for (int i = 0; i < 2; ++i)
#pragma unroll
                for (int j = 0; j < 2; ++j) acc[i][j] = f32x4{0.f, 0.f, 0.f, 0.f};
#pragma unroll
            for (int cz = 0; cz < 3; ++cz)
#pragma unroll
                for (int cy = 0; cy < 3; ++cy) {
                    const int pz = cz == 2, dz = cz == 1, py = cy == 2, dy = cy == 1;
                    const bf16x8 *w = wr[cz * 3 + cy];
                    const bf16x8 *f = dy ? fo[dz] : fn[dz];
                    f32x4 c = acc[pz][py];
                    c = __builtin_amdgcn_mfma_f32_16x16x32_bf16(w[2], f[0], c, 0, 0, 0);
                    c = __builtin_amdgcn_mfma_f32_16x16x32_bf16(w[0], f[2], c, 0, 0, 0);
                    c = __builtin_amdgcn_mfma_f32_16x16x32_bf16(w[1], f[1], c, 0, 0, 0);
                    c = __builtin_amdgcn_mfma_f32_16x16x32_bf16(w[1], f[0], c, 0, 0, 0);
                    c = __builtin_amdgcn_mfma_f32_16x16x32_bf16(w[0], f[1], c, 0, 0, 0);
                    c = __builtin_amdgcn_mfma_f32_16x16x32_bf16(w[0], f[0], c, 0, 0, 0);
                    acc[pz][py] = c;
                }
#pragma unroll
            for (int d = 0; d < 2; ++d)
#pragma unroll
                for (int pc = 0; pc < 3; ++pc) fo[d][pc] = fn[d][pc];
            f32x4 vv[4];
#pragma unroll
            for (int i = 0; i < 4; ++i) {
                f32x4 v = acc[i >> 1][i & 1];
                v.x += bias4.x; v.y += bias4.y; v.z += bias4.z; v.w += bias4.w;
                vv[i] = v;
                if constexpr (AMAX)
                    amx = fmaxf(fmaxf(amx, fmaxf(__builtin_fabsf(v.x), __builtin_fabsf(v.y))), fmaxf(__builtin_fabsf(v.z), __builtin_fabsf(v.w)));
            }
#pragma unroll
            for (int i = 0; i < 4; ++i) {
                const int pz = i >> 1, py = i & 1;
                const f32x4 v = vv[i];
                const unsigned orow = ((unsigned)p * 32u + (unsigned)(2 * iz + pz)) * 32u + (unsigned)(2 * iy + py);
                __builtin_amdgcn_raw_buffer_store_b128(__builtin_bit_cast(i32x4, v), out_rsrc, (int)st_o, (int)(orow * 1024u), 0);
                if constexpr (SUMS) {
                    const float s = (v.x + v.y) + (v.z + v.w);
                    const float t = s + __shfl_xor(s, 16, 64);
                    __builtin_amdgcn_raw_buffer_store_b32(__builtin_bit_cast(int, t), sum_rsrc, (int)sm_o, (int)(orow * 128u), 0);
                }
            }
            if constexpr (AMAX) {
                if (k == T3F_PF - 1) {
                    float mx = amx;
#pragma unroll
                    for (int off = 32; off >= 1; off >>= 1) mx = fmaxf(mx, __shfl_xor(mx, off, 64));
                    const unsigned off = (live && iy == 15 && lane == 0) ? 0u : SW_OOB;
                    __builtin_amdgcn_raw_buffer_store_b32(__builtin_bit_cast(int, mx), amx_rsrc, (int)off, (int)((unsigned)(p * 16 + iz) * 4u), 0);
                    amx = iy == 15 ? 0.f : amx;
                }
            }
            __builtin_amdgcn_sched_barrier(0);
            asm volatile("s_nop 3" :: "v"(vv[0]), "v"(vv[1]), "v"(vv[2]), "v"(vv[3]) T3_CLOBBER);
        }
    }
}

constexpr int T3B_PF = 2;
template <bool MASK, bool SUMS>
__global__ __launch_bounds__(256, 2) void t3d_bwd_kernel(const T3BwdArgs a) {
    extern __shared__ __attribute__((aligned(16))) char t3lds[];
    const int lane = threadIdx.x & 63, wave = __builtin_amdgcn_readfirstlane((int)(threadIdx.x >> 6));
    char *strip = t3lds + wave * T3B_WAVE;
    if (lane < 24) {
        const int r = lane >> 1;
        *reinterpret_cast<i32x4 *>(strip + r * T3B_ROWB + (32 + (lane & 1)) * 16) = i32x4{0, 0, 0, 0};
    }
    const int n = lane & 15, kg = lane >> 4;
    const int w_off = (lane >> 1) * 16 + (lane & 1) * 8;
    const int f_off = (2 * n + kg) * 16;
    f16x8 wr[9][2];
#pragma unroll
    for (int c = 0; c < 9; ++c)
#pragma unroll
        for (int pc = 0; pc < 2; ++pc)
            wr[c][pc] = *reinterpret_cast<const f16x8 *>(a.W + ((size_t)(c * 2 + pc) * 64 + lane) * 8);
#pragma unroll
    for (int c = 0; c < 9; ++c)
#pragma unroll
        for (int pc = 0; pc < 2; ++pc) asm volatile("" : "+v"(wr[c][pc]));
    const __amdgpu_buffer_rsrc_t in_rsrc = sw_rsrc(a.dout, (unsigned long long)a.N * 32 * 32 * 32 * 8 * 4);
    const __amdgpu_buffer_rsrc_t out_rsrc = sw_rsrc(a.din, (unsigned long long)a.N * 16 * 16 * 16 * 16 * 4);
    const __amdgpu_buffer_rsrc_t sum_rsrc = sw_rsrc(a.dsum, SUMS ? (unsigned long long)a.N * 16 * 16 * 16 * 4 : 0ull);
    const __amdgpu_buffer_rsrc_t msk_rsrc = sw_rsrc(a.mask_bits, MASK ? (unsigned long long)a.N * 16 * 16 * 16 * 4 : 0ull);
    const unsigned ld_off = (unsigned)lane * 16u;
    const unsigned st_off = (unsigned)n * 64u + (unsigned)kg * 16u;
    const unsigned mk_off = (unsigned)n * 4u + (unsigned)kg;
    static_assert(T3B_PF == 2, "the sum store pairs the two tiles of a pass over the body");
    const unsigned sm_off = kg < 2 ? (unsigned)n * 4u + (unsigned)kg * 64u : SW_OOB;
    const float sc = a.scale;
    const int total = t3_total_tiles(a.N);

    auto stage = [&](int slot, const f32x4 &R) __attribute__((always_inline)) {
        const float x0 = R.x * sc, x1 = R.y * sc, x2 = R.z * sc, x3 = R.w * sc;
        const f16x2 h01 = __builtin_convertvector(f32x2{x0, x1}, f16x2), h23 = __builtin_convertvector(f32x2{x2, x3}, f16x2);
        const f16x2 l01 = __builtin_convertvector(f32x2{x0 - (float)h01.x, x1 - (float)h01.y}, f16x2);
        const f16x2 l23 = __builtin_convertvector(f32x2{x2 - (float)h23.x, x3 - (float)h23.y}, f16x2);
        *reinterpret_cast<i32x2 *>(strip + (2 * slot) * T3B_ROWB + w_off) = i32x2{__builtin_bit_cast(int, h01), __builtin_bit_cast(int, h23)};
        *reinterpret_cast<i32x2 *>(strip + (2 * slot + 1) * T3B_ROWB + w_off) = i32x2{__builtin_bit_cast(int, l01), __builtin_bit_cast(int, l23)};
    };
    f32x4 R[T3B_PF][6];
    unsigned MK[T3B_PF];
    auto fetch = [&](int T, f32x4 *r, unsigned &mk) __attribute__((always_inline)) {
        const T3Cur c = t3_tile(T, total, wave);
        const int iy = 15 - c.s;
        const unsigned b0 = (((unsigned)c.p * 32u + (unsigned)(2 * c.iz)) * 32u + (unsigned)(2 * iy)) * 1024u;
        const unsigned okl = c.ok ? ld_off : SW_OOB, ok2 = (c.ok && 2 * c.iz + 2 < 32) ? ld_off : SW_OOB;
#pragma unroll
        for (int tz = 0; tz < 3; ++tz)
#pragma unroll
            for (int ty = 0; ty < 2; ++ty)
                r[tz * 2 + ty] = __builtin_bit_cast(f32x4, __builtin_amdgcn_raw_buffer_load_b128(in_rsrc, (int)(tz < 2 ? okl : ok2),
                                                                                                 (int)(b0 + (unsigned)tz * 32768u + (unsigned)ty * 1024u), 0));
        if constexpr (MASK)
            mk = (unsigned)(unsigned char)__builtin_amdgcn_raw_buffer_load_b8(msk_rsrc, (int)(c.ok ? mk_off : SW_OOB),
                                                                             (int)((((unsigned)c.p * 16u + (unsigned)c.iz) * 16u + (unsigned)iy) * 64u), 0);
    };
#pragma unroll
    for (int k = 0; k < T3B_PF; ++k) {
        MK[k] = 0u;
#pragma unroll
        for (int s = 0; s < 6; ++s) R[k][s] = f32x4{0.f, 0.f, 0.f, 0.f};
    }

    f16x8 fo[3][2];
#pragma unroll
    for (int tz = 0; tz < 3; ++tz)
#pragma unroll
        for (int pc = 0; pc < 2; ++pc) fo[tz][pc] = f16x8{0, 0, 0, 0, 0, 0, 0, 0};
    static_assert(16 % T3B_PF == 0, "a sweep must start at k = 0");
    if (total > 0)
    for (int T0 = -T3B_PF; T0 < total; T0 += T3B_PF) {
        const bool live = T0 >= 0;
        const unsigned st_o = live ? st_off : SW_OOB, sm_o = live ? sm_off : SW_OOB;
        float s_odd = 0.f;
#pragma unroll
        for (int k = 0; k < T3B_PF; ++k) {
            const int T = T0 + k;
            __builtin_amdgcn_sched_barrier(0);
            const T3Cur cur = t3_tile(live ? T : 0, total, wave);
            const int p = cur.p, iz = cur.iz, iy = 15 - cur.s;
#pragma unroll
            for (int s = 0; s < 6; ++s) stage(s, R[k][s]);
            const unsigned nb = MK[k];
            fetch(T + T3B_PF, R[k], MK[k]);
            f16x8 fn[3][2][2];
#pragma unroll
            for (int tz = 0; tz < 3; ++tz)
#pragma unroll
                for (int ty = 0; ty < 2; ++ty)
#pragma unroll
                    for (int pc = 0; pc < 2; ++pc)
                        fn[tz][ty][pc] = *reinterpret_cast<const f16x8 *>(strip + ((2 * tz + ty) * 2 + pc) * T3B_ROWB + f_off);
            if (k == 0) {
                const int keep = cur.s == 0 ? 0 : -1;
#pragma unroll
                for (int tz = 0; tz < 3; ++tz)
#pragma unroll
                    for (int pc = 0; pc < 2; ++pc) {
                        i32x4 t = __builtin_bit_cast(i32x4, fo[tz][pc]);
                        t.x &= keep; t.y &= keep; t.z &= keep; t.w &= keep;
                        fo[tz][pc] = __builtin_bit_cast(f16x8, t);
                    }
            }
            f32x4 c = f32x4{0.f, 0.f, 0.f, 0.f};
#pragma unroll
            for (int tz = 0; tz < 3; ++tz)
#pragma unroll
                for (int ty = 0; ty < 3; ++ty) {
                    const f16x8 *w = wr[tz * 3 + ty];
                    const f16x8 *f = ty == 2 ? fo[tz] : fn[tz][ty];
                    c = __builtin_amdgcn_mfma_f32_16x16x32_f16(w[1], f[0], c, 0, 0, 0);
                    c = __builtin_amdgcn_mfma_f32_16x16x32_f16(w[0], f[1], c, 0, 0, 0);
                    c = __builtin_amdgcn_mfma_f32_16x16x32_f16(w[0], f[0], c, 0, 0, 0);
                }
#pragma unroll
            for (int tz = 0; tz < 3; ++tz)
#pragma unroll
                for (int pc = 0; pc < 2; ++pc) fo[tz][pc] = fn[tz][0][pc];
            const unsigned crow = ((unsigned)p * 16u + (unsigned)iz) * 16u + (unsigned)iy;
            f32x4 v = f32x4{c.x * a.inv, c.y * a.inv, c.z * a.inv, c.w * a.inv};
            if constexpr (MASK) {
                v.x = (nb & 1u) ? v.x : 0.f; v.y = (nb & 2u) ? v.y : 0.f;
                v.z = (nb & 4u) ? v.z : 0.f; v.w = (nb & 8u) ? v.w : 0.f;
            }
#ifndef T3_NO_OPAQUE
            asm volatile("" : "+v"(v));
#endif
            __builtin_amdgcn_raw_buffer_store_b128(__builtin_bit_cast(i32x4, v), out_rsrc, (int)st_o, (int)(crow * 1024u), 0);
            if constexpr (SUMS) {
                float s = (v.x + v.y) + (v.z + v.w);
                s += __shfl_xor(s, 16, 64);
                s += __shfl_xor(s, 32, 64);
                if (k == 0) s_odd = s;
                else
                    __builtin_amdgcn_raw_buffer_store_b32(__builtin_bit_cast(int, kg == 1 ? s_odd : s), sum_rsrc, (int)sm_o, (int)(crow * 64u), 0);
            }
            __builtin_amdgcn_sched_barrier(0);
            asm volatile("s_nop 3" :: "v"(v) T3_CLOBBER);
        }
    }
}

struct T8FwdArgs {
    const float *in;
    float *out;
    const unsigned short *W;
    const float *bias;
    float *osum;
    int N;
};
constexpr int T8_WBYTES = 27 * 3 * 1024;
constexpr int T8_ROWB = 8 * 64 + 32;
constexpr int T8_SLOT = 3 * T8_ROWB;
constexpr int T8_PLANE = 3 * T8_SLOT;
constexpr int T8_WAVE = 2 * T8_PLANE;

template <bool SUMS>
__global__ __launch_bounds__(512, 2) void t3d8_fwd_kernel(const T8FwdArgs a) {
    extern __shared__ __attribute__((aligned(16))) char t3lds[];
    {
        const i32x4 *src = reinterpret_cast<const i32x4 *>(a.W);
        i32x4 *dst = reinterpret_cast<i32x4 *>(t3lds);
        for (int i = threadIdx.x; i < T8_WBYTES / 16; i += 512) dst[i] = src[i];
    }
    __syncthreads();
    const int lane = threadIdx.x & 63, wave = __builtin_amdgcn_readfirstlane((int)(threadIdx.x >> 6));
    const int n = lane & 15, kg = lane >> 4, r = n >> 3, ix = n & 7;
    char *strip = t3lds + T8_WBYTES + wave * T8_WAVE;
    f32x4 bias4 = *reinterpret_cast<const f32x4 *>(a.bias + 4 * kg);
    asm volatile("" : "+v"(bias4));
    const __amdgpu_buffer_rsrc_t in_rsrc = sw_rsrc(a.in, (unsigned long long)a.N * 8 * 8 * 8 * 32 * 4);
    const __amdgpu_buffer_rsrc_t out_rsrc = sw_rsrc(a.out, (unsigned long long)a.N * 16 * 16 * 16 * 16 * 4);
    const __amdgpu_buffer_rsrc_t sum_rsrc = sw_rsrc(a.osum, SUMS ? (unsigned long long)a.N * 16 * 16 * 16 * 4 : 0ull);
    const int iz = wave;
    const char *wl = t3lds + lane * 16;
    const int npw = a.N > (int)blockIdx.x ? (a.N - (int)blockIdx.x + (int)gridDim.x - 1) / (int)gridDim.x : 0;
    const unsigned ld_off = (unsigned)lane * 16u;
    const int w_off = (lane >> 3) * 64 + (lane & 7) * 8;
    const int f_off0 = ix * 64 + kg * 16, f_off1 = (ix > 0 ? ix - 1 : 0) * 64 + kg * 16;
    const int keepx = ix > 0 ? -1 : 0;

    f32x4 R[2][4];
    auto fetch = [&](int u, int j, f32x4 *rr) __attribute__((always_inline)) {
        const bool ok = u >= 0 && u < npw;
        const int p = (int)blockIdx.x + (int)gridDim.x * (ok ? u : 0);
        const unsigned pb = (((unsigned)p * 8u + (unsigned)iz) * 8u + (unsigned)(2 * j)) * 1024u;
        const unsigned o0 = ok ? ld_off : SW_OOB, o1 = (ok && iz > 0) ? ld_off : SW_OOB;
        rr[0] = __builtin_bit_cast(f32x4, __builtin_amdgcn_raw_buffer_load_b128(in_rsrc, (int)o0, (int)pb, 0));
        rr[1] = __builtin_bit_cast(f32x4, __builtin_amdgcn_raw_buffer_load_b128(in_rsrc, (int)o0, (int)(pb + 1024u), 0));
        rr[2] = __builtin_bit_cast(f32x4, __builtin_amdgcn_raw_buffer_load_b128(in_rsrc, (int)o1, (int)(pb - 8u * 1024u), 0));
        rr[3] = __builtin_bit_cast(f32x4, __builtin_amdgcn_raw_buffer_load_b128(in_rsrc, (int)o1, (int)(pb - 8u * 1024u + 1024u), 0));
    };
#pragma unroll
    for (int b = 0; b < 2; ++b)
#pragma unroll
        for (int i = 0; i < 4; ++i) R[b][i] = f32x4{0.f, 0.f, 0.f, 0.f};

    if (npw > 0)
    for (int u = -1; u < npw; ++u) {
        const bool live = u >= 0;
        const int p = (int)blockIdx.x + (int)gridDim.x * (live ? u : 0);
#pragma unroll
        for (int j = 0; j < 4; ++j) {
            __builtin_amdgcn_sched_barrier(0);
            const int b = j & 1;
            const int s0 = (2 * j) % 3;
            if (j == 0) {
                for (int i = lane; i < 2 * 3 * (T8_ROWB / 16); i += 64) {
                    const int pl = i / (3 * (T8_ROWB / 16)), q = i % (3 * (T8_ROWB / 16));
                    *reinterpret_cast<i32x4 *>(strip + pl * T8_PLANE + s0 * T8_SLOT + q * 16) = i32x4{0, 0, 0, 0};
                }
            }
#pragma unroll
            for (int i = 0; i < 4; ++i) {
                const int pl = i >> 1, sl = (s0 + 1 + (i & 1)) % 3;
                float x = R[b][i].x, y = R[b][i].y, z = R[b][i].z, w = R[b][i].w;
                const unsigned h0 = t3_split2(x, y), h1 = t3_split2(z, w);
                const unsigned m0 = t3_split2(x, y), m1 = t3_split2(z, w);
                char *dst = strip + pl * T8_PLANE + sl * T8_SLOT + w_off;
                *reinterpret_cast<i32x2 *>(dst) = i32x2{(int)h0, (int)h1};
                *reinterpret_cast<i32x2 *>(dst + T8_ROWB) = i32x2{(int)m0, (int)m1};
                *reinterpret_cast<i32x2 *>(dst + 2 * T8_ROWB) = i32x2{(int)t3_pack2(x, y), (int)t3_pack2(z, w)};
            }
            fetch(j < 2 ? u : u + 1, (j + 2) & 3, R[b]);
            const int ro0 = (r ? (s0 + 2) % 3 : (s0 + 1) % 3) * T8_SLOT, ro1 = (r ? (s0 + 1) % 3 : s0 % 3) * T8_SLOT;
            f32x4 acc[8];
#pragma unroll
            for (int i = 0; i < 8; ++i) acc[i] = f32x4{0.f, 0.f, 0.f, 0.f};
#pragma unroll
            for (int d = 0; d < 8; ++d) {
                const int dz = d >> 2, dy = (d >> 1) & 1, dx = d & 1;
                const char *src = strip + dz * T8_PLANE + (dy ? ro1 : ro0) + (dx ? f_off1 : f_off0);
                i32x4 q0 = *reinterpret_cast<const i32x4 *>(src), q1 = *reinterpret_cast<const i32x4 *>(src + T8_ROWB), q2 = *reinterpret_cast<const i32x4 *>(src + 2 * T8_ROWB);
                if (dx) {
                    q0.x &= keepx; q0.y &= keepx; q0.z &= keepx; q0.w &= keepx;
                    q1.x &= keepx; q1.y &= keepx; q1.z &= keepx; q1.w &= keepx;
                    q2.x &= keepx; q2.y &= keepx; q2.z &= keepx; q2.w &= keepx;
                }
                const bf16x8 f0 = __builtin_bit_cast(bf16x8, q0), f1 = __builtin_bit_cast(bf16x8, q1), f2 = __builtin_bit_cast(bf16x8, q2);
#pragma unroll
                for (int qz = 0; qz < (dz ? 1 : 2); ++qz)
#pragma unroll
                    for (int qy = 0; qy < (dy ? 1 : 2); ++qy)
#pragma unroll
                        for (int qx = 0; qx < (dx ? 1 : 2); ++qx) {
                            const int cz = dz ? 1 : (qz ? 2 : 0), cy = dy ? 1 : (qy ? 2 : 0), cx = dx ? 1 : (qx ? 2 : 0);
                            const int pz = cz == 2, py = cy == 2, px = cx == 2;
                            const int combo = (cz * 3 + cy) * 3 + cx;
                            const bf16x8 w0 = *reinterpret_cast<const bf16x8 *>(wl + (combo * 3 + 0) * 1024);
                            const bf16x8 w1 = *reinterpret_cast<const bf16x8 *>(wl + (combo * 3 + 1) * 1024);
                            const bf16x8 w2 = *reinterpret_cast<const bf16x8 *>(wl + (combo * 3 + 2) * 1024);
                            f32x4 c = acc[(pz * 2 + py) * 2 + px];
                            c = __builtin_amdgcn_mfma_f32_16x16x32_bf16(w2, f0, c, 0, 0, 0);
                            c = __builtin_amdgcn_mfma_f32_16x16x32_bf16(w0, f2, c, 0, 0, 0);
                            c = __builtin_amdgcn_mfma_f32_16x16x32_bf16(w1, f1, c, 0, 0, 0);
                            c = __builtin_amdgcn_mfma_f32_16x16x32_bf16(w1, f0, c, 0, 0, 0);
                            c = __builtin_amdgcn_mfma_f32_16x16x32_bf16(w0, f1, c, 0, 0, 0);
                            c = __builtin_amdgcn_mfma_f32_16x16x32_bf16(w0, f0, c, 0, 0, 0);
                            acc[(pz * 2 + py) * 2 + px] = c;
                        }
            }
            const unsigned vb = (((unsigned)p * 16u + (unsigned)(2 * iz)) * 16u + (unsigned)(2 * (2 * j + r))) * 16u + (unsigned)(2 * ix);
            f32x4 vv[8];
#pragma unroll
            for (int i = 0; i < 8; ++i) {
                f32x4 v = acc[i];
                v.x += bias4.x; v.y += bias4.y; v.z += bias4.z; v.w += bias4.w;
                vv[i] = v;
            }
#pragma unroll
            for (int i = 0; i < 8; ++i) {
                const int pz = i >> 2, py = (i >> 1) & 1, px = i & 1;
                const unsigned vox = vb + (unsigned)(pz * 256 + py * 16 + px);
                __builtin_amdgcn_raw_buffer_store_b128(__builtin_bit_cast(i32x4, vv[i]), out_rsrc, (int)(live ? vox * 64u + (unsigned)kg * 16u : SW_OOB), 0, 0);
            }
            if constexpr (SUMS) {
// ... 178 lines not shown
```

Baseline: 290,800.

## Roll next-plane epilogue prefetches into row loop instead of tail bursts

In the c3d forward kernel, the weight-difference prefetches for the next plane are issued inside the epilogue row loop as ring slots free up, instead of as a burst after the row sweep. The 8-wave backward kernel does the same for mask loads and narrows the mask queue type. The t3d kernel with sums defers its mask byte load until after the current use. A debug knob to cap the forward grid and an info query for it are also added. The goal is to spread load latency across compute and reduce tail stalls, at the cost of more live registers for the second epilogue descriptor.

```diff
diff --git a/include/alq.h b/include/alq.h
--- a/include/alq.h
+++ b/include/alq.h
@@ -287,7 +287,8 @@
     ALQ_INFO_DCP_FORM = 16,
     ALQ_INFO_E3D_BWD_FORM = 17,
     ALQ_INFO_C3D_BWD_WAVES = 19,
-    ALQ_INFO_C3D_BWD_GRID = 20
+    ALQ_INFO_C3D_BWD_GRID = 20,
+    ALQ_INFO_C3D_FWD_GRID = 21
 };
 int alq_model_engine_info(alq_model *m, int what);
 
diff --git a/nn-active-learning_amd/csrc/alq_internal.h b/nn-active-learning_amd/csrc/alq_internal.h
--- a/nn-active-learning_amd/csrc/alq_internal.h
+++ b/nn-active-learning_amd/csrc/alq_internal.h
@@ -348,7 +348,8 @@
 int c3d_fwd_build(const View &in, const View &out, const int k[3], const int lo[3], const int s[3], C3dPlan *plan);
 void c3d_fwd_pack(C3dPlan *plan, const std::vector<float> &Bmat );
 int c3d_fwd_launch(alq_ctx *ctx, const C3dPlan &plan, const View &in, const float *bias, int N, const unsigned *amaxA, const unsigned *amaxB,
-                   const float *fc_W, float *fc_part, float *asum_part, unsigned char *fc_bits, float flip_tau);
+                   const float *fc_W, float *fc_part, float *asum_part, unsigned char *fc_bits, float flip_tau,
+                   int *grid_out = nullptr );
 int c3d_bwd_build(const View &fwd_in, const View &fwd_out, const int k[3], const int lo[3], const int s[3], C3dPlan *plan);
 void c3d_bwd_pack(C3dPlan *plan, const std::vector<float> &Bmat_fwd );
 void c3d_presplit_vec(const float *v, long long F, int e, std::vector<unsigned short> *out);
diff --git a/nn-active-learning_amd/csrc/c3d.hip b/nn-active-learning_amd/csrc/c3d.hip
--- a/nn-active-learning_amd/csrc/c3d.hip
+++ b/nn-active-learning_amd/csrc/c3d.hip
@@ -5,6 +5,7 @@
 #include <cmath>
 #include <cstdlib>
 #include <cstring>
+#include <type_traits>
 #include <vector>
 
 namespace alq {
@@ -20,7 +21,7 @@
 #define C3_WD 4
 #endif
 static_assert(C3_PF == 8 || C3_PF == 16, "the ring of staging registers must divide the 16 units of a plane");
-static_assert(C3_WD >= 1 && C3_WD <= 8, "weight-difference slices are fetched 1..8 rows ahead");
+static_assert(C3_WD >= 1 && C3_WD <= 8 && 8 % C3_WD == 0, "weight-difference slices are fetched 1, 2, 4 or 8 rows ahead: row i + C3_WD - 8 of the next plane takes the ring slot of row i");
 #ifndef C3_ABL
 #define C3_ABL 0
 #endif
@@ -203,20 +204,10 @@
         wdq[i % C3_WD] = __builtin_bit_cast(f32x4, __builtin_amdgcn_raw_buffer_load_b128(wd_rsrc, (int)E.off_w, (int)((E.row_f + (unsigned)i * 256u) * 4u), 0));
     };
 
-    auto wd_first = [&](const Epi &E) __attribute__((always_inline)) {
-        wd_load(E, IC<0>{});
-        if constexpr (C3_WD > 1) wd_load(E, IC<1>{});
-        if constexpr (C3_WD > 2) wd_load(E, IC<2>{});
-        if constexpr (C3_WD > 3) wd_load(E, IC<3>{});
-        if constexpr (C3_WD > 4) wd_load(E, IC<4>{});
-        if constexpr (C3_WD > 5) wd_load(E, IC<5>{});
-        if constexpr (C3_WD > 6) wd_load(E, IC<6>{});
-        if constexpr (C3_WD > 7) wd_load(E, IC<7>{});
-    };
-    auto epi_row = [&](auto S, auto I, const Epi &E) __attribute__((always_inline)) {
+    auto epi_row = [&](auto S, auto I, const Epi &E, const Epi &En) __attribute__((always_inline)) {
         constexpr int s = decltype(S)::value, i = decltype(I)::value;
         const f32x4 w4 = wdq[i % C3_WD];
-        if constexpr (i + C3_WD < 8) wd_load(E, IC<i + C3_WD>{});
+        if constexpr (i + C3_WD < 8) wd_load(E, IC<i + C3_WD>{}); else wd_load(En, IC<i + C3_WD - 8>{});
         const f32x4 c = acc[s][i];
         f32x4 val;
         if constexpr (ONEACC) {
@@ -295,6 +286,7 @@
         }
         const bool ev = z >= 2 || (z == 0 && pi > 0);
         const Epi E = epi_setup(ev, z >= 2 ? pi : pi - 1, z >= 2 ? z - 2 : D - 1);
+        const Epi En = epi_setup(z + 1 < D ? z >= 1 : true, pi, z + 1 < D ? z - 1 : D - 2);
 
         auto frag = [&](int j, int s, f16x8 &bh, f16x8 &bl) __attribute__((always_inline)) {
             const char *p = lds + abase + j * C3_ROW + s * 32;
@@ -308,7 +300,7 @@
             constexpr int j = decltype(J)::value, s = decltype(SS)::value, b = 2 * j + s;
             __builtin_amdgcn_sched_barrier(0);
             if constexpr (s == 0 && j < 8) {
-                if constexpr (!(C3_ABL & 2)) epi_row(IC<S_hi>{}, J, E);
+                if constexpr (!(C3_ABL & 2)) epi_row(IC<S_hi>{}, J, E, En);
             }
             if constexpr (!(C3_ABL & 1) && j >= 2) {
                 constexpr int u = 2 * (j - 2) + s;
@@ -355,10 +347,6 @@
         auto row = [&](auto J) __attribute__((always_inline)) { block(J, IC<0>{}); block(J, IC<1>{}); };
         row(IC<0>{}); row(IC<1>{}); row(IC<2>{}); row(IC<3>{}); row(IC<4>{});
         row(IC<5>{}); row(IC<6>{}); row(IC<7>{}); row(IC<8>{}); row(IC<9>{});
-        {
-            const Epi En = epi_setup(z + 1 < D ? z >= 1 : true, pi, z + 1 < D ? z - 1 : D - 2);
-            wd_first(En);
-        }
         if constexpr (R == 0) { if (z == 0 && pi > 0) finish_patch((int)patch_of(pi - 1)); }
         c1_pi = c2_pi; c1_z = c2_z;
         advance(c2_pi, c2_z);
@@ -366,14 +354,11 @@
     auto light = [&](auto S, int pe, int zo) __attribute__((always_inline)) {
         constexpr int s = decltype(S)::value;
         const Epi E = epi_setup(true, pe, zo);
-        auto rows = [&](auto I) __attribute__((always_inline)) { epi_row(S, I, E); };
+        const Epi En = epi_setup(zo == D - 2, pe, D - 1);
+        auto rows = [&](auto I) __attribute__((always_inline)) { epi_row(S, I, E, En); };
         rows(IC<0>{}); rows(IC<1>{}); rows(IC<2>{}); rows(IC<3>{}); rows(IC<4>{}); rows(IC<5>{}); rows(IC<6>{}); rows(IC<7>{});
 #pragma unroll
         for (int i = 0; i < 8; ++i) { acc[s][i] = f32x4{0.f, 0.f, 0.f, 0.f}; if constexpr (!ONEACC) accx[s][i] = f32x4{0.f, 0.f, 0.f, 0.f}; }
-        {
-            const Epi En = epi_setup(zo == D - 2, pe, D - 1);
-            wd_first(En);
-        }
     };
 
     __syncthreads();
@@ -891,7 +876,8 @@
     int c1_pi = 0, c1_z = 0, c2_pi = 0, c2_z = 0;
     auto advance = [&](int &pi, int &z) __attribute__((always_inline)) { if (++z == D) { z = 0; ++pi; } };
 
-    unsigned mkq[2][2] = {{0u, 0u}, {0u, 0u}};
+    typedef typename std::conditional<NW == 8, unsigned char, unsigned>::type mk_t;
+    mk_t mkq[2][2] = {{0, 0}, {0, 0}};
     struct Epi { unsigned pv; unsigned row_v; float inv; unsigned off_mask, off_dB, off_sum; };
     auto epi_setup = [&](bool valid, int pe, int zo) __attribute__((always_inline)) {
         Epi e;
@@ -905,6 +891,7 @@
     };
     auto mask_load = [&](const Epi &E, auto I) __attribute__((always_inline)) {
         constexpr int i = decltype(I)::value;
+        if constexpr (C3_B7ABL & 16) return;
 #pragma unroll
         for (int hx = 0; hx < 2; ++hx)
             mkq[i & 1][hx] = (unsigned char)__builtin_amdgcn_raw_buffer_load_b8(mask_rsrc, (int)E.off_mask,
@@ -912,10 +899,12 @@
     };
     const bool has_mask = a.maskA != nullptr;
     float t_keep = 0.f;
-    auto epi_half = [&](auto S, auto I, auto HX, const Epi &E) __attribute__((always_inline)) {
+    constexpr bool ROLL = NW == 8;
+    auto epi_half = [&](auto S, auto I, auto HX, const Epi &E, const Epi &En) __attribute__((always_inline)) {
         constexpr int s = decltype(S)::value, i = decltype(I)::value, hx = decltype(HX)::value;
         const unsigned mk = mkq[i & 1][hx];
         if constexpr (hx == 1 && i + 2 < RW) mask_load(E, IC<i + 2>{});
+        if constexpr (ROLL && hx == 1 && i + 2 >= RW) mask_load(En, IC<i + 2 - RW>{});
         const f32x4 c = acc[s][i][hx];
         const int nib = (lq < 2 && has_mask) ? (int)mk : 15;
         const float v0 = c.x * E.inv, v1 = c.y * E.inv, v2 = c.z * E.inv, v3 = c.w * E.inv;
@@ -944,9 +933,9 @@
             __builtin_amdgcn_raw_buffer_store_b32(__builtin_bit_cast(int, ts), sB_rsrc, (int)(lq >= 2 ? E.off_sum : SW_OOB), (int)(rowv * 4u), 0);
         }
     };
-    auto epi_row = [&](auto S, auto I, const Epi &E) __attribute__((always_inline)) {
-        epi_half(S, I, IC<0>{}, E);
-        epi_half(S, I, IC<1>{}, E);
+    auto epi_row = [&](auto S, auto I, const Epi &E, const Epi &En) __attribute__((always_inline)) {
+        epi_half(S, I, IC<0>{}, E, En);
+        epi_half(S, I, IC<1>{}, E, En);
     };
     auto s_weights = [&](int kill, f16x8 &sh, f16x8 &sl) __attribute__((always_inline)) {
         const int km = lq == kill ? 0 : -1;
@@ -980,6 +969,8 @@
         const unsigned z1 = (unsigned)c1_z, z2 = (unsigned)c2_z;
         const bool ev = z >= 2 || (z == 0 && pi > 0);
         const Epi E = epi_setup(ev, z >= 2 ? pi : pi - 1, z >= 2 ? z - 2 : D - 1);
+        Epi En{};
+        if constexpr (ROLL) En = epi_setup(z + 1 < D ? z >= 1 : true, pi, z + 1 < D ? z - 1 : D - 2);
         f16x8 sh, sl;
         s_weights(z == 1 ? 0 : -1, sh, sl);
 
@@ -1026,8 +1017,8 @@
                     frag_b(i, hx, fc);
                     if constexpr (!(C3_B7ABL & 4)) frag_s(i, hx, fc);
                     if constexpr (!(C3_B7ABL & 1)) {
-                        if (hx == 0) epi_half(IC<S_hi>{}, I, IC<0>{}, E);
-                        else epi_half(IC<S_hi>{}, I, IC<1>{}, E);
+                        if (hx == 0) epi_half(IC<S_hi>{}, I, IC<0>{}, E, En);
+                        else epi_half(IC<S_hi>{}, I, IC<1>{}, E, En);
                     } else { const f32x4 k0 = acc[S_hi][i][hx]; asm volatile("" :: "v"(k0)); }
                     if (hx == 0) frag_a(i, 1, fn);
                     else if (i < RW - 1) frag_a(i + 1, 0, fn);
@@ -1050,7 +1041,7 @@
                 }
                 return;
             }
-            if constexpr (!(C3_B7ABL & 1)) epi_row(IC<S_hi>{}, I, E);
+            if constexpr (!(C3_B7ABL & 1)) epi_row(IC<S_hi>{}, I, E, En);
             else { const f32x4 k0 = acc[S_hi][i][0], k1 = acc[S_hi][i][1]; asm volatile("" :: "v"(k0), "v"(k1)); }
             if constexpr ((i & 1) == 0 && !(C3_B7ABL & 2)) {
                 stage_unit(wbase, IC<i / 2>{});
@@ -1073,10 +1064,10 @@
         };
         row(IC<0>{}); row(IC<1>{}); row(IC<2>{}); row(IC<3>{});
         if constexpr (RW == 8) { row(IC<4>{}); row(IC<5>{}); row(IC<6>{}); row(IC<7>{}); }
-        {
-            const Epi En = epi_setup(z + 1 < D ? z >= 1 : true, pi, z + 1 < D ? z - 1 : D - 2);
-            mask_load(En, IC<0>{});
-            mask_load(En, IC<1>{});
+        if constexpr (!ROLL) {
+            const Epi Et = epi_setup(z + 1 < D ? z >= 1 : true, pi, z + 1 < D ? z - 1 : D - 2);
+            mask_load(Et, IC<0>{});
+            mask_load(Et, IC<1>{});
         }
         c1_pi = c2_pi; c1_z = c2_z;
         advance(c2_pi, c2_z);
@@ -1085,7 +1076,9 @@
         constexpr int s = decltype(S)::value;
         constexpr bool last = decltype(LAST)::value != 0;
         const Epi E = epi_setup(true, pe, zo);
-        auto rows = [&](auto I) __attribute__((always_inline)) { epi_row(S, I, E); };
+        Epi En{};
+        if constexpr (ROLL) En = epi_setup(zo == D - 2, pe, D - 1);
+        auto rows = [&](auto I) __attribute__((always_inline)) { epi_row(S, I, E, En); };
         rows(IC<0>{}); rows(IC<1>{}); rows(IC<2>{}); rows(IC<3>{});
         if constexpr (RW == 8) { rows(IC<4>{}); rows(IC<5>{}); rows(IC<6>{}); rows(IC<7>{}); }
 #pragma unroll
@@ -1105,10 +1098,10 @@
                     acc[sp][i][hx] = mac3(acc[sp][i][hx], sh, sl, bh, bl);
                 }
         }
-        {
-            const Epi En = epi_setup(zo == D - 2, pe, D - 1);
-            mask_load(En, IC<0>{});
-            mask_load(En, IC<1>{});
+        if constexpr (!ROLL) {
+            const Epi Et = epi_setup(zo == D - 2, pe, D - 1);
+            mask_load(Et, IC<0>{});
+            mask_load(Et, IC<1>{});
         }
     };
 
@@ -1198,7 +1191,8 @@
 }
 
 int c3d_fwd_launch(alq_ctx *ctx, const C3dPlan &plan, const View &in, const float *bias, int N, const unsigned *amaxA, const unsigned *amaxB,
-                   const float *fc_W, float *fc_part, float *asum_part, unsigned char *fc_bits, float flip_tau) {
+                   const float *fc_W, float *fc_part, float *asum_part, unsigned char *fc_bits, float flip_tau, int *grid_out) {
+    if (grid_out) *grid_out = 0;
     ALQ_REQUIRE(plan.ok && plan.d_W, ALQ_EINVAL, "c3d: weights not set");
     ALQ_REQUIRE(in.split == 8 && in.cs == 8 && in.C == 16 && in.D == plan.D && in.H == 32 && in.W == 32 && plan.D == 32, ALQ_EINVAL, "c3d: input view mismatch");
     ALQ_REQUIRE(amaxA && amaxB && fc_W && fc_part && bias, ALQ_EINVAL, "c3d: missing argument");
@@ -1208,7 +1202,9 @@
     a.inA = in.p; a.inB = in.p + in.delta; a.W = plan.d_W; a.bias = bias; a.amaxA = amaxA; a.amaxB = amaxB;
     a.fc_W = fc_W; a.fc_part = fc_part; a.asum_part = asum_part; a.fc_bits = fc_bits; a.N = N; a.D = plan.D; a.e_w = plan.w_exp;
     a.flip_tau = flip_tau; a.clk = nullptr;
-    const unsigned grid = (unsigned)std::min(N, 256);
+    unsigned grid = (unsigned)std::min(N, 256);
+    if (g_dbg_knobs[KNOB_C3F_GRID_CAP] > 0) grid = std::min<unsigned>(grid, (unsigned)g_dbg_knobs[KNOB_C3F_GRID_CAP]);
+    if (grid_out) *grid_out = (int)grid;
     ProfScope ps(ctx, PROF_IGEMM_F16, plan.flops_per_patch * N);
     auto go = [&](auto kfn) { return sweep_launch(ctx, kfn, grid, 256, C3_LDS, a); };
     if (fc_bits) return plan.oneacc ? go(c3d_fwd_kernel<true, true>) : go(c3d_fwd_kernel<true, false>);
diff --git a/nn-active-learning_amd/csrc/engine_switches.h b/nn-active-learning_amd/csrc/engine_switches.h
--- a/nn-active-learning_amd/csrc/engine_switches.h
+++ b/nn-active-learning_amd/csrc/engine_switches.h
@@ -17,11 +17,12 @@
     KNOB_DCP_NARROW = 8,
     KNOB_E3D_GRID_CAP = 9,
     KNOB_C3B7_GRID_CAP = 10,
-    ALQ_NKNOBS = 11
+    KNOB_C3F_GRID_CAP = 11,
+    ALQ_NKNOBS = 12
 };
 
 struct EngineSwitches {
-    int knobs[ALQ_NKNOBS] = {0, 0, 0, 0, 0, 0, 0, 0, 0, 0, 0};
+    int knobs[ALQ_NKNOBS] = {0, 0, 0, 0, 0, 0, 0, 0, 0, 0, 0, 0};
     int disable_v2 = 0;
     int disable_v3 = 0;
     int disable_v4 = 0;
diff --git a/nn-active-learning_amd/csrc/igemm2.hip b/nn-active-learning_amd/csrc/igemm2.hip
--- a/nn-active-learning_amd/csrc/igemm2.hip
+++ b/nn-active-learning_amd/csrc/igemm2.hip
@@ -507,7 +507,7 @@
 int g_no_f16x2 = 0;
 int g_no_xcd_order = 0;
 int g_no_fixed = 0;
-int g_dbg_knobs[ALQ_NKNOBS] = {0, 0, 0, 0, 0, 0, 0, 0, 0, 0, 0};
+int g_dbg_knobs[ALQ_NKNOBS] = {0, 0, 0, 0, 0, 0, 0, 0, 0, 0, 0, 0};
 
 template <int NTW, bool WRES, int GEO, bool SUMS>
 static int launch2_s(alq_ctx *ctx, const Igemm2Plan &plan, const Igemm2Args &a, unsigned grid) {
diff --git a/nn-active-learning_amd/csrc/model.hip b/nn-active-learning_amd/csrc/model.hip
--- a/nn-active-learning_amd/csrc/model.hip
+++ b/nn-active-learning_amd/csrc/model.hip
@@ -6,7 +6,7 @@
 
 using namespace alq;
 
-static int g_knob_override[ALQ_NKNOBS] = {-1, -1, -1, -1, -1, -1, -1, -1, -1, -1, -1};
+static int g_knob_override[ALQ_NKNOBS] = {-1, -1, -1, -1, -1, -1, -1, -1, -1, -1, -1, -1};
 
 static void apply_knobs(const alq_model *m) {
     for (int k = 0; k < ALQ_NKNOBS; ++k) g_dbg_knobs[k] = g_knob_override[k] >= 0 ? g_knob_override[k] : m->sw.knobs[k];
@@ -681,6 +681,7 @@
         case ALQ_INFO_E3D_BWD_FORM: return m->last.bwd.e3b_form;
         case ALQ_INFO_C3D_BWD_WAVES: return m->last.bwd.c3_bwd ? (m->sw.c3_bwd_rows == 7 ? m->sw.c3_bwd_waves : 1) : 0;
         case ALQ_INFO_C3D_BWD_GRID: return m->last.bwd.c3_bwd ? m->last.bwd.c3b_grid : 0;
+        case ALQ_INFO_C3D_FWD_GRID: return m->last.fwd.c3 ? m->last.fwd.c3f_grid : 0;
         default: break;
     }
     set_error("alq_model_engine_info: bad argument");
diff --git a/nn-active-learning_amd/csrc/model_types.h b/nn-active-learning_amd/csrc/model_types.h
--- a/nn-active-learning_amd/csrc/model_types.h
+++ b/nn-active-learning_amd/csrc/model_types.h
@@ -66,6 +66,7 @@
     struct Fwd {
         bool head_fused = false;
         bool c3 = false;
+        int c3f_grid = 0;
         int t3f = 0;
         int d3f = 0;
         int f3f = 0;
diff --git a/nn-active-learning_amd/csrc/passes.hip b/nn-active-learning_amd/csrc/passes.hip
--- a/nn-active-learning_amd/csrc/passes.hip
+++ b/nn-active-learning_amd/csrc/passes.hip
@@ -236,7 +236,7 @@
     if (P.c3_head)
         ALQ_TRY(c3d_fwd_launch(ctx, ly.c3f, in, ly.d_bias, N, fz.in_amax, fz.in_amax2, nx.fc_wv, nx.c3_part,
                                P.with_sums ? nx.c3_asum : nullptr, reinterpret_cast<unsigned char *>(fz.fc_bits),
-                               flipfix ? std::ldexp(ly.fwd_l1, -24) : 0.f));
+                               flipfix ? std::ldexp(ly.fwd_l1, -24) : 0.f, &m->last.fwd.c3f_grid));
     else
         ALQ_TRY(igemm4_launch(ctx, ly.fwd[0].p4, in, ly.out, ly.d_bias, ly.spec.relu, 0, N, PROF_IGEMM3_FWD, &fz));
     if (flipfix)
diff --git a/nn-active-learning_amd/csrc/t3d.hip b/nn-active-learning_amd/csrc/t3d.hip
--- a/nn-active-learning_amd/csrc/t3d.hip
+++ b/nn-active-learning_amd/csrc/t3d.hip
@@ -273,9 +273,15 @@
             for (int ty = 0; ty < 2; ++ty)
                 r[tz * 2 + ty] = __builtin_bit_cast(f32x4, __builtin_amdgcn_raw_buffer_load_b128(in_rsrc, (int)(tz < 2 ? okl : ok2),
                                                                                                  (int)(b0 + (unsigned)tz * 32768u + (unsigned)ty * 1024u), 0));
-        if constexpr (MASK)
+        if constexpr (MASK && !SUMS)
             mk = (unsigned)(unsigned char)__builtin_amdgcn_raw_buffer_load_b8(msk_rsrc, (int)(c.ok ? mk_off : SW_OOB),
                                                                              (int)((((unsigned)c.p * 16u + (unsigned)c.iz) * 16u + (unsigned)iy) * 64u), 0);
+    };
+    auto fetch_mask = [&](int T, unsigned &mk) __attribute__((always_inline)) {
+        const T3Cur c = t3_tile(T, total, wave);
+        const int iy = 15 - c.s;
+        mk = (unsigned)(unsigned char)__builtin_amdgcn_raw_buffer_load_b8(msk_rsrc, (int)(c.ok ? mk_off : SW_OOB),
+                                                                         (int)((((unsigned)c.p * 16u + (unsigned)c.iz) * 16u + (unsigned)iy) * 64u), 0);
     };
 #pragma unroll
     for (int k = 0; k < T3B_PF; ++k) {
@@ -344,6 +350,7 @@
             if constexpr (MASK) {
                 v.x = (nb & 1u) ? v.x : 0.f; v.y = (nb & 2u) ? v.y : 0.f;
                 v.z = (nb & 4u) ? v.z : 0.f; v.w = (nb & 8u) ? v.w : 0.f;
+                if constexpr (SUMS) fetch_mask(T + T3B_PF, MK[k]);
             }
 #ifndef T3_NO_OPAQUE
             asm volatile("" : "+v"(v));
```

Result: no change. 291,700 (median of 6 runs) (+0.3%).
